# mlelarge/graph_neural_net

Measured on AMD Instinct MI355X. Metric: graph-pairs/sec FGNN fwd+bwd, N=50 regular pairs, higher is better.
Workload: dtype f32

## Files before the change

graph_neural_net_amd/_lib.py:

```python
import ctypes as C
import os

import torch

_HERE = os.path.dirname(os.path.abspath(__file__))
LIB_PATH = os.environ.get('FGNN_LIB') or os.path.join(_HERE, 'libfgnn_hip.so')

FGNN_H = 32
FGNN_TILE = 32
FGNN_MAX_DEPTH = 3
FGNN_RANGE_WG = 256
FGNN_LSAP_MAX_N = 2048
FGNN_MAX_LEVELS = 64
FGNN_QAP_MAX_N = 256
FGNN_QAPW_MAX_N = 256
FGNN_SPECTRAL_MAX_N = 256
FGNN_SPECTRAL_MAX_POWERS = 8
FGNN_PLANTED_MAX_N = 256
FGNN_SCORE_SPLIT = 4

c_float_p = C.c_void_p


class Slab(C.Structure):
    _fields_ = [('ptr', C.c_void_p), ('gstride', C.c_longlong), ('ldp', C.c_longlong), ('C', C.c_int),
                ('nrm', C.c_void_p), ('beta', C.c_void_p)]


class MlpFwdArgs(C.Structure):
    _fields_ = [('G', C.c_int), ('N', C.c_int), ('depth', C.c_int), ('nmlp', C.c_int),
                ('nvalid', C.c_void_p),
                ('a', Slab), ('b', Slab),
                ('W', (C.c_void_p * FGNN_MAX_DEPTH) * 2),
                ('bias', (C.c_void_p * FGNN_MAX_DEPTH) * 2),
                ('z', C.c_void_p * 2),
                ('ldz', C.c_longlong),
                ('part', C.c_void_p * 2),
                ('cnt', C.c_void_p), ('packed', C.c_void_p), ('xbits', C.c_void_p), ('xdeg', C.c_void_p),
                ('ranges', C.c_void_p), ('cu_share', C.c_int)]


class DwJob(C.Structure):
    _fields_ = [('dy', C.c_void_p), ('d_gstride', C.c_longlong), ('d_ld', C.c_longlong), ('relu_mask', C.c_void_p),
                ('x', C.c_void_p), ('x_gstride', C.c_longlong), ('x_ld', C.c_longlong), ('M', C.c_int), ('K', C.c_int)]


class ChainLayer(C.Structure):
    _fields_ = [('W', C.c_void_p), ('w_ostride', C.c_longlong), ('w_kstride', C.c_longlong), ('bias', C.c_void_p),
                ('M', C.c_int), ('K', C.c_int), ('relu', C.c_int), ('mask', C.c_void_p), ('out', C.c_void_p),
                ('o_gstride', C.c_longlong)]


class ChainArgs(C.Structure):
    _fields_ = [('x', C.c_void_p), ('x_gstride', C.c_longlong), ('x_ld', C.c_longlong), ('depth', C.c_int),
                ('layer', ChainLayer * 3), ('o_ld', C.c_longlong), ('nvalid', C.c_void_p), ('G', C.c_int), ('N', C.c_int)]


class Mlp64Args(C.Structure):
    _fields_ = [('x', C.c_void_p), ('x_gstride', C.c_longlong), ('x_ld', C.c_longlong), ('cin', C.c_int),
                ('xb', C.c_void_p), ('xb_gstride', C.c_longlong), ('xb_ld', C.c_longlong), ('cb', C.c_int),
                ('packed', C.c_void_p), ('nvalid', C.c_void_p), ('G', C.c_int), ('N', C.c_int),
                ('out', C.c_void_p), ('o_gstride', C.c_longlong), ('o_ld', C.c_longlong),
                ('dz', C.c_void_p), ('dz_gstride', C.c_longlong), ('dz_ld', C.c_longlong),
                ('dx', C.c_void_p), ('dx_gstride', C.c_longlong), ('dx_ld', C.c_longlong),
                ('dxb', C.c_void_p), ('dxb_gstride', C.c_longlong), ('dxb_ld', C.c_longlong),
                ('accumulate_dx', C.c_int), ('accumulate_dxb', C.c_int),
                ('wpart', C.c_void_p)]


class Mlp64PackJob(C.Structure):
    _fields_ = [('W', C.c_void_p * 3), ('bias', C.c_void_p * 3), ('cin', C.c_int), ('packed', C.c_void_p)]


class MlpBwdArgs(C.Structure):
    _fields_ = [('G', C.c_int), ('N', C.c_int), ('depth', C.c_int),
                ('nvalid', C.c_void_p),
                ('a', Slab), ('b', Slab),
                ('W', C.c_void_p * FGNN_MAX_DEPTH),
                ('bias', C.c_void_p * FGNN_MAX_DEPTH),
                ('dy', C.c_void_p), ('dgstride', C.c_longlong), ('ldd', C.c_longlong),
                ('z', C.c_void_p), ('zgstride', C.c_longlong), ('ldz', C.c_longlong),
                ('coef', C.c_void_p), ('s12', C.c_void_p), ('znrm', C.c_void_p),
                ('dxa', C.c_void_p), ('dxa_gstride', C.c_longlong), ('dxa_ld', C.c_longlong),
                ('dxb', C.c_void_p), ('dxb_gstride', C.c_longlong), ('dxb_ld', C.c_longlong),
                ('accumulate_a', C.c_int), ('accumulate_b', C.c_int),
                ('wpart', C.c_void_p), ('s12part', C.c_void_p), ('packed', C.c_void_p),
                ('s12tiles', C.c_void_p), ('s12_out', C.c_void_p), ('xbits', C.c_void_p), ('xdeg', C.c_void_p),
                ('ranges', C.c_void_p), ('cu_share', C.c_int)]


class Slab16(C.Structure):
    _fields_ = [('ptr', C.c_void_p), ('gstride', C.c_longlong), ('ldp', C.c_longlong), ('C', C.c_int),
                ('nrm', C.c_void_p), ('beta', C.c_void_p)]


class MlpFwd16Args(C.Structure):
    _fields_ = [('G', C.c_int), ('N', C.c_int), ('ldr', C.c_int), ('depth', C.c_int), ('nmlp', C.c_int),
                ('nvalid', C.c_void_p),
                ('a', Slab16), ('b', Slab16),
                ('z', C.c_void_p * 2), ('ldz', C.c_longlong),
                ('part', C.c_void_p * 2), ('cnt', C.c_void_p), ('packed', C.c_void_p), ('ranges', C.c_void_p)]


class MlpBwd16Args(C.Structure):
    _fields_ = [('G', C.c_int), ('N', C.c_int), ('ldr', C.c_int), ('depth', C.c_int),
                ('nvalid', C.c_void_p),
                ('a', Slab16), ('b', Slab16),
                ('dy', C.c_void_p), ('dgstride', C.c_longlong), ('ldd', C.c_longlong),
                ('z', C.c_void_p), ('zgstride', C.c_longlong), ('ldz', C.c_longlong),
                ('coef', C.c_void_p),
                ('dxa', C.c_void_p), ('dxa_gstride', C.c_longlong), ('dxa_ld', C.c_longlong),
                ('dxb', C.c_void_p), ('dxb_gstride', C.c_longlong), ('dxb_ld', C.c_longlong),
                ('accumulate_a', C.c_int), ('accumulate_b', C.c_int),
                ('wpart', C.c_void_p), ('s12part', C.c_void_p), ('packed', C.c_void_p), ('ranges', C.c_void_p)]


class GradJob(C.Structure):
    _fields_ = [('wpart', C.c_void_p), ('count', C.c_int), ('out', C.c_void_p), ('s12', C.c_void_p),
                ('nrm', C.c_void_p), ('dgn_w', C.c_void_p), ('dgn_b', C.c_void_p), ('rows', C.c_int), ('scale', C.c_float), ('scale_dev', C.c_void_p)]


class PackJob(C.Structure):
    _fields_ = [('kind', C.c_int), ('ca', C.c_int), ('cb', C.c_int), ('depth', C.c_int), ('nmlp', C.c_int),
                ('W', (C.c_void_p * FGNN_MAX_DEPTH) * 2), ('bias', (C.c_void_p * FGNN_MAX_DEPTH) * 2),
                ('out', C.c_void_p)]


class PairgenArgs(C.Structure):
    _fields_ = [('seed', C.c_ulonglong), ('first', C.c_longlong), ('B', C.c_int), ('N', C.c_int),
                ('family', C.c_int), ('noise_model', C.c_int), ('edge_density', C.c_double),
                ('thr_edge', C.c_ulonglong), ('thr_noise1', C.c_ulonglong), ('thr_noise2', C.c_ulonglong),
                ('thr_vertex', C.c_ulonglong), ('swaps_per_edge', C.c_int),
                ('bits1', C.c_void_p), ('bits2', C.c_void_p), ('nvalid', C.c_void_p)]


FGNN_GUARD_MAX_PARTS = 64
FGNN_GUARD_SKIP_NONFINITE = 1
FGNN_GUARD_NONFINITE = 1


class GuardRecord(C.Structure):
    _fields_ = [('max_norm', C.c_double), ('norm', C.c_double), ('coef', C.c_double),
                ('flags', C.c_int), ('skipped', C.c_int), ('arrivals', C.c_int), ('mode', C.c_int),
                ('partial', C.c_double * FGNN_GUARD_MAX_PARTS)]


class EvalRecord(C.Structure):
    _fields_ = [('ce_sum', C.c_double), ('nodes', C.c_longlong), ('correct_lsap', C.c_longlong), ('correct_max', C.c_longlong),
                ('pairs', C.c_longlong), ('steps', C.c_longlong)]


MAX_GRAD_JOBS = 16
MAX_PACK_JOBS = 24
_VP, _LL, _I, _F = C.c_void_p, C.c_longlong, C.c_int, C.c_float

_SIGNATURES = {
    'fgnn_last_error': [],
    'fgnn_version': [],
    'fgnn_tiles_per_graph': [_I],
    'fgnn_mlp_bwd_num_workgroups': [],
    'fgnn_pack_floats': [_I, _I, _I, _I, _I],
    'fgnn_pack_operands': [_VP, _I, _VP],
    'fgnn_mlp_fwd': [C.POINTER(MlpFwdArgs), _VP],
    'fgnn_pack_x3_floats': [_I, _I, _I, _I, _I],
    'fgnn_pack_x3_operands': [_VP, _I, _VP],
    'fgnn_mlp_fwd_x3': [C.POINTER(MlpFwdArgs), _VP],
    'fgnn_debug_mlp_fwd_masks': [C.POINTER(MlpFwdArgs), _VP, _VP, _VP],
    'fgnn_debug_mlp_fwd_x3_masks': [C.POINTER(MlpFwdArgs), _VP, _VP, _VP],
    'fgnn_debug_matmul_variant': [_I],
    'fgnn_gn_finalize': [_VP, _VP, _VP, _VP, _I, _I, _I, _F, _VP, _VP],
    'fgnn_gn_finalize2': [_VP, _VP, _VP, _VP, _VP, _VP, _I, _I, _I, _F, _VP, _VP, _VP],
    'fgnn_gn_plane_supported': [_I],
    'fgnn_gn_plane_fwd': [_VP, _LL, _LL, _VP, _VP, _VP, _I, _I, _I, _F, _VP, _LL, _LL, _VP, _VP],
    'fgnn_gn_plane_bwd': [_VP, _LL, _LL, _VP, _LL, _LL, _VP, _VP, _I, _I, _I, _VP, _LL, _LL, _VP, _VP, _VP, _VP],
    'fgnn_gn_stats': [_VP, _LL, _LL, _VP, _VP, _I, _I, _I, _F, _VP, _VP],
    'fgnn_gn_apply': [_VP, _LL, _LL, _VP, _VP, _VP, _I, _I, _I, _VP, _LL, _LL, _VP],
    'fgnn_ragged_tile_ranges': [_VP, _I, _I, _VP, _VP],
    'fgnn_ragged_tile_ranges_order': [_VP, _I, _I, _VP, _VP, _VP],
    'fgnn_ragged_tile_ranges16': [_VP, _I, _I, _I, _VP, _VP],
    'fgnn_conv1x1_dw_multi': [C.POINTER(DwJob), _I, _VP, _I, _I, _VP, _VP],
    'fgnn_conv_chain_supported': [_I, _I, C.POINTER(C.c_int)],
    'fgnn_conv_chain': [C.POINTER(ChainArgs), _VP],
    'fgnn_mlp64_supported': [_I, _I, _I],
    'fgnn_mlp64_num_workgroups': [],
    'fgnn_mlp64_param_count': [_I],
    'fgnn_mlp64_packed_floats': [_I],
    'fgnn_mlp64_pack': [_VP, _VP, _VP, _VP, _VP, _VP, _I, _VP, _VP],
    'fgnn_mlp64_pack_multi': [C.POINTER(Mlp64PackJob), _I, _VP],
    'fgnn_mlp64_fwd': [C.POINTER(Mlp64Args), _VP],
    'fgnn_mlp64_bwd': [C.POINTER(Mlp64Args), _VP],
    'fgnn_conv1x1': [_VP, _LL, _LL, _VP, _VP, _LL, _LL, _VP, _I, _VP, _I, _I, _I, _I, _VP, _LL, _LL, _VP],
    'fgnn_conv1x1_dw_chunks': [_I, _I],
    'fgnn_conv1x1_dw': [_VP, _LL, _LL, _VP, _VP, _LL, _LL, _VP, _I, _I, _I, _I, _VP, _VP],
    'fgnn_chan_matmul_fwd': [C.POINTER(Slab), C.POINTER(Slab), _VP, _I, _I, _VP, _LL, _LL, _VP],
    'fgnn_chan_matmul_fwd_ord': [C.POINTER(Slab), C.POINTER(Slab), _VP, _I, _I, _VP, _LL, _LL, _VP, _I, _VP],
    'fgnn_chan_matmul_fwd_fin_supported': [_I],
    'fgnn_chan_matmul_fwd_fin': [C.POINTER(Slab), C.POINTER(Slab), _VP, _VP, _VP, _VP, _VP, _F, _VP, _I, _I, _VP, _LL, _LL, _VP],
    'fgnn_chan_matmul_fwd_fin_ord': [C.POINTER(Slab), C.POINTER(Slab), _VP, _VP, _VP, _VP, _VP, _F, _VP, _I, _I, _VP, _LL, _LL, _VP, _I, _VP],
    'fgnn_colmax_fwd': [C.POINTER(Slab), _VP, _I, _I, _VP, _VP, _VP],
    'fgnn_colmax_fwd_fin_supported': [_I],
    'fgnn_colmax_fwd_fin': [C.POINTER(Slab), _VP, _VP, _VP, _F, _VP, _I, _I, _VP, _VP, _VP],
    'fgnn_score_ce_fwd': [_VP, _VP, _VP, _I, _I, _I, _VP, _VP, _VP, _VP],
    'fgnn_score_row_blocks': [_I, _I],
    'fgnn_score_ce_fwd_blocks': [_VP, _VP, _VP, _I, _I, _I, _I, _VP, _VP, _VP, _VP],
    'fgnn_score_ce_bwd': [_VP, _VP, _VP, _VP, _VP, _VP, _I, _I, _I, _VP, _VP, _VP],
    'fgnn_score_ce_fwd_blocks_labels': [_VP, _VP, _VP, _VP, _I, _I, _I, _I, _VP, _VP, _VP, _VP],
    'fgnn_score_ce_bwd_labels': [_VP, _VP, _VP, _VP, _VP, _VP, _VP, _I, _I, _I, _VP, _VP, _VP],
    'fgnn_score_ce_bwd_w': [_VP, _VP, _VP, _VP, _VP, _VP, _VP, _VP, _I, _I, _I, _VP, _VP, _VP],
    'fgnn_pair_weights': [_VP, _VP, _I, _VP, _I, _I, _VP, _VP, _VP],
    'fgnn_pair_loss_w': [_VP, _I, _VP, _I, _VP, _VP],
    'fgnn_ce_fwd_labels': [_VP, _VP, _VP, _I, _I, _VP, _VP, _VP],
    'fgnn_ce_bwd_labels': [_VP, _VP, _VP, _VP, _VP, _I, _I, _VP, _VP],
    'fgnn_inv_node_count': [_VP, _I, _VP, _VP],
    'fgnn_score_bwd': [_VP, _VP, _VP, _VP, _I, _I, _I, _VP, _VP, _VP],
    'fgnn_ce_fwd': [_VP, _VP, _I, _I, _VP, _VP, _VP],
    'fgnn_ce_bwd': [_VP, _VP, _VP, _VP, _I, _I, _VP, _VP],
    'fgnn_colmax_bwd': [_VP, _VP, _VP, _I, _I, _I, _VP, _LL, _LL, C.POINTER(Slab), _VP, _VP],
    'fgnn_gn_bwd_stats': [_VP, _LL, _LL, _VP, _LL, _LL, _VP, _VP, _I, _I, _I, _VP, _VP],
    'fgnn_gn_bwd_coef': [_VP, _VP, _VP, _I, _I, _I, _VP, _VP, _VP, _VP],
    'fgnn_gn_bwd_coef_tiles': [_VP, _VP, _VP, _I, _I, _I, _VP, _VP, _VP],
    'fgnn_grad_finalize': [_VP, _I, _I, _I, _I, _VP],
    'fgnn_gn_bwd_apply': [_VP, _LL, _LL, _VP, _LL, _LL, _VP, _VP, _I, _I, _I, _VP, _LL, _LL, _VP],
    'fgnn_mlp_bwd': [C.POINTER(MlpBwdArgs), _VP],
    'fgnn_mlp_bwd_x3': [C.POINTER(MlpBwdArgs), _VP],
    'fgnn_mlp_bwd_pair': [C.POINTER(MlpBwdArgs), C.POINTER(MlpBwdArgs), _VP],
    'fgnn_mlp_bwd_t16': [C.POINTER(MlpBwdArgs), _VP],
    'fgnn_mlp_bwd_t16_supported': [C.POINTER(MlpBwdArgs)],
    'fgnn_mlp_bwd_pair_t16': [C.POINTER(MlpBwdArgs), C.POINTER(MlpBwdArgs), _VP],
    'fgnn_mlp_bwd_pair_x3': [C.POINTER(MlpBwdArgs), C.POINTER(MlpBwdArgs), _VP],
    'fgnn_block1_struct_supported': [_I, _I, _I],
    'fgnn_block1_struct_table_floats': [_I],
    'fgnn_block1_struct_ws_floats': [_I, _I],
    'fgnn_block1_struct_rows': [_I, _I],
    'fgnn_block1_struct_fwd': [_VP, _VP, _I, _I, _VP, _VP, _VP, _VP, _VP, C.c_float, _VP, _VP, _VP, _LL, _LL, _VP, _VP, _VP, _VP, _VP, _VP, _VP],
    'fgnn_block1_struct_bwd': [_VP, _VP, _I, _I, _VP, _VP, _VP, _VP, _VP, _VP, _VP, _VP, _LL, _LL, _VP, _VP, _VP, _VP, _VP, _VP],
    'fgnn_block1_struct_fwd_pack': [_VP, _VP, _I, _I, _VP, _VP, _VP, _VP, _VP, C.c_float, _VP, _VP, _VP, _LL, _LL, _VP, _VP, _VP, _VP, _VP, _VP, _VP, _I, _VP],
    'fgnn_block1_struct_fwd16_pack': [_VP, _VP, _I, _I, _I, _VP, _VP, _VP, _VP, _VP, C.c_float, _VP, _VP, _VP, _LL, _LL, _VP, _VP, _VP, _VP, _VP, _VP, _VP, _I, _VP],
    'fgnn_block1_struct_fwd16': [_VP, _VP, _I, _I, _I, _VP, _VP, _VP, _VP, _VP, C.c_float, _VP, _VP, _VP, _LL, _LL, _VP, _VP, _VP, _VP, _VP, _VP, _VP],
    'fgnn_block1_struct_bwd16': [_VP, _VP, _I, _I, _I, _VP, _VP, _VP, _VP, _VP, _VP, _VP, _VP, _LL, _LL, _VP, _VP, _VP, _VP, _VP, _VP],
    'fgnn_mlp_bwd_coef_tiles_supported': [_I, _I],
    'fgnn_mlp_param_count': [_I, _I],
    'fgnn_reduce_partials': [_VP, _I, _I, _VP, _VP],
    'fgnn_chan_matmul_bwd': [C.POINTER(Slab), C.POINTER(Slab), _VP, _LL, _LL, _VP, _I, _I, _VP, _VP, _LL, _LL, _VP, _VP, _VP],
    'fgnn_chan_matmul_bwd_ord': [C.POINTER(Slab), C.POINTER(Slab), _VP, _LL, _LL, _VP, _I, _I, _VP, _VP, _LL, _LL, _VP, _VP, _VP, _I, _VP],
    'fgnn_sum_scale': [_VP, _I, _I, _F, _VP, _VP],
    'fgnn_adam_step': [_VP, _VP, _VP, _VP, _I, C.c_double, C.c_double, C.c_double, C.c_double, _I, C.c_double, _VP],
    'fgnn_adam_step_dev': [_VP, _VP, _VP, _VP, _I, _VP, _VP, _VP],
    'fgnn_grad_guard': [_VP, _I, _VP, _VP, _VP],
    'fgnn_adam_step_guarded': [_VP, _VP, _VP, _VP, _I, _VP, _VP, _VP, _VP],
    'fgnn_expand_adjacency': [_VP, _VP, _I, _I, _VP, _VP],
    'fgnn_pack_adjacency': [_VP, _VP, _I, _I, _VP, _VP, _VP],
    'fgnn_pack_adjacency_ld': [_VP, _VP, _I, _I, _I, _VP, _VP, _VP],
    'fgnn_pack_adjacency_pair': [_VP, _VP, _VP, _VP, _I, _I, _I, _VP, _VP, _VP, _VP, _VP],
    'fgnn_adjacency_degree': [_VP, _VP, _I, _I, _VP, _VP],
    'fgnn_accuracy_max': [_VP, _VP, _I, _I, _VP, _VP],
    'fgnn_lsap_accuracy': [_VP, _LL, _I, _VP, _I, _I, _VP, _VP, _VP],
    'fgnn_pairgen_supported': [_I, _I, _I],
    'fgnn_pairgen': [C.POINTER(PairgenArgs), _VP],
    'fgnn_pairgen_indexed': [C.POINTER(PairgenArgs), _VP, _VP],
    'fgnn_pairgen_levels': [C.POINTER(PairgenArgs), _VP, _VP, _I, _VP, _VP],
    'fgnn_epoch_index': [C.c_ulonglong, C.c_ulonglong, _LL, _LL, _LL, _VP, _VP],
    'fgnn_qap_objective': [_VP, _VP, _VP, _VP, _I, _I, _VP, _VP, _VP, _VP, _VP],
    'fgnn_qap_improve_cost': [_VP, _VP, _VP, _VP, _I, _I, _VP, _LL, _I, _VP],
    'fgnn_greedy_qap_ws_bytes': [_I, _I],
    'fgnn_greedy_qap': [_VP, _VP, _VP, _VP, _I, _I, _I, _VP, _LL, _VP, _VP, _VP, _VP, _VP],
    'fgnn_greedy_qap_labels': [_VP, _VP, _VP, _VP, _VP, _I, _I, _I, _VP, _LL, _VP, _VP, _VP, _VP, _VP],
    'fgnn_qapw_objective': [_VP, _VP, _LL, _I, _VP, _VP, _I, _I, _VP, _VP, _VP, _VP, _VP, _VP],
    'fgnn_qapw_improve_cost': [_VP, _VP, _LL, _I, _VP, _VP, _I, _I, _VP, _LL, _I, _VP],
    'fgnn_greedy_qapw_ws_bytes': [_I, _I],
    'fgnn_greedy_qapw': [_VP, _VP, _LL, _I, _VP, _VP, _I, _I, _I, _VP, _LL, _VP, _VP, _VP, _VP, _VP],
    'fgnn_greedy_qapw_labels': [_VP, _VP, _LL, _I, _VP, _VP, _VP, _I, _I, _I, _VP, _LL, _VP, _VP, _VP, _VP, _VP],
    'fgnn_planted_perm': [C.c_ulonglong, _LL, _VP, _VP, _I, _I, _VP, _VP],
    'fgnn_relabel_bits': [_VP, _VP, _VP, _I, _I, _VP, _VP],
    'fgnn_relabel_dense': [_VP, _VP, _VP, _I, _I, _I, _I, _VP, _VP],
    'fgnn_count_matches': [_VP, _VP, _VP, _I, _I, _VP, _VP],
    'fgnn_accuracy_max_labels': [_VP, _VP, _VP, _I, _I, _VP, _VP],
    'fgnn_spectral_features': [_VP, _VP, _I, _I, _I, _VP, _I, _VP],
    'fgnn_eval_pairs': [_VP, _VP, _VP, _I, _I, _VP, _LL, _I, _VP, _VP, _VP],
    'fgnn_eval_pairs_labels': [_VP, _VP, _VP, _I, _I, _VP, _LL, _I, _VP, _VP, _VP],
    'fgnn_eval_fold': [_VP, _VP, _VP, _VP, _I, _I, _I, _VP, _VP, _VP, _VP],
    'fgnn_eval_fold_bins': [_VP, _VP, _VP, _VP, _I, _I, _I, _VP, _I, _VP, _VP, _VP, _VP],
    'fgnn_tiles_per_graph16': [_I, _I],
    'fgnn_to_bf16': [_VP, _VP, _I, _I, _I, _I, _VP, _LL, _LL, _VP],
    'fgnn_from_bf16': [_VP, _LL, _LL, _I, _I, _I, _I, _VP, _VP],
    'fgnn_to_bf16_pad': [_VP, _VP, _I, _I, _I, _I, _I, _VP, _LL, _VP],
    'fgnn_pack16_floats': [_I, _I, _I, _I, _I],
    'fgnn_pack16_operands': [_VP, _I, _VP],
    'fgnn_mlp_fwd16': [C.POINTER(MlpFwd16Args), _VP],
    'fgnn_debug_mlp_fwd16_masks': [C.POINTER(MlpFwd16Args), _VP, _VP, _VP],
    'fgnn_gn_finalize_tpg': [_VP, _VP, _VP, _VP, _I, _I, _I, _I, _F, _VP, _VP],
    'fgnn_gn_finalize2_tpg': [_VP, _VP, _VP, _VP, _VP, _VP, _I, _I, _I, _I, _F, _VP, _VP, _VP],
    'fgnn_gn_bwd_coef_tiles_tpg': [_VP, _VP, _VP, _I, _I, _I, _I, _VP, _VP, _VP],
    'fgnn_chan_matmul_fwd16': [C.POINTER(Slab16), C.POINTER(Slab16), _VP, _I, _I, _I, _VP, _LL, _LL, _VP],
    'fgnn_chan_matmul_fwd16_fin': [C.POINTER(Slab16), C.POINTER(Slab16), _VP, _VP, _VP, _VP, _VP, _F, _I, _VP, _I, _I, _I, _VP, _LL,
                                   _LL, _VP],
    'fgnn_chan_matmul_bwd16': [C.POINTER(Slab16), C.POINTER(Slab16), _VP, _LL, _LL, _VP, _I, _I, _I, _VP, _VP, _LL, _LL, _VP, _VP, _VP],
    'fgnn_chan_matmul_bwd16_t': [C.POINTER(Slab16), C.POINTER(Slab16), _VP, _LL, _LL, _VP, _I, _VP, _I, _I, _I, _VP, _VP, _LL, _LL,
                                 _VP, _VP, _VP],
    'fgnn_chan_matmul_bwd16_tc': [C.POINTER(Slab16), C.POINTER(Slab16), _VP, _LL, _LL, _VP, _I, _VP, _I, _I, _I, _VP, _VP, _LL, _LL,
                                  _VP, _VP, _VP, _VP, _VP],
    'fgnn_colmax_bwd16_coef': [_VP, _VP, _VP, _I, _I, _I, _I, _VP, _LL, _LL, C.POINTER(Slab16), _VP, _VP, _VP],
    'fgnn_colmax_fwd16': [C.POINTER(Slab16), _VP, _I, _I, _I, _VP, _VP, _VP],
    'fgnn_colmax_bwd16': [_VP, _VP, _VP, _I, _I, _I, _I, _VP, _LL, _LL, C.POINTER(Slab16), _VP, _VP],
    'fgnn_mlp_bwd16': [C.POINTER(MlpBwd16Args), _VP],
    'fgnn_mlp_bwd16_pair': [C.POINTER(MlpBwd16Args), C.POINTER(MlpBwd16Args), _VP],
}
_RESTYPES = {'fgnn_last_error': C.c_char_p, 'fgnn_block1_struct_ws_floats': C.c_longlong, 'fgnn_greedy_qap_ws_bytes': C.c_longlong,
             'fgnn_greedy_qapw_ws_bytes': C.c_longlong}
EXPORTS = tuple(_SIGNATURES)

_lib = None


def load(allow_missing=False):
    global _lib
    if _lib is not None:
        return _lib
    if not os.path.exists(LIB_PATH):
        raise RuntimeError(
            'graph_neural_net_amd: %s is missing. Build it with '
            '`python -c "import __graft_entry__ as g; g.build()"` or `make -C graph_neural_net_amd/csrc`. '
            'There is no CPU fallback.' % LIB_PATH)
    lib = C.CDLL(LIB_PATH)
    for name, argtypes in _SIGNATURES.items():
        if allow_missing and not hasattr(lib, name):
            continue
        fn = getattr(lib, name)
        fn.argtypes = argtypes
        fn.restype = _RESTYPES.get(name, C.c_int)
    _lib = lib
    return lib


def last_error():
    return load().fgnn_last_error().decode('utf-8', 'replace')


PROFILE = None


def call(name, *args, tag=None):
    if PROFILE is not None:
        e0 = torch.cuda.Event(enable_timing=True)
        e1 = torch.cuda.Event(enable_timing=True)
        e0.record()
        rc = getattr(load(), name)(*args)
        e1.record()
        PROFILE.append((tag or name, e0, e1, name, args))
    else:
        rc = getattr(load(), name)(*args)
    if rc != 0:
        raise RuntimeError('%s failed (rc=%d): %s' % (name, rc, last_error()))


def relaunch(name, args):
    rc = getattr(load(), name)(*args[:-1], stream_ptr())
    if rc != 0:
        raise RuntimeError('%s failed (rc=%d): %s' % (name, rc, last_error()))


def stream_ptr():
    return C.c_void_p(torch.cuda.current_stream().cuda_stream)


def ptr(t):
    if t is None:
        return None
    if not t.is_cuda:
        raise RuntimeError('graph_neural_net_amd: expected a CUDA/HIP tensor, got device %s '
                           '(there is no CPU path)' % (t.device,))
    return C.c_void_p(t.data_ptr())


def make_slab(t, gstride, ldp, channels, nrm=None, beta=None):
    s = Slab()
    s.ptr = t.data_ptr() if t is not None else None
    s.gstride = gstride
    s.ldp = ldp
    s.C = channels
    s.nrm = nrm.data_ptr() if nrm is not None else None
    s.beta = beta.data_ptr() if beta is not None else None
    return s


def make_slab16(t, gstride, ldp, channels, nrm=None, beta=None):
    s = Slab16()
    s.ptr = t.data_ptr() if t is not None else None
    s.gstride = gstride
    s.ldp = ldp
    s.C = channels
    s.nrm = nrm.data_ptr() if nrm is not None else None
    s.beta = beta if isinstance(beta, int) else (beta.data_ptr() if beta is not None else None)
    return s


def tiles_per_graph(n):
    return (n * n + FGNN_TILE - 1) // FGNN_TILE


def mlp_param_count(cin, depth):
    return 32 * cin + 32 + (depth - 1) * (32 * 32 + 32)
```

graph_neural_net_amd/csrc/fgnn_bwd32.h:

```cpp
#pragma once
#include "fgnn_common.h"

namespace {

constexpr int BWD_WG = 256;
constexpr int NW = 8;
constexpr int NP = 4;
static_assert(BWD_WG == FGNN_RANGE_WG, "fgnn_ragged_tile_ranges splits for the backward grid");

DEVI float4 coef_from_sums(const float4 n, const float2 sv, float nv) {
    const float m = nv * nv;
    float4 k;
    k.x = n.x;
    k.y = n.y;
    k.z = m > 0.f ? -n.y * sv.y * n.w / m : 0.f;
    k.w = m > 0.f ? -n.y * sv.x / m : 0.f;
    return k;
}
DEVI float4 coef_record(const fgnn_mlp_bwd_args &A, int g, int ch, int nv) {
    if (A.coef) return reinterpret_cast<const float4 *>(A.coef)[(long long)g * FGNN_H + ch];
    const float4 n = reinterpret_cast<const float4 *>(A.znrm)[(long long)g * FGNN_H + ch];
    const float2 sv = reinterpret_cast<const float2 *>(A.s12)[(long long)g * FGNN_H + ch];
    return coef_from_sums(n, sv, (float)nv);
}
DEVI float4 coef_record(const fgnn_mlp_bwd_args &A, int g, int ch) {
    if (A.coef) return reinterpret_cast<const float4 *>(A.coef)[(long long)g * FGNN_H + ch];
    const float4 n = reinterpret_cast<const float4 *>(A.znrm)[(long long)g * FGNN_H + ch];
    const float2 sv = reinterpret_cast<const float2 *>(A.s12)[(long long)g * FGNN_H + ch];
    return coef_from_sums(n, sv, (float)nvalid_of(A.nvalid, g, A.N));
}


struct PairArgs {
    fgnn_mlp_bwd_args m[2];
};

template <int PCOUNT, int NWV>
DEVI void sum_wave_partials(const float *smem, float *wpart) {
    static_assert(PCOUNT % 4 == 0, "partials are summed four at a time");
    float4 *out = reinterpret_cast<float4 *>(wpart + (long long)blockIdx.x * PCOUNT);
    const float4 *part4 = reinterpret_cast<const float4 *>(smem);
    for (int e = threadIdx.x; e < PCOUNT / 4; e += 64 * NWV) {
        float4 a = part4[e];
#pragma unroll
        for (int w = 1; w < NWV; ++w) {
            const float4 b = part4[w * (PCOUNT / 4) + e];
            a.x += b.x;
            a.y += b.y;
            a.z += b.z;
            a.w += b.w;
        }
        out[e] = a;
    }
}
template <int PCOUNT>
DEVI void sum_pair_partials(const float *smem, const PairArgs &P) {
    static_assert(PCOUNT % 4 == 0, "partials are summed four at a time");
    const float4 *part4 = reinterpret_cast<const float4 *>(smem);
    for (int e = threadIdx.x; e < 2 * (PCOUNT / 4); e += 64 * NW) {
        const int m = e >= PCOUNT / 4 ? 1 : 0, ee = e - m * (PCOUNT / 4);
        float4 a = part4[(4 * m) * (PCOUNT / 4) + ee];
#pragma unroll
        for (int w = 1; w < NP; ++w) {
            const float4 b = part4[(4 * m + w) * (PCOUNT / 4) + ee];
            a.x += b.x;
            a.y += b.y;
            a.z += b.z;
            a.w += b.w;
        }
        reinterpret_cast<float4 *>(P.m[m].wpart + (long long)blockIdx.x * PCOUNT)[ee] = a;
    }
}

inline int check_mlp_bwd_common(const fgnn_mlp_bwd_args *a, const char *fn, int tile_bits) {
    FGNN_CHECK(a->dy && a->z && a->wpart, "%s: missing dy/z/wpart", fn);
    FGNN_CHECK(a->coef || (a->s12 && a->znrm) || (a->s12tiles && a->znrm), "%s: need coef, or s12 + znrm, or s12tiles + znrm", fn);
    const long long lim = 0x7fffffffll / 4, G = a->G;
    FGNN_CHECK(G * a->a.gstride < lim && G * a->b.gstride < lim && G * a->dgstride < lim && G * a->zgstride < lim &&
               G * a->dxa_gstride < lim && G * a->dxb_gstride < lim,
               "%s: a tensor exceeds 2 GiB (32-bit buffer addressing); split the batch", fn);
    FGNN_CHECK(G * fgnn_tiles_per_graph(a->N) < (1ll << tile_bits), "%s: too many tiles", fn);
    FGNN_CHECK(BWD_WG == fgnn_mlp_bwd_num_workgroups(), "%s: workgroup count differs from fgnn_mlp_bwd", fn);
    return 0;
}
inline int check_pair_common(const fgnn_mlp_bwd_args *a1, const fgnn_mlp_bwd_args *a2, const char *fn, int tile_bits, bool dense_only) {
    FGNN_CHECK(a1 && a2, "%s: null args", fn);
    FGNN_CHECK(BWD_WG == fgnn_mlp_bwd_num_workgroups(), "%s: workgroup count differs from fgnn_mlp_bwd", fn);
    FGNN_CHECK(a1->G > 0 && a1->N > 0 && a1->G == a2->G && a1->N == a2->N && a1->depth == a2->depth,
               "%s: the two MLPs must share G, N and depth", fn);
    FGNN_CHECK((!dense_only || a1->a.ptr) && a1->a.ptr == a2->a.ptr && a1->a.C == a2->a.C && a1->a.gstride == a2->a.gstride &&
               a1->a.ldp == a2->a.ldp && a1->a.nrm == a2->a.nrm && a1->a.beta == a2->a.beta &&
               (dense_only || (a1->xbits == a2->xbits && a1->xdeg == a2->xdeg)) && a1->nvalid == a2->nvalid,
               "%s: the two MLPs must read the same input slab", fn);
    FGNN_CHECK(!a1->dxa && !a1->s12part, "%s: the input gradient and its tile sums belong to the SECOND argument block", fn);
    FGNN_CHECK(!a1->s12tiles && !a2->s12tiles, "%s: s12tiles is an mlp3 feature", fn);
    for (const fgnn_mlp_bwd_args *a : {a1, a2}) {
        FGNN_CHECK(a->dy && a->z && a->wpart, "%s: missing dy/z/wpart", fn);
        FGNN_CHECK(a->coef || (a->s12 && a->znrm), "%s: need coef, or s12 + znrm", fn);
        const long long lim = 0x7fffffffll / 4, G = a->G;
        FGNN_CHECK(G * a->a.gstride < lim && G * a->dgstride < lim && G * a->zgstride < lim && G * a->dxa_gstride < lim,
                   "%s: a tensor exceeds 2 GiB (32-bit buffer addressing); split the batch", fn);
    }
    FGNN_CHECK((long long)a1->G * fgnn_tiles_per_graph(a1->N) < (1ll << tile_bits), "%s: too many tiles", fn);
    return 0;
}

}
```

graph_neural_net_amd/csrc/fgnn_bwd_t16.h:

```cpp
#pragma once
#include "fgnn_t16.h"
#include "fgnn_pack.h"
#include "fgnn_bwd32.h"

namespace {

using namespace t16;

template <int CB, int IMAGES, int NSLOTS>
struct BwdT16Layout {
    static constexpr int DEPTH = 3;
    static constexpr PkBwd PK = pk_bwd(32, CB, DEPTH);
    static constexpr int OFF_W1 = PK.off_wh, OFF_WT1 = PK.off_wt, OFF_WT2 = PK.off_wt + 16;
    static constexpr int BIAS_F = PK.bias_f;
    static constexpr int WEIGHT_F = pk_pad_floats(PK.floats);
    static constexpr int NSLOT = NSLOTS;
    static constexpr int CIN = 32 + CB;
    static constexpr int PCOUNT = 32 * CIN + 32 + (DEPTH - 1) * (32 * 32 + 32);
    static constexpr int TILE_OFF = IMAGES * WEIGHT_F;
    static constexpr int TILE_END = TILE_OFF + NW * NSLOT * TILE_F;
    static constexpr int RED_F = NW * PCOUNT;
};


#define FGNN_T16_READ_RECORDS(norm)                                 \
    _Pragma("unroll") for (int s = 0; s < 8; ++s) {                 \
        const float4 k4 = rec[chan_s(s) + chan_q(q)];               \
        kx[s] = k4.x;                                               \
        ky[s] = k4.y;                                               \
        kz[s] = k4.z;                                               \
        kw[s] = k4.w;                                               \
        if (norm) {                                                 \
            const float4 n = rec[32 + chan_s(s) + chan_q(q)];       \
            mean[s] = n.x;                                          \
            av[s] = n.y;                                            \
        }                                                           \
    }

#define FGNN_T16_RECOMPUTE_HIDDEN(acc, h1, h2)                                              \
    _Pragma("unroll") for (int s = 0; s < 8; ++s) h1[s] = relu1(acc[s >> 2][s & 3]);        \
    stage8(S0, lane_base, h1);                                                              \
    load_bias(acc, wl + L::BIAS_F, 1, q);                                                   \
    gemm32<L::OFF_W1>(acc, wl, h1, lane);                                                   \
    _Pragma("unroll") for (int s = 0; s < 8; ++s) h2[s] = relu1(acc[s >> 2][s & 3]);        \
    stage8(S1, lane_base, h2);

#define FGNN_T16_DZ(dpre)                                                                                                   \
    _Pragma("unroll") for (int s = 0; s < 8; ++s) dpre[s] = fmaf(kz[s], zr[s] - kx[s], fmaf(ky[s], dyr[s], kw[s]));         \
    if (!full) {                                                                                                            \
        _Pragma("unroll") for (int s = 0; s < 8; ++s) dpre[s] = valid ? dpre[s] : 0.f;                                      \
    }

#define FGNN_T16_HIDDEN_BWD(OFF_WT, dpre, dW, db, Dt, In, h)                                                \
    {                                                                                                       \
        f32x4 a2[2];                                                                                        \
        a2[0] = a2[1] = zero4();                                                                            \
        gemm32<OFF_WT>(a2, wl, dpre, lane);                                                                 \
        wgrad16(dW, db, Dt, In, lane);                                                                      \
        _Pragma("unroll") for (int s = 0; s < 8; ++s) dpre[s] = h[s] > 0.f ? a2[s >> 2][s & 3] : 0.f;       \
    }

#define FGNN_T16_DB_BUTTERFLY(db0, db1, db2)            \
    _Pragma("unroll") for (int b = 0; b < 2; ++b) {     \
        db0[b] += __shfl_xor(db0[b], 16);               \
        db0[b] += __shfl_xor(db0[b], 32);               \
        db1[b] += __shfl_xor(db1[b], 16);               \
        db1[b] += __shfl_xor(db1[b], 32);               \
        db2[b] += __shfl_xor(db2[b], 16);               \
        db2[b] += __shfl_xor(db2[b], 32);               \
    }

}
```

graph_neural_net_amd/csrc/fgnn_norm.h:

```cpp
#pragma once
#include "fgnn_common.h"

DEVI float4 nrm_record(float mean, float m2, float m, float nv, float w, float eps) {
    const float var = m > 0.f ? m2 / m : 0.f;
    const float ve = var + eps;
    const float q = nv > 0.f ? 1.f / (2.f * sqrtf(nv * ve)) : 0.f;
    float4 o;
    o.x = mean;
    o.y = w * q;
    o.z = q;
    o.w = 1.f / ve;
    return o;
}

struct TilePartials {
    float nb[4], mb[4], qb[4];
};
DEVI TilePartials finalize_load(const float *part, const float *cnt, int g, int c, int C, int tpg, int lane, bool tr = false) {
    TilePartials p;
    const int ts = tr ? 1 : C, cs = tr ? tpg : 1;
#pragma unroll
    for (int k = 0; k < 4; ++k) {
        const int t = lane + WAVE * k;
        const bool ok = t < tpg;
        const int tc = ok ? t : 0;
        const float n = cnt[(long long)g * tpg + tc];
        const float2 pm = reinterpret_cast<const float2 *>(part)[(long long)g * tpg * C + (long long)tc * ts + (long long)c * cs];
        p.nb[k] = ok ? n : 0.f;
        p.mb[k] = pm.x;
        p.qb[k] = ok ? pm.y : 0.f;
    }
    return p;
}
DEVI float4 finalize_reduce(const TilePartials &p, float nv, float w, float eps) {
    float sn = 0.f, sm = 0.f;
#pragma unroll
    for (int k = 0; k < 4; ++k) {
        sn += p.nb[k];
        sm += p.nb[k] * p.mb[k];
    }
    sn = wave_sum(sn);
    sm = wave_sum(sm);
    const float mean = sn > 0.f ? sm / sn : 0.f;
    float m2 = 0.f;
#pragma unroll
    for (int k = 0; k < 4; ++k) {
        const float d = p.mb[k] - mean;
        m2 += p.qb[k] + p.nb[k] * d * d;
    }
    m2 = wave_sum(m2);
    return nrm_record(mean, m2, sn, nv, w, eps);
}

struct NormRec {
    float mean, a, beta;
    bool on;
};
DEVI NormRec norm_of(const fgnn_slab &s, int g, int c) {
    NormRec r;
    r.on = s.nrm != nullptr;
    if (r.on) {
        const float4 n = reinterpret_cast<const float4 *>(s.nrm)[(long long)g * s.C + c];
        r.mean = n.x;
        r.a = n.y;
        r.beta = s.beta ? s.beta[c] : 0.f;
    } else {
        r.mean = 0.f;
        r.a = 1.f;
        r.beta = 0.f;
    }
    return r;
}
DEVI NormRec norm_from(const float4 &n, const fgnn_slab &s, int c) {
    NormRec r;
    r.on = true;
    r.mean = n.x;
    r.a = n.y;
    r.beta = s.beta ? s.beta[c] : 0.f;
    return r;
}

DEVI float4 finalize_wave(const float *part, const float *cnt, int g, int c, int C, int tpg, float nv, float w, float eps,
                          int lane, bool tr = false) {
    return finalize_reduce(finalize_load(part, cnt, g, c, C, tpg, lane, tr), nv, w, eps);
}
DEVI float4 finalize_wave_any(const float *part, const float *cnt, int g, int c, int C, int tpg, float nv, float w, float eps, int lane,
                              bool tr = false) {
    if (tpg <= 4 * WAVE) return finalize_wave(part, cnt, g, c, C, tpg, nv, w, eps, lane, tr);
    constexpr int U = 8;
    float sn = 0.f, sm = 0.f;
    const float *cg = cnt + (long long)g * tpg;
    const int ts = tr ? 1 : C;
    const float2 *pg = reinterpret_cast<const float2 *>(part) + (long long)g * tpg * C + (long long)c * (tr ? tpg : 1);
    for (int t0 = lane; t0 < tpg; t0 += U * WAVE) {
        float n[U], x[U];
#pragma unroll
        for (int k = 0; k < U; ++k) {
            const int t = t0 + k * WAVE, tc = t < tpg ? t : 0;
            n[k] = t < tpg ? cg[tc] : 0.f;
            x[k] = pg[(long long)tc * ts].x;
        }
#pragma unroll
        for (int k = 0; k < U; ++k) {
            sn += n[k];
            sm += n[k] * x[k];
        }
    }
    sn = wave_sum(sn);
    sm = wave_sum(sm);
    const float mean = sn > 0.f ? sm / sn : 0.f;
    float m2 = 0.f;
    for (int t0 = lane; t0 < tpg; t0 += U * WAVE) {
        float n[U];
        float2 pm[U];
#pragma unroll
        for (int k = 0; k < U; ++k) {
            const int t = t0 + k * WAVE, tc = t < tpg ? t : 0;
            n[k] = t < tpg ? cg[tc] : 0.f;
            pm[k] = pg[(long long)tc * ts];
            if (t >= tpg) pm[k].y = 0.f;
        }
#pragma unroll
        for (int k = 0; k < U; ++k) {
            const float d = pm[k].x - mean;
            m2 += pm[k].y + n[k] * d * d;
        }
    }
    m2 = wave_sum(m2);
    return nrm_record(mean, m2, sn, nv, w, eps);
}
```

graph_neural_net_amd/csrc/matmul.hip:

```cpp
#include "fgnn_common.h"
#include "fgnn_norm.h"

namespace {

constexpr int TM = 64;
constexpr int LDS_LD = 65;

DEVI void stage_tile(float *lds, const float *mat, int N, int nv, int row0, int col0, const NormRec &nr, int tid) {
    if (row0 == 0 && col0 == 0 && N <= TM) {
        for (int e = tid; e < TM * TM; e += 256) lds[(e >> 6) * LDS_LD + (e & 63)] = 0.f;
        __syncthreads();
        const int P = N * N;
        for (int e = tid; e < P; e += 256) {
            const int r = e / N, c = e - r * N;
            float v = mat[e];
            const bool ok = r < nv && c < nv;
            v = ok ? (nr.on ? (v - nr.mean) * nr.a + nr.beta : v) : 0.f;
            lds[r * LDS_LD + c] = v;
        }
    } else {
        for (int e = tid; e < TM * TM; e += 256) {
            const int r = e >> 6, c = e & 63;
            const int gr = row0 + r, gc = col0 + c;
            float v = 0.f;
            if (gr < nv && gc < nv) {
                v = mat[(long long)gr * N + gc];
                if (nr.on) v = (v - nr.mean) * nr.a + nr.beta;
            }
            lds[r * LDS_LD + c] = v;
        }
    }
}

DEVI void store_quadrant(float *out, int N, int row0, int col0, const f32x16 &acc, int lane) {
    const int j = lane & 31, h = lane >> 5;
    const int col = col0 + j;
#pragma unroll
    for (int r = 0; r < 16; ++r) {
        const int row = row0 + ch_of(r, h);
        if (row < N && col < N) out[(long long)row * N + col] = acc[r];
    }
}

DEVI void s12_epilogue(float (&red)[4][4], float sa1, float sa2, float sb1, float sb2, float *s12a, float *s12b, int gc, int tid) {
    const int lane = tid & 63, wave = tid >> 6;
    sa1 = wave_sum(sa1);
    sa2 = wave_sum(sa2);
    sb1 = wave_sum(sb1);
    sb2 = wave_sum(sb2);
    if (lane == 0) {
        red[wave][0] = sa1;
        red[wave][1] = sa2;
        red[wave][2] = sb1;
        red[wave][3] = sb2;
    }
    __syncthreads();
    if (tid < 4) {
        const float v = (red[0][tid] + red[1][tid]) + (red[2][tid] + red[3][tid]);
        float *dst = (tid < 2 ? s12a : s12b) + (long long)gc * 2 + (tid & 1);
        *dst = v;
    }
}

__global__ __launch_bounds__(256) void chan_matmul_fwd_kernel(const fgnn_slab ya, const fgnn_slab yb,
                                                              const int *nvalid, int N, float *out,
                                                              long long ogstride, long long ldo) {
    __shared__ float As[TM * LDS_LD];
    __shared__ float Bs[TM * LDS_LD];
    const int C = ya.C;
    const int gc = blockIdx.z;
    const int g = gc / C, c = gc - g * C;
    const int nv = nvalid_of(nvalid, g, N);
    const int row0 = blockIdx.y * TM, col0 = blockIdx.x * TM;
    const int tid = threadIdx.x, lane = tid & 63, wave = tid >> 6;
    const int qi = wave >> 1, qj = wave & 1;
    const int j = lane & 31, h = lane >> 5;
    const float *A = ya.ptr + (long long)g * ya.gstride + (long long)c * ya.ldp;
    const float *B = yb.ptr + (long long)g * yb.gstride + (long long)c * yb.ldp;
    const NormRec na = norm_of(ya, g, c), nb = norm_of(yb, g, c);
    float *O = out + (long long)g * ogstride + (long long)c * ldo;

    f32x16 acc;
#pragma unroll
    for (int r = 0; r < 16; ++r) acc[r] = 0.f;
    const bool live = (row0 + 32 * qi < N) && (col0 + 32 * qj < N);

    for (int k0 = 0; k0 < N; k0 += TM) {
        if (k0) __syncthreads();
        stage_tile(As, A, N, nv, row0, k0, na, tid);
        stage_tile(Bs, B, N, nv, k0, col0, nb, tid);
        __syncthreads();
        if (live) {
            const int kmax = (N - k0 < TM ? N - k0 : TM);
            const float *ap = As + (32 * qi + j) * LDS_LD + h;
            const float *bp = Bs + h * LDS_LD + 32 * qj + j;
            for (int k = 0; k < kmax; k += 2) acc = mfma32(ap[k], bp[k * LDS_LD], acc);
        }
    }
    if (live) store_quadrant(O, N, row0 + 32 * qi, col0 + 32 * qj, acc, lane);
}

__global__ __launch_bounds__(256) void chan_matmul_bwd_kernel(const fgnn_slab ya, const fgnn_slab yb,
                                                              const float *dm, long long dmg, long long ldm,
                                                              const int *nvalid, int N, float *da, float *db,
                                                              long long ogstride, long long ldo, float *s12a,
                                                              float *s12b) {
    __shared__ float Xs[TM * LDS_LD];
    __shared__ float Ds[TM * LDS_LD];
    __shared__ float red[4][4];
    const int C = ya.C;
    const int gc = blockIdx.z;
    const int g = gc / C, c = gc - g * C;
    const int nv = nvalid_of(nvalid, g, N);
    const int row0 = blockIdx.y * TM, col0 = blockIdx.x * TM;
    const int tid = threadIdx.x, lane = tid & 63, wave = tid >> 6;
    const int qi = wave >> 1, qj = wave & 1;
    const int j = lane & 31, h = lane >> 5;
    const float *A = ya.ptr + (long long)g * ya.gstride + (long long)c * ya.ldp;
    const float *B = yb.ptr + (long long)g * yb.gstride + (long long)c * yb.ldp;
    const float *D = dm + (long long)g * dmg + (long long)c * ldm;
    const NormRec na = norm_of(ya, g, c), nb = norm_of(yb, g, c);
    NormRec none;
    none.on = false; none.mean = 0.f; none.a = 1.f; none.beta = 0.f;
    float *OA = da + (long long)g * ogstride + (long long)c * ldo;
    float *OB = db + (long long)g * ogstride + (long long)c * ldo;
    const bool live = (row0 + 32 * qi < N) && (col0 + 32 * qj < N);

    f32x16 acc;
#pragma unroll
    for (int r = 0; r < 16; ++r) acc[r] = 0.f;
    for (int j0 = 0; j0 < N; j0 += TM) {
        if (j0) __syncthreads();
        stage_tile(Ds, D, N, nv, row0, j0, none, tid);
        stage_tile(Xs, B, N, nv, col0, j0, nb, tid);
        __syncthreads();
        if (live) {
            const int kmax = (N - j0 < TM ? N - j0 : TM);
            const float *ap = Ds + (32 * qi + j) * LDS_LD + h;
            const float *bp = Xs + (32 * qj + j) * LDS_LD + h;
            for (int k = 0; k < kmax; k += 2) acc = mfma32(ap[k], bp[k], acc);
        }
    }
    if (live) store_quadrant(OA, N, row0 + 32 * qi, col0 + 32 * qj, acc, lane);
    float sa1 = 0.f, sa2 = 0.f, sb1 = 0.f, sb2 = 0.f;
    if (s12a && live) {
        const int col = col0 + 32 * qj + j;
#pragma unroll
        for (int r = 0; r < 16; ++r) {
            const int row = row0 + 32 * qi + ch_of(r, h);
            if (row < nv && col < nv) {
                sa1 += acc[r];
                sa2 += acc[r] * (A[(long long)row * N + col] - na.mean);
            }
        }
    }

#pragma unroll
    for (int r = 0; r < 16; ++r) acc[r] = 0.f;
    for (int i0 = 0; i0 < N; i0 += TM) {
        __syncthreads();
        stage_tile(Xs, A, N, nv, i0, row0, na, tid);
        stage_tile(Ds, D, N, nv, i0, col0, none, tid);
        __syncthreads();
        if (live) {
            const int kmax = (N - i0 < TM ? N - i0 : TM);
            const float *ap = Xs + h * LDS_LD + 32 * qi + j;
            const float *bp = Ds + h * LDS_LD + 32 * qj + j;
            for (int k = 0; k < kmax; k += 2) acc = mfma32(ap[k * LDS_LD], bp[k * LDS_LD], acc);
        }
    }
    if (live) store_quadrant(OB, N, row0 + 32 * qi, col0 + 32 * qj, acc, lane);
    if (s12a) {
        if (live) {
            const int col = col0 + 32 * qj + j;
#pragma unroll
            for (int r = 0; r < 16; ++r) {
                const int row = row0 + 32 * qi + ch_of(r, h);
                if (row < nv && col < nv) {
                    sb1 += acc[r];
                    sb2 += acc[r] * (B[(long long)row * N + col] - nb.mean);
                }
            }
        }
        s12_epilogue(red, sa1, sa2, sb1, sb2, s12a, s12b, gc, tid);
    }
}

template <bool WANT_U>
DEVI void load_tile_regs(float (&v)[16], float (&u)[16], const float *mat, int N, int nv, const NormRec &nr, int tid) {
#pragma unroll
    for (int k = 0; k < 16; ++k) {
        const int e = tid + 256 * k;
        const int r = e >> 6, c = e & 63;
        const bool ok = r < nv && c < nv;
        const float x = mat[ok ? r * N + c : 0];
        const float d = x - nr.mean;
        v[k] = ok ? (nr.on ? d * nr.a + nr.beta : x) : 0.f;
        if (WANT_U) u[k] = ok ? d : 0.f;
    }
}
DEVI void store_tile_lds(float *lds, const float (&v)[16], int tid) {
#pragma unroll
    for (int k = 0; k < 16; ++k) {
        const int e = tid + 256 * k;
        lds[(e >> 6) * LDS_LD + (e & 63)] = v[k];
    }
}
DEVI void frag_to_lds(float *lds, int row0, int col0, const f32x16 &acc, int lane) {
    const int j = lane & 31, h = lane >> 5;
#pragma unroll
    for (int r = 0; r < 16; ++r) lds[(row0 + ch_of(r, h)) * LDS_LD + col0 + j] = acc[r];
}
template <bool WANT_S>
DEVI void tile_to_global(const View &ov, int mat_off4, const float *lds, int N, const float (&u)[16], float &s1,
                         float &s2, int tid) {
    const int c = tid & 63, r0 = __builtin_amdgcn_readfirstlane(tid >> 6);
    const int voff = c < N ? (r0 * N + c) * 4 : OOB_OFF;
    const float *lp = lds + r0 * LDS_LD + c;
#pragma unroll
    for (int k = 0; k < 16; ++k) {
        const float t = lp[4 * k * LDS_LD];
        buf_store(t, ov, r0 + 4 * k < N ? voff : OOB_OFF, mat_off4 + k * 16 * N);
        if (WANT_S) {
            s1 += t;
            s2 += t * u[k];
        }
    }
}

DEVI void load_tile_raw(float (&x)[16], const View &v, int mat_off4, int N, int nv, int tid) {
    const int c = tid & 63, r0 = __builtin_amdgcn_readfirstlane(tid >> 6);
    const int voff = c < nv ? (r0 * N + c) * 4 : OOB_OFF;
#pragma unroll
    for (int k = 0; k < 16; ++k) {
        const int r = r0 + 4 * k;
        x[k] = buf_load(v, r < nv ? voff : OOB_OFF, mat_off4 + k * 16 * N);
    }
}
template <bool WANT_U>
DEVI void finish_tile(float (&v)[16], float (&u)[16], const float (&x)[16], int nv, const NormRec &nr, int tid) {
#pragma unroll
    for (int k = 0; k < 16; ++k) {
        const int e = tid + 256 * k;
        const int r = e >> 6, c = e & 63;
        const bool ok = r < nv && c < nv;
        const float d = x[k] - nr.mean;
        v[k] = ok ? (nr.on ? d * nr.a + nr.beta : x[k]) : 0.f;
        if (WANT_U) u[k] = ok ? d : 0.f;
    }
}

struct FinArgs {
    const float *part_a, *part_b, *cnt, *gw_a, *gw_b;
    float *nrm_a, *nrm_b;
    float eps;
    int tpg;
};
template <bool FIN>
__global__ __launch_bounds__(256, 4) void chan_matmul_fwd1_kernel(const fgnn_slab ya, const fgnn_slab yb,
                                                               const int *nvalid, int N, int M, float *out,
                                                               long long ogstride, long long ldo, const FinArgs F) {
    __shared__ float As[TM * LDS_LD];
    __shared__ float Bs[TM * LDS_LD];
    __shared__ float4 fin_rec[2];
    const int C = ya.C;
    const int tid = threadIdx.x, lane = tid & 63, wave = tid >> 6;
    const int qi = wave >> 1, qj = wave & 1;
    const int j = lane & 31, h = lane >> 5;
    float xa[16], xb[16], dummy[16];
    const int G = M / C;
    const View vA = make_view(ya.ptr, ya.gstride, ya.ldp, G), vB = make_view(yb.ptr, yb.gstride, yb.ldp, G);
    const View vO = make_view(out, ogstride, ldo, G);
    const int gc = blockIdx.x;
    {
        const int g = gc / C, c = gc - g * C;
        const int nv = nvalid_of(nvalid, g, N);
        TilePartials tp;
        if (FIN && wave < 2) tp = finalize_load(wave ? F.part_b : F.part_a, F.cnt, g, c, C, F.tpg, lane);
        load_tile_raw(xa, vA, g * vA.gs4 + c * vA.ld4, N, nv, tid);
        load_tile_raw(xb, vB, g * vB.gs4 + c * vB.ld4, N, nv, tid);
        NormRec na, nb;
        if (FIN) {
            if (wave < 2) {
                const float4 r = finalize_reduce(tp, (float)nv, (wave ? F.gw_b : F.gw_a) ? (wave ? F.gw_b : F.gw_a)[c] : 1.f, F.eps);
                if (lane == 0) {
                    fin_rec[wave] = r;
                    reinterpret_cast<float4 *>(wave ? F.nrm_b : F.nrm_a)[gc] = r;
                }
            }
            __syncthreads();
            const float4 ra = fin_rec[0], rb = fin_rec[1];
            na = norm_from(ra, ya, c);
            nb = norm_from(rb, yb, c);
        } else {
            na = norm_of(ya, g, c);
            nb = norm_of(yb, g, c);
        }
        const int o_off = g * vO.gs4 + c * vO.ld4;
        {
            float va[16], vb[16];
            finish_tile<false>(va, dummy, xa, nv, na, tid);
            finish_tile<false>(vb, dummy, xb, nv, nb, tid);
            store_tile_lds(As, va, tid);
            store_tile_lds(Bs, vb, tid);
        }
        __syncthreads();
        f32x16 acc;
#pragma unroll
        for (int r = 0; r < 16; ++r) acc[r] = 0.f;
        if (32 * qi < N && 32 * qj < N) {
            const float *ap = As + (32 * qi + j) * LDS_LD + h;
            const float *bp = Bs + h * LDS_LD + 32 * qj + j;
            for (int k = 0; k < N; k += 2) acc = mfma32(ap[k], bp[k * LDS_LD], acc);
        }
        __syncthreads();
        frag_to_lds(As, 32 * qi, 32 * qj, acc, lane);
        __syncthreads();
        float s1 = 0.f, s2 = 0.f;
        tile_to_global<false>(vO, o_off, As, N, dummy, s1, s2, tid);
    }
}

__global__ __launch_bounds__(256, 4) void chan_matmul_bwd1_kernel(const fgnn_slab ya, const fgnn_slab yb,
                                                               const float *dm, long long dmg, long long ldm,
                                                               const int *nvalid, int N, int M, float *da, float *db,
                                                               long long ogstride, long long ldo, float *s12a,
                                                               float *s12b) {
    __shared__ float Bs[TM * LDS_LD];
    __shared__ float Ds[TM * LDS_LD];
    __shared__ float red[4][4];
    const int C = ya.C;
    const int tid = threadIdx.x, lane = tid & 63, wave = tid >> 6;
    const int qi = wave >> 1, qj = wave & 1;
    const int j = lane & 31, h = lane >> 5;
    NormRec none;
    none.on = false; none.mean = 0.f; none.a = 1.f; none.beta = 0.f;
    float xa[16], xb[16], xd[16], dummy[16];
    const int G = M / C;
    const View vA = make_view(ya.ptr, ya.gstride, ya.ldp, G), vB = make_view(yb.ptr, yb.gstride, yb.ldp, G);
    const View vD = make_view(dm, dmg, ldm, G);
    const View vOA = make_view(da, ogstride, ldo, G), vOB = make_view(db, ogstride, ldo, G);
    const int gc = blockIdx.x;
    {
        const int g = gc / C, c = gc - g * C;
        const int nv = nvalid_of(nvalid, g, N);
        load_tile_raw(xa, vA, g * vA.gs4 + c * vA.ld4, N, nv, tid);
        load_tile_raw(xb, vB, g * vB.gs4 + c * vB.ld4, N, nv, tid);
        load_tile_raw(xd, vD, g * vD.gs4 + c * vD.ld4, N, nv, tid);
        const NormRec na = norm_of(ya, g, c), nb = norm_of(yb, g, c);
        const int o_off = g * vOA.gs4 + c * vOA.ld4;
        float ua[16], ub[16], va[16];
        finish_tile<true>(va, ua, xa, nv, na, tid);
        {
            float vb[16], vd[16];
            finish_tile<true>(vb, ub, xb, nv, nb, tid);
            finish_tile<false>(vd, dummy, xd, nv, none, tid);
            store_tile_lds(Bs, vb, tid);
            store_tile_lds(Ds, vd, tid);
        }
        __syncthreads();
        const bool live = 32 * qi < N && 32 * qj < N;
        f32x16 accA, accB;
#pragma unroll
        for (int r = 0; r < 16; ++r) {
            accA[r] = 0.f;
            accB[r] = 0.f;
        }
        if (live) {
            const float *ap = Ds + (32 * qi + j) * LDS_LD + h;
            const float *bp = Bs + (32 * qj + j) * LDS_LD + h;
            for (int k = 0; k < N; k += 2) accA = mfma32(ap[k], bp[k], accA);
        }
        __syncthreads();
        store_tile_lds(Bs, va, tid);
        __syncthreads();
        if (live) {
            const float *ap = Bs + h * LDS_LD + 32 * qi + j;
            const float *bp = Ds + h * LDS_LD + 32 * qj + j;
            for (int k = 0; k < N; k += 2) accB = mfma32(ap[k * LDS_LD], bp[k * LDS_LD], accB);
        }
        __syncthreads();
        frag_to_lds(Ds, 32 * qi, 32 * qj, accA, lane);
        frag_to_lds(Bs, 32 * qi, 32 * qj, accB, lane);
        __syncthreads();
        float sa1 = 0.f, sa2 = 0.f, sb1 = 0.f, sb2 = 0.f;
        if (s12a) {
            tile_to_global<true>(vOA, o_off, Ds, N, ua, sa1, sa2, tid);
            tile_to_global<true>(vOB, o_off, Bs, N, ub, sb1, sb2, tid);
            s12_epilogue(red, sa1, sa2, sb1, sb2, s12a, s12b, gc, tid);
        } else {
            tile_to_global<false>(vOA, o_off, Ds, N, dummy, sa1, sa2, tid);
            tile_to_global<false>(vOB, o_off, Bs, N, dummy, sb1, sb2, tid);
        }
    }
}


int g_mm_wave_variant = 1;
inline bool mm_wave_variant() { return (g_mm_wave_variant & 1) != 0; }
inline bool mm_narrow() { return (g_mm_wave_variant & 8) != 0; }
constexpr int WLD = 68;
constexpr int W_WAVES = 2;

DEVI rsrc_t mat_rsrc(const float *p, int bytes) {
    return __builtin_amdgcn_make_buffer_rsrc(const_cast<float *>(p), 0, bytes, 0x00020000);
}
DEVI float rsrc_load(rsrc_t r, int voff, int soff) {
    return __builtin_bit_cast(float, __builtin_amdgcn_raw_buffer_load_b32(r, voff, soff, 0));
}
DEVI void rsrc_store(float x, rsrc_t r, int voff, int soff) {
    __builtin_amdgcn_raw_buffer_store_b32(__builtin_bit_cast(unsigned, x), r, voff, soff, 0);
}
DEVI float2 rsrc_load2(rsrc_t r, int voff, int soff) {
    typedef unsigned u2 __attribute__((ext_vector_type(2)));
    const u2 v = __builtin_amdgcn_raw_buffer_load_b64(r, voff, soff, 0);
    const unsigned a = v.x, b = v.y;
    return make_float2(__builtin_bit_cast(float, a), __builtin_bit_cast(float, b));
}
DEVI void rsrc_store2(float x, float y, rsrc_t r, int voff, int soff) {
    typedef unsigned u2 __attribute__((ext_vector_type(2)));
    u2 v;
    v.x = __builtin_bit_cast(unsigned, x);
    v.y = __builtin_bit_cast(unsigned, y);
    __builtin_amdgcn_raw_buffer_store_b64(v, r, voff, soff, 0);
}

#define FGNN_W_CONTEXT(LDS_FLOATS)                                                                                       \
    __shared__ __attribute__((aligned(16))) float lds[W_WAVES * (LDS_FLOATS)];                                           \
    const int lane = threadIdx.x & 63, wv = __builtin_amdgcn_readfirstlane(threadIdx.x >> 6);                            \
    const int gc = xcd_swizzle(blockIdx.x, gridDim.x) * W_WAVES + wv;                                                    \
    if (gc >= M) return;                                                                                                 \
    const int C = ya.C;                                                                                                  \
    const int g = gc / C, c = gc - g * C;                                                                                \
    const int nv = __builtin_amdgcn_readfirstlane(nvalid_of(nvalid, g, N));                                              \
    const int j = lane & 31, h = lane >> 5;                                                                              \
    float *As = lds + wv * (LDS_FLOATS);                                                                                 \
    const rsrc_t rA = mat_rsrc(ya.ptr + (long long)g * ya.gstride + (long long)c * ya.ldp, nv * N * 4);                  \
    const rsrc_t rB = mat_rsrc(yb.ptr + (long long)g * yb.gstride + (long long)c * yb.ldp, nv * N * 4);                  \
    const rsrc_t rO = mat_rsrc(out + (long long)g * ogstride + (long long)c * ldo, N * N * 4);
#define FGNN_W_PRODUCTS(NB_, BVAL)                                                                                       \
    f32x16 acc[NB_][NB_];                                                                                                \
    _Pragma("unroll") for (int rb = 0; rb < NB_; ++rb)                                                                   \
        _Pragma("unroll") for (int cb = 0; cb < NB_; ++cb)                                                               \
            _Pragma("unroll") for (int r = 0; r < 16; ++r) acc[rb][cb][r] = 0.f;                                         \
    _Pragma("unroll") for (int q = 0; q < KQ; ++q) {                                                                     \
        float4 af[NB_];                                                                                                  \
        _Pragma("unroll") for (int rb = 0; rb < NB_; ++rb)                                                               \
            af[rb] = *reinterpret_cast<const float4 *>(As + (32 * rb + j) * WLD + h * 32 + 4 * q);                       \
        _Pragma("unroll") for (int t = 0; t < 4; ++t) {                                                                  \
            const int s = 4 * q + t;                                                                                     \
            if (q == KQ - 1 && 2 * s >= N) break;                                                                        \
            float bv[NB_];                                                                                               \
            BVAL                                                                                                         \
            _Pragma("unroll") for (int rb = 0; rb < NB_; ++rb) {                                                         \
                const float a = t == 0 ? af[rb].x : (t == 1 ? af[rb].y : (t == 2 ? af[rb].z : af[rb].w));               \
                _Pragma("unroll") for (int cb = 0; cb < NB_; ++cb) acc[rb][cb] = mfma32(a, bv[cb], acc[rb][cb]);         \
            }                                                                                                            \
        }                                                                                                                \
    }
#define FGNN_W_RECORDS                                                                                                   \
    float meanA, aA, meanB, aB;                                                                                          \
    if (FIN) {                                                                                                           \
        const float4 ra = finalize_reduce(ta, (float)nv, F.gw_a ? F.gw_a[c] : 1.f, F.eps);                               \
        const float4 rb = finalize_reduce(tb, (float)nv, F.gw_b ? F.gw_b[c] : 1.f, F.eps);                               \
        if (lane == 0) {                                                                                                 \
            reinterpret_cast<float4 *>(F.nrm_a)[gc] = ra;                                                                \
            reinterpret_cast<float4 *>(F.nrm_b)[gc] = rb;                                                                \
        }                                                                                                                \
        meanA = ra.x; aA = ra.y; meanB = rb.x; aB = rb.y;                                                                \
    } else {                                                                                                             \
        const NormRec na = norm_of(ya, g, c), nb = norm_of(yb, g, c);                                                    \
        meanA = na.mean; aA = na.a; meanB = nb.mean; aB = nb.a;                                                          \
    }                                                                                                                    \
    const bool onA = FIN || ya.nrm != nullptr, onB = FIN || yb.nrm != nullptr;                                           \
    const float betaA = (onA && ya.beta) ? ya.beta[c] : 0.f, betaB = (onB && yb.beta) ? yb.beta[c] : 0.f;
DEVI constexpr int wave_row_off(int rb, int r, int N) { return (32 * rb + (r & 3) + 8 * (r >> 2)) * N * 4; }

template <int KQ>
DEVI void wave_rows_load(float (&x)[8 * KQ], rsrc_t r, int N, int voff) {
#pragma unroll
    for (int i = 0; i < 8 * KQ; ++i) x[i] = rsrc_load(r, voff, i < N ? i * N * 4 : 0);
}
template <int KQ>
DEVI void wave_rows_stage(float *T, const float (&x)[8 * KQ], float mean, float a_eff, float b_eff, int nv, int N, int lane) {
    if (nv < N) {
#pragma unroll
        for (int i = 0; i < 8 * KQ; ++i) {
            const float v = (x[i] - mean) * a_eff + b_eff;
            T[i * WLD + lane] = i < nv ? v : 0.f;
        }
    } else {
#pragma unroll
        for (int i = 0; i < 8 * KQ; ++i) T[i * WLD + lane] = (x[i] - mean) * a_eff + b_eff;
    }
}

template <int KQ, bool FIN>
__global__ __launch_bounds__(64 * W_WAVES, 2) void chan_matmul_fwd_w_kernel(const fgnn_slab ya, const fgnn_slab yb,
                                                                           const int *nvalid, int N, int M, float *out,
                                                                           long long ogstride, long long ldo,
                                                                           const FinArgs F) {
    constexpr int KH = 4 * KQ;
    constexpr bool TWO = KQ > 4;
    constexpr int NB = TWO ? 2 : 1;
    FGNN_W_CONTEXT(32 * NB * WLD)

    TilePartials ta, tb;
    if (FIN) {
        ta = finalize_load(F.part_a, F.cnt, g, c, C, F.tpg, lane);
        tb = finalize_load(F.part_b, F.cnt, g, c, C, F.tpg, lane);
    }
    float xa[8 * KQ], xb[NB][KH];
    wave_rows_load<KQ>(xa, rA, N, lane < nv ? lane * 4 : OOB_OFF);
    int voffB[NB];
#pragma unroll
    for (int cb = 0; cb < NB; ++cb) {
        const int col = 32 * cb + j;
        voffB[cb] = col < nv ? (h * N + col) * 4 : OOB_OFF;
    }
#pragma unroll
    for (int s = 0; s < KH; ++s)
#pragma unroll
        for (int cb = 0; cb < NB; ++cb) xb[cb][s] = rsrc_load(rB, voffB[cb] + s * 2 * N * 4, 0);
    FGNN_W_RECORDS
    {
        const bool okc = lane < nv;
        wave_rows_stage<KQ>(As, xa, meanA, okc ? aA : 0.f, okc ? betaA : 0.f, nv, N, (lane & 1) * 32 + (lane >> 1));
    }
    float aeB[NB], beB[NB];
#pragma unroll
    for (int cb = 0; cb < NB; ++cb) {
        const bool okc = 32 * cb + j < nv;
        aeB[cb] = okc ? aB : 0.f;
        beB[cb] = okc ? betaB : 0.f;
    }
    FGNN_W_PRODUCTS(NB, _Pragma("unroll") for (int cb = 0; cb < NB; ++cb) bv[cb] = (xb[cb][s] - meanB) * aeB[cb] + beB[cb];)
#pragma unroll
    for (int cb = 0; cb < NB; ++cb) {
        const int col = 32 * cb + j;
        const int voffO = col < N ? (4 * h * N + col) * 4 : OOB_OFF;
#pragma unroll
        for (int rb = 0; rb < NB; ++rb)
#pragma unroll
            for (int r = 0; r < 16; ++r) rsrc_store(acc[rb][cb][r], rO, voffO + wave_row_off(rb, r, N), 0);
    }
}

template <int KQ, bool FIN>
__global__ __launch_bounds__(64 * W_WAVES, 2) void chan_matmul_fwd_w2_kernel(const fgnn_slab ya, const fgnn_slab yb,
                                                                            const int *nvalid, int N, int M, float *out,
                                                                            long long ogstride, long long ldo,
                                                                            const FinArgs F) {
    static_assert(KQ > 4, "two column blocks: 32 < N <= 64");
    constexpr int KH = 4 * KQ;
    FGNN_W_CONTEXT(64 * WLD)

    TilePartials ta, tb;
    if (FIN) {
        ta = finalize_load(F.part_a, F.cnt, g, c, C, F.tpg, lane);
        tb = finalize_load(F.part_b, F.cnt, g, c, C, F.tpg, lane);
    }
    const bool ok0 = 2 * j < nv, ok1 = 2 * j + 1 < nv;
    float2 xa[KH], xb[KH];
    {
        const int voffA = ok0 ? (h * N + 2 * j) * 4 : OOB_OFF;
#pragma unroll
        for (int p = 0; p < KH; ++p) xa[p] = rsrc_load2(rA, voffA, 2 * p < N ? 2 * p * N * 4 : 0);
        const int voffB = ok0 ? (h * N + 2 * j) * 4 : OOB_OFF;
#pragma unroll
        for (int s = 0; s < KH; ++s) xb[s] = rsrc_load2(rB, voffB, 2 * s < N ? 2 * s * N * 4 : 0);
    }
    FGNN_W_RECORDS
    {
        const float a0 = ok0 ? aA : 0.f, b0 = ok0 ? betaA : 0.f, a1 = ok1 ? aA : 0.f, b1 = ok1 ? betaA : 0.f;
#pragma unroll
        for (int p = 0; p < KH; ++p) {
            const int row = 2 * p + h;
            const bool rok = row < nv;
            const float v0 = (xa[p].x - meanA) * a0 + b0;
            const float v1 = ((ok1 ? xa[p].y : 0.f) - meanA) * a1 + b1;
            As[row * WLD + j] = rok ? v0 : 0.f;
            As[row * WLD + 32 + j] = rok ? v1 : 0.f;
        }
    }
    const float aeB[2] = {ok0 ? aB : 0.f, ok1 ? aB : 0.f}, beB[2] = {ok0 ? betaB : 0.f, ok1 ? betaB : 0.f};
    FGNN_W_PRODUCTS(2, bv[0] = (xb[s].x - meanB) * aeB[0] + beB[0];
                       bv[1] = ((ok1 ? xb[s].y : 0.f) - meanB) * aeB[1] + beB[1];)
    {
        const bool two = 2 * j + 1 < N;
        const int voffO = 2 * j < N ? (4 * h * N + 2 * j) * 4 : OOB_OFF;
#pragma unroll
        for (int rb = 0; rb < 2; ++rb)
#pragma unroll
            for (int r = 0; r < 16; ++r) {
                if (two) rsrc_store2(acc[rb][0][r], acc[rb][1][r], rO, voffO, wave_row_off(rb, r, N));
                else rsrc_store(acc[rb][0][r], rO, voffO, wave_row_off(rb, r, N));
            }
    }
}

template <bool FIN>
int launch_fwd_w(const fgnn_slab *ya, const fgnn_slab *yb, const int *nvalid, int N, int M, float *out, long long ogstride,
                 long long ldo, const FinArgs &F, hipStream_t st) {
    const int KQ = (N + 7) / 8, grid = (M + W_WAVES - 1) / W_WAVES;
    if (KQ == 8 && !mm_narrow() && (N & 1) == 0) {
        hipLaunchKernelGGL((chan_matmul_fwd_w2_kernel<8, FIN>), dim3(grid), dim3(64 * W_WAVES), 0, st, *ya, *yb, nvalid, N, M, out,
                           ogstride, ldo, F);
        return 0;
    }
#define FGNN_W(K_)                                                                                                       \
    case K_:                                                                                                             \
        hipLaunchKernelGGL((chan_matmul_fwd_w_kernel<K_, FIN>), dim3(grid), dim3(64 * W_WAVES), 0, st, *ya, *yb, nvalid, N, \
                           M, out, ogstride, ldo, F);                                                                    \
        break;
    switch (KQ) {
        FGNN_W(1) FGNN_W(2) FGNN_W(3) FGNN_W(4) FGNN_W(5) FGNN_W(6) FGNN_W(7) FGNN_W(8)
    }
#undef FGNN_W
    return 0;
}

constexpr int BIG_NW = 8, BIG_THREADS = 64 * BIG_NW, BIG_KC = 32, BIG_LDK = 36;
constexpr int BIG_SPLIT_MAX_MATRICES = 8 * 256;

struct BigSrc {
    View v;
    int off4;
    NormRec nr;
};

template <int NT>
struct BigCfg {
    static constexpr int XM = 32 * NT;
    static constexpr int MAXT = NT * NT / BIG_NW;
    static constexpr int SWEEPS = XM * BIG_KC / BIG_THREADS;
    static constexpr int KC_F = XM * BIG_LDK, KR_F = BIG_KC * XM;
    static constexpr int BUF_F = 2 * KC_F;
    static constexpr int LDS_BYTES = 2 * BUF_F * 4;
};

template <int NT, bool KC>
DEVI void big_load(float (&x)[BigCfg<NT>::SWEEPS], const BigSrc &s, int N, int nv, int k0, int tid) {
    using Cf = BigCfg<NT>;
    if (KC) {
        const int kk = tid & 31, xr = tid >> 5;
        const int base = (k0 + kk) < nv ? (xr * N + k0 + kk) * 4 : OOB_OFF;
#pragma unroll
        for (int i = 0; i < Cf::SWEEPS; ++i)
            x[i] = buf_load(s.v, (xr + 16 * i) < nv ? base : OOB_OFF, s.off4 + 16 * i * N * 4);
    } else {
        constexpr int RPS = BIG_THREADS / Cf::XM;
        const int kk = tid / Cf::XM, c = tid % Cf::XM;
        const int base = c < nv ? ((k0 + kk) * N + c) * 4 : OOB_OFF;
#pragma unroll
        for (int i = 0; i < Cf::SWEEPS; ++i)
            x[i] = buf_load(s.v, (k0 + kk + RPS * i) < nv ? base : OOB_OFF, s.off4 + RPS * i * N * 4);
    }
}

template <int NT, bool KC>
DEVI void big_stage(float *P, const float (&x)[BigCfg<NT>::SWEEPS], const BigSrc &s, int nv, int k0, int tid) {
    using Cf = BigCfg<NT>;
    if (KC) {
        const int kk = tid & 31, xr = tid >> 5;
        const bool kok = (k0 + kk) < nv;
        float *dst = P + xr * BIG_LDK + kk;
#pragma unroll
        for (int i = 0; i < Cf::SWEEPS; ++i) {
            const float m = (kok && (xr + 16 * i) < nv) ? 1.f : 0.f;
            dst[16 * i * BIG_LDK] = s.nr.on ? ((x[i] - s.nr.mean) * s.nr.a + s.nr.beta) * m : x[i];
        }
    } else {
        constexpr int RPS = BIG_THREADS / Cf::XM;
        const int kk = tid / Cf::XM, c = tid % Cf::XM;
        const bool cok = c < nv;
        float *dst = P + kk * Cf::XM + c;
#pragma unroll
        for (int i = 0; i < Cf::SWEEPS; ++i) {
            const float m = (cok && (k0 + kk + RPS * i) < nv) ? 1.f : 0.f;
            dst[RPS * i * Cf::XM] = s.nr.on ? ((x[i] - s.nr.mean) * s.nr.a + s.nr.beta) * m : x[i];
        }
    }
}

template <int NT, bool KC>
DEVI void big_operand(float (&o)[16], const float *P, int t, int j, int h) {
    if (KC) {
        const float4 *p = reinterpret_cast<const float4 *>(P + (32 * t + j) * BIG_LDK + 16 * h);
#pragma unroll
        for (int q = 0; q < 4; ++q) {
            const float4 v = p[q];
            o[4 * q + 0] = v.x;
            o[4 * q + 1] = v.y;
            o[4 * q + 2] = v.z;
            o[4 * q + 3] = v.w;
        }
    } else {
        const float *p = P + (16 * h) * BigCfg<NT>::XM + 32 * t + j;
#pragma unroll
        for (int s = 0; s < 16; ++s) o[s] = p[s * BigCfg<NT>::XM];
    }
}

template <int NT, bool KC>
DEVI void big_operand4(float (&o)[4], const float *P, int t, int j, int h, int q) {
    if (KC) {
        const float4 v = reinterpret_cast<const float4 *>(P + (32 * t + j) * BIG_LDK + 16 * h)[q];
        o[0] = v.x;
        o[1] = v.y;
        o[2] = v.z;
        o[3] = v.w;
    } else {
        const float *p = P + (16 * h + 4 * q) * BigCfg<NT>::XM + 32 * t + j;
#pragma unroll
        for (int s = 0; s < 4; ++s) o[s] = p[s * BigCfg<NT>::XM];
    }
}

template <int NT, bool A_KC, bool B_KC>
DEVI void big_gemm(f32x16 (&acc)[BigCfg<NT>::MAXT], const BigSrc &A, const BigSrc &B, float *lds, int N, int nv,
                   int ntv, int tid) {
    using Cf = BigCfg<NT>;
    const int lane = tid & 63, wv = __builtin_amdgcn_readfirstlane(tid >> 6);
    const int j = lane & 31, h = lane >> 5;
    const int T = ntv * ntv;
    constexpr int FA = A_KC ? Cf::KC_F : Cf::KR_F;
#pragma unroll
    for (int ti = 0; ti < Cf::MAXT; ++ti)
#pragma unroll
        for (int r = 0; r < 16; ++r) acc[ti][r] = 0.f;
    const int nkc = (nv + BIG_KC - 1) / BIG_KC;
    int tms[Cf::MAXT], tns[Cf::MAXT];
    if constexpr (NT != 8) {
#pragma unroll
        for (int ti = 0; ti < Cf::MAXT; ++ti) {
            const int t = wv + BIG_NW * ti;
            tms[ti] = t / ntv;
            tns[ti] = t - tms[ti] * ntv;
        }
    }
    float xa[Cf::SWEEPS], xb[Cf::SWEEPS];
    big_load<NT, A_KC>(xa, A, N, nv, 0, tid);
    big_load<NT, B_KC>(xb, B, N, nv, 0, tid);
    big_stage<NT, A_KC>(lds, xa, A, nv, 0, tid);
    big_stage<NT, B_KC>(lds + FA, xb, B, nv, 0, tid);
    __syncthreads();
    for (int c = 0; c < nkc; ++c) {
        const int cur = c & 1;
        const bool more = c + 1 < nkc;
        if (more) {
            big_load<NT, A_KC>(xa, A, N, nv, (c + 1) * BIG_KC, tid);
            big_load<NT, B_KC>(xb, B, N, nv, (c + 1) * BIG_KC, tid);
        }
        const float *pa = lds + cur * Cf::BUF_F, *pb = pa + FA;
        const int kv = nv - c * BIG_KC;
        const int nq = kv >= 13 ? 4 : (kv + 3) >> 2;
        if constexpr (NT == 8) {
#pragma unroll
            for (int ti = 0; ti < Cf::MAXT; ++ti) {
                const int t = wv + BIG_NW * ti;
                if (t < T) {
                    const int tm = t / ntv, tn = t - tm * ntv;
                    float a[16], b[16];
                    big_operand<NT, A_KC>(a, pa, tm, j, h);
                    big_operand<NT, B_KC>(b, pb, tn, j, h);
#pragma unroll
                    for (int s = 0; s < 16; ++s) acc[ti] = mfma32(a[s], b[s], acc[ti]);
                }
            }
        } else {
        for (int q = 0; q < nq; ++q) {
#pragma unroll
            for (int ti = 0; ti < Cf::MAXT; ++ti) {
                if (wv + BIG_NW * ti < T) {
                    float a[4], b[4];
                    big_operand4<NT, A_KC>(a, pa, tms[ti], j, h, q);
                    big_operand4<NT, B_KC>(b, pb, tns[ti], j, h, q);
#pragma unroll
                    for (int s = 0; s < 4; ++s) acc[ti] = mfma32(a[s], b[s], acc[ti]);
                }
            }
        }
        }
        if (more) {
            float *nx = lds + (cur ^ 1) * Cf::BUF_F;
            big_stage<NT, A_KC>(nx, xa, A, nv, (c + 1) * BIG_KC, tid);
            big_stage<NT, B_KC>(nx + FA, xb, B, nv, (c + 1) * BIG_KC, tid);
        }
        __syncthreads();
    }
}

template <int NT, bool WANT_S>
DEVI void big_store(const f32x16 (&acc)[BigCfg<NT>::MAXT], const View &ov, int o_off4, const BigSrc &raw, int N,
                    int nv, int ntv, float &s1, float &s2, int tid) {
    const int lane = tid & 63, wv = __builtin_amdgcn_readfirstlane(tid >> 6);
    const int j = lane & 31, h = lane >> 5;
    const int T = ntv * ntv;
#pragma unroll
    for (int ti = 0; ti < BigCfg<NT>::MAXT; ++ti) {
        const int t = wv + BIG_NW * ti;
        if (t < T) {
            const int tm = t / ntv, tn = t - tm * ntv;
            const int col = 32 * tn + j;
            const int rowb = 32 * tm + 4 * h;
            const int base = col < N ? (rowb * N + col) * 4 : OOB_OFF;
            const int vbase = col < nv ? (rowb * N + col) * 4 : OOB_OFF;
            float u[16];
            if (WANT_S) {
#pragma unroll
                for (int r = 0; r < 16; ++r) {
                    const int dr = (r & 3) + 8 * (r >> 2);
                    u[r] = buf_load(raw.v, (rowb + dr) < nv ? vbase : OOB_OFF, raw.off4 + dr * N * 4);
                }
            }
#pragma unroll
            for (int r = 0; r < 16; ++r) {
                const int dr = (r & 3) + 8 * (r >> 2);
                buf_store(acc[ti][r], ov, (rowb + dr) < N ? base : OOB_OFF, o_off4 + dr * N * 4);
                if (WANT_S) {
                    const float m = ((rowb + dr) < nv && col < nv) ? 1.f : 0.f;
                    s1 += acc[ti][r] * m;
                    s2 += acc[ti][r] * ((u[r] - raw.nr.mean) * m);
                }
            }
        }
    }
}

DEVI void big_zero_fill(const View &ov, int o_off4, int N, int nv, int X, int tid, bool tiles_only) {
    if (X >= N) return;
    if (!tiles_only) {
        for (int e = tid; e < N * N; e += BIG_THREADS) {
            const int r = e / N, c = e - r * N;
            if (r >= X || c >= X) buf_store(0.f, ov, e * 4, o_off4);
        }
        return;
    }
    const int w = N - X;
    for (int e = tid; e < nv * w; e += BIG_THREADS) {
        const int r = e / w, c = X + (e - r * w);
        buf_store(0.f, ov, (r * N + c) * 4, o_off4);
    }
    if (nv == X && tid < 32 && tid < N) buf_store(0.f, ov, (nv * N + tid) * 4, o_off4);
}

DEVI BigSrc big_src(const fgnn_slab &s, int G, int g, int c) {
    BigSrc b;
    b.v = make_view(s.ptr, s.gstride, s.ldp, G);
    b.off4 = g * b.v.gs4 + c * b.v.ld4;
    b.nr = norm_of(s, g, c);
    return b;
}
DEVI BigSrc big_src_plain(const float *p, long long gs, long long ld, int G, int g, int c) {
    BigSrc b;
    b.v = make_view(p, gs, ld, G);
    b.off4 = g * b.v.gs4 + c * b.v.ld4;
    b.nr.on = false;
    b.nr.mean = 0.f;
    b.nr.a = 1.f;
    b.nr.beta = 0.f;
    return b;
}

template <int NT, bool FIN>
__global__ __launch_bounds__(BIG_THREADS) void chan_matmul_fwd_big_kernel(const fgnn_slab ya, const fgnn_slab yb,
                                                                           const int *nvalid, int N, int G, float *out,
                                                                           long long ogstride, long long ldo,
                                                                           const int *order, const FinArgs F, const int fill) {
    extern __shared__ __attribute__((aligned(16))) float big_lds[];
    __shared__ float4 fin_rec[2];
    const int C = ya.C, gi = blockIdx.x / C, c = blockIdx.x - gi * C, tid = threadIdx.x;
    const int g = order ? order[gi] : gi;
    const int nv = nvalid_of(nvalid, g, N), ntv = (nv + 31) / 32;
    BigSrc A = FIN ? big_src_plain(ya.ptr, ya.gstride, ya.ldp, G, g, c) : big_src(ya, G, g, c);
    BigSrc B = FIN ? big_src_plain(yb.ptr, yb.gstride, yb.ldp, G, g, c) : big_src(yb, G, g, c);
    if (FIN) {
        const int wv = tid >> 6, lane = tid & 63;
        if (wv < 2) {
            const float *gw = wv ? F.gw_b : F.gw_a;
            const float4 r = finalize_wave_any(wv ? F.part_b : F.part_a, F.cnt, g, c, C, F.tpg, (float)nv, gw ? gw[c] : 1.f, F.eps, lane);
            if (lane == 0) {
                fin_rec[wv] = r;
                reinterpret_cast<float4 *>(wv ? F.nrm_b : F.nrm_a)[g * C + c] = r;
            }
        }
        __syncthreads();
        const float4 ra = fin_rec[0], rb = fin_rec[1];
        A.nr = norm_from(ra, ya, c);
        B.nr = norm_from(rb, yb, c);
    }
    const View vO = make_view(out, ogstride, ldo, G);
    const int o_off = g * vO.gs4 + c * vO.ld4;
    big_zero_fill(vO, o_off, N, nv, 32 * ntv, tid, fill != 0);
    if (ntv == 0) return;
    f32x16 acc[BigCfg<NT>::MAXT];
    big_gemm<NT, true, false>(acc, A, B, big_lds, N, nv, ntv, tid);
    float s1 = 0.f, s2 = 0.f;
    big_store<NT, false>(acc, vO, o_off, A, N, nv, ntv, s1, s2, tid);
}

template <int NT>
__global__ __launch_bounds__(BIG_THREADS) void chan_matmul_bwd_big_kernel(const fgnn_slab ya, const fgnn_slab yb,
                                                                           const float *dm, long long dmg, long long ldm,
                                                                           const int *nvalid, int N, int G, float *da,
                                                                           float *db, long long ogstride, long long ldo,
                                                                           float *s12a, float *s12b, const int *order,
                                                                           int split, const int fill) {
    extern __shared__ __attribute__((aligned(16))) float big_lds[];
    __shared__ float red[BIG_NW][4];
    const int item = split ? blockIdx.x >> 1 : blockIdx.x;
    const bool do_a = !split || (blockIdx.x & 1) == 0, do_b = !split || (blockIdx.x & 1) == 1;
    const int C = ya.C, gi = item / C, c = item - gi * C, tid = threadIdx.x;
    const int g = order ? order[gi] : gi, gc = g * C + c;
    const int lane = tid & 63, wv = tid >> 6;
    const int nv = nvalid_of(nvalid, g, N), ntv = (nv + 31) / 32;
    const BigSrc A = big_src(ya, G, g, c), B = big_src(yb, G, g, c);
    const BigSrc D = big_src_plain(dm, dmg, ldm, G, g, c);
    const View vOA = make_view(da, ogstride, ldo, G), vOB = make_view(db, ogstride, ldo, G);
    const int o_off = g * vOA.gs4 + c * vOA.ld4;
    if (do_a) big_zero_fill(vOA, o_off, N, nv, 32 * ntv, tid, fill != 0);
    if (do_b) big_zero_fill(vOB, o_off, N, nv, 32 * ntv, tid, fill != 0);
    float sa1 = 0.f, sa2 = 0.f, sb1 = 0.f, sb2 = 0.f;
    if (ntv > 0) {
        f32x16 acc[BigCfg<NT>::MAXT];
        if (do_a) {
            big_gemm<NT, true, true>(acc, D, B, big_lds, N, nv, ntv, tid);
            if (s12a) big_store<NT, true>(acc, vOA, o_off, A, N, nv, ntv, sa1, sa2, tid);
            else big_store<NT, false>(acc, vOA, o_off, A, N, nv, ntv, sa1, sa2, tid);
        }
        if (do_b) {
            big_gemm<NT, false, false>(acc, A, D, big_lds, N, nv, ntv, tid);
            if (s12a) big_store<NT, true>(acc, vOB, o_off, B, N, nv, ntv, sb1, sb2, tid);
            else big_store<NT, false>(acc, vOB, o_off, B, N, nv, ntv, sb1, sb2, tid);
        }
    }
    if (s12a) {
        sa1 = wave_sum(sa1);
        sa2 = wave_sum(sa2);
        sb1 = wave_sum(sb1);
        sb2 = wave_sum(sb2);
        if (lane == 0) {
            red[wv][0] = sa1;
            red[wv][1] = sa2;
            red[wv][2] = sb1;
            red[wv][3] = sb2;
        }
        __syncthreads();
        if (tid < 4 && (tid < 2 ? do_a : do_b)) {
            float v = 0.f;
#pragma unroll
            for (int w = 0; w < BIG_NW; ++w) v += red[w][tid];
            float *dst = (tid < 2 ? s12a : s12b) + (long long)gc * 2 + (tid & 1);
            *dst = v;
        }
    }
}

inline bool big_path(int N) { return N > TM && N <= 256; }

}

template <int MT, bool FIN>
static void launch_fwd_big(const fgnn_slab *ya, const fgnn_slab *yb, const int *nvalid, int N, int G, float *out, long long ogstride,
                           long long ldo, const int *order, const FinArgs &F, int fill, hipStream_t st) {
    static LdsAttrCache attr_cache;
    (void)fgnn_raise_lds(attr_cache, (const void *)chan_matmul_fwd_big_kernel<MT, FIN>, BigCfg<MT>::LDS_BYTES);
    hipLaunchKernelGGL((chan_matmul_fwd_big_kernel<MT, FIN>), dim3(G * ya->C), dim3(BIG_THREADS), BigCfg<MT>::LDS_BYTES, st, *ya, *yb, nvalid, N, G, out,
                       ogstride, ldo, order, F, fill);
}

static int check_2gib(const char *name, int G, long long s0, long long s1, long long s2 = 0, long long s3 = 0) {
    FGNN_CHECK((long long)G * s0 < 0x7fffffffll / 4 && (long long)G * s1 < 0x7fffffffll / 4 && (long long)G * s2 < 0x7fffffffll / 4 &&
               (long long)G * s3 < 0x7fffffffll / 4,
               "%s: a tensor exceeds 2 GiB (32-bit buffer addressing); split the batch", name);
    return 0;
}

template <bool FIN>
static int chan_matmul_fwd_dispatch(const char *name, const fgnn_slab *ya, const fgnn_slab *yb, const int *nvalid, int G, int N,
                                    float *out, long long ogstride, long long ldo, const int *order, int fill, const FinArgs &F,
                                    hipStream_t st) {
    const int M = G * ya->C;
    if (FIN || big_path(N)) {
        if (check_2gib(name, G, ya->gstride, yb->gstride, ogstride)) return 1;
    } else if (N <= TM) {
        if (check_2gib(name, G, ya->gstride, yb->gstride)) return 1;
        FGNN_CHECK((long long)G * ogstride < 0x7fffffffll / 4, "%s: output exceeds 2 GiB", name);
    }
    if (N <= TM) {
        if (mm_wave_variant()) launch_fwd_w<FIN>(ya, yb, nvalid, N, M, out, ogstride, ldo, F, st);
        else hipLaunchKernelGGL(chan_matmul_fwd1_kernel<FIN>, dim3(M), dim3(256), 0, st, *ya, *yb, nvalid, N, M, out, ogstride, ldo, F);
    } else if (big_path(N)) {
        if (N <= 128) launch_fwd_big<4, FIN>(ya, yb, nvalid, N, G, out, ogstride, ldo, order, F, fill, st);
        else launch_fwd_big<8, FIN>(ya, yb, nvalid, N, G, out, ogstride, ldo, order, F, fill, st);
    } else if constexpr (!FIN) {
        const int t = (N + TM - 1) / TM;
        hipLaunchKernelGGL(chan_matmul_fwd_kernel, dim3(t, t, M), dim3(256), 0, st, *ya, *yb, nvalid, N, out, ogstride, ldo);
    }
    FGNN_LAUNCH_CHECK();
    return 0;
}

extern "C" int fgnn_chan_matmul_fwd(const fgnn_slab *ya, const fgnn_slab *yb, const int *nvalid, int G, int N,
                                    float *out, long long ogstride, long long ldo, void *stream) {
    return fgnn_chan_matmul_fwd_ord(ya, yb, nvalid, G, N, out, ogstride, ldo, nullptr, 0, stream);
}

extern "C" int fgnn_chan_matmul_fwd_ord(const fgnn_slab *ya, const fgnn_slab *yb, const int *nvalid, int G, int N,
                                        float *out, long long ogstride, long long ldo, const int *order, int fill, void *stream) {
    FGNN_CHECK(!order || nvalid, "fgnn_chan_matmul_fwd_ord: an order needs the nvalid it was derived from");
    FGNN_CHECK(ya && yb && out && ya->ptr && yb->ptr, "fgnn_chan_matmul_fwd: null argument");
    FGNN_CHECK(ya->C == yb->C && ya->C > 0 && G > 0 && N > 0, "fgnn_chan_matmul_fwd: bad shapes");
    FGNN_CHECK((long long)G * ya->C <= 65535 * 1024ll, "fgnn_chan_matmul_fwd: G*C too large");
    return chan_matmul_fwd_dispatch<false>("fgnn_chan_matmul_fwd", ya, yb, nvalid, G, N, out, ogstride, ldo, order, fill, FinArgs{},
                                           (hipStream_t)stream);
}

extern "C" int fgnn_chan_matmul_fwd_fin_supported(int N) { return (N <= TM || big_path(N)) ? 1 : 0; }

extern "C" int fgnn_debug_matmul_variant(int wave_per_matrix) {
    FGNN_CHECK((wave_per_matrix & ~9) == 0, "fgnn_debug_matmul_variant: bits 0 and 3 only (got %d)", wave_per_matrix);
    g_mm_wave_variant = wave_per_matrix;
    return 0;
}

extern "C" int fgnn_chan_matmul_fwd_fin(const fgnn_slab *ya, const fgnn_slab *yb, const float *part_a, const float *part_b,
                                        const float *cnt, const float *gn_weight_a, const float *gn_weight_b, float eps,
                                        const int *nvalid, int G, int N, float *out, long long ogstride, long long ldo,
                                        void *stream) {
    return fgnn_chan_matmul_fwd_fin_ord(ya, yb, part_a, part_b, cnt, gn_weight_a, gn_weight_b, eps, nvalid, G, N, out, ogstride, ldo, nullptr, 0, stream);
}

extern "C" int fgnn_chan_matmul_fwd_fin_ord(const fgnn_slab *ya, const fgnn_slab *yb, const float *part_a, const float *part_b,
                                            const float *cnt, const float *gn_weight_a, const float *gn_weight_b, float eps,
                                            const int *nvalid, int G, int N, float *out, long long ogstride, long long ldo,
                                            const int *order, int fill, void *stream) {
    FGNN_CHECK(!order || nvalid, "fgnn_chan_matmul_fwd_fin_ord: an order needs the nvalid it was derived from");
    FGNN_CHECK(ya && yb && out && ya->ptr && yb->ptr && part_a && part_b && cnt, "fgnn_chan_matmul_fwd_fin: null argument");
    FGNN_CHECK(ya->nrm && yb->nrm, "fgnn_chan_matmul_fwd_fin: the slabs must carry the record buffers to fill");
    FGNN_CHECK(ya->C == yb->C && ya->C > 0 && G > 0 && N > 0, "fgnn_chan_matmul_fwd_fin: bad shapes");
    FGNN_CHECK(N <= TM || big_path(N), "fgnn_chan_matmul_fwd_fin: N=%d > 256 (use fgnn_gn_finalize2 + fgnn_chan_matmul_fwd)", N);
    const FinArgs F = {part_a, part_b, cnt, gn_weight_a, gn_weight_b, const_cast<float *>(ya->nrm), const_cast<float *>(yb->nrm), eps,
                       fgnn_tiles_per_graph(N)};
    return chan_matmul_fwd_dispatch<true>("fgnn_chan_matmul_fwd_fin", ya, yb, nvalid, G, N, out, ogstride, ldo, order, fill, F,
                                          (hipStream_t)stream);
}

extern "C" int fgnn_chan_matmul_bwd(const fgnn_slab *ya, const fgnn_slab *yb, const float *dm, long long dmgstride,
                                    long long ldm, const int *nvalid, int G, int N, float *da, float *db,
                                    long long ogstride, long long ldo, float *s12a, float *s12b, void *stream) {
    return fgnn_chan_matmul_bwd_ord(ya, yb, dm, dmgstride, ldm, nvalid, G, N, da, db, ogstride, ldo, s12a, s12b, nullptr,
                                    0, stream);
}

extern "C" int fgnn_chan_matmul_bwd_ord(const fgnn_slab *ya, const fgnn_slab *yb, const float *dm, long long dmgstride,
                                        long long ldm, const int *nvalid, int G, int N, float *da, float *db,
                                        long long ogstride, long long ldo, float *s12a, float *s12b, const int *order,
                                        int fill, void *stream) {
    FGNN_CHECK(!order || nvalid, "fgnn_chan_matmul_bwd_ord: an order needs the nvalid it was derived from");
    FGNN_CHECK(ya && yb && dm && da && db && ya->ptr && yb->ptr, "fgnn_chan_matmul_bwd: null argument");
    FGNN_CHECK(ya->C == yb->C && ya->C > 0 && G > 0 && N > 0, "fgnn_chan_matmul_bwd: bad shapes");
    FGNN_CHECK((s12a == nullptr) == (s12b == nullptr), "fgnn_chan_matmul_bwd: s12a and s12b come together");
    FGNN_CHECK(!s12a || (ya->nrm && yb->nrm), "fgnn_chan_matmul_bwd: s12 outputs need normalised slabs");
    const int t = (N + TM - 1) / TM;
    const bool fused = s12a && t == 1;
    if (t == 1) {
        if (check_2gib("fgnn_chan_matmul_bwd", G, ya->gstride, yb->gstride, dmgstride)) return 1;
        FGNN_CHECK((long long)G * ogstride < 0x7fffffffll / 4, "fgnn_chan_matmul_bwd: output exceeds 2 GiB");
        const int M = G * ya->C;
        hipLaunchKernelGGL(chan_matmul_bwd1_kernel, dim3(M), dim3(256), 0, (hipStream_t)stream, *ya, *yb, dm,
                           dmgstride, ldm, nvalid, N, M, da, db, ogstride, ldo, s12a, s12b);
        FGNN_LAUNCH_CHECK();
        return 0;
    }
    if (big_path(N)) {
        if (check_2gib("fgnn_chan_matmul_bwd", G, ya->gstride, yb->gstride, dmgstride, ogstride)) return 1;
#define FGNN_BIG_BWD(MT)                                                                                              \
    {                                                                                                                 \
        static LdsAttrCache attr_cache;                                                                           \
        (void)fgnn_raise_lds(attr_cache, (const void *)chan_matmul_bwd_big_kernel<MT>, BigCfg<MT>::LDS_BYTES);                   \
        hipLaunchKernelGGL(chan_matmul_bwd_big_kernel<MT>, dim3(G * ya->C * (split ? 2 : 1)), dim3(BIG_THREADS),      \
                           BigCfg<MT>::LDS_BYTES, (hipStream_t)stream, *ya, *yb, dm, dmgstride, ldm, nvalid, N, G, da, \
                           db, ogstride, ldo, s12a, s12b, order, split, fill);                                            \
    }
        const int split = (order && (long long)G * ya->C <= BIG_SPLIT_MAX_MATRICES) ? 1 : 0;
        if (N <= 128) FGNN_BIG_BWD(4)
        else FGNN_BIG_BWD(8)
#undef FGNN_BIG_BWD
        FGNN_LAUNCH_CHECK();
        return 0;
    }
    hipLaunchKernelGGL(chan_matmul_bwd_kernel, dim3(t, t, G * ya->C), dim3(256), 0, (hipStream_t)stream, *ya, *yb, dm,
                       dmgstride, ldm, nvalid, N, da, db, ogstride, ldo, fused ? s12a : nullptr, fused ? s12b : nullptr);
    FGNN_LAUNCH_CHECK();
    if (s12a && !fused) {
        int rc = fgnn_gn_bwd_stats(da, ogstride, ldo, ya->ptr, ya->gstride, ya->ldp, ya->nrm, nvalid, G, ya->C, N, s12a, stream);
        if (rc) return rc;
        rc = fgnn_gn_bwd_stats(db, ogstride, ldo, yb->ptr, yb->gstride, yb->ldp, yb->nrm, nvalid, G, yb->C, N, s12b, stream);
        if (rc) return rc;
    }
    return 0;
}
```

graph_neural_net_amd/csrc/mlp_bwd_pair_t16.hip:

```cpp
#include "fgnn_bwd_t16.h"

#ifdef FGNN_PHASES
__device__ unsigned long long *g_phase16_buf = nullptr;
#define PH_DECL unsigned long long ph_[16] = {0, 0, 0, 0, 0, 0, 0, 0, 0, 0, 0, 0, 0, 0, 0, 0}; unsigned long long ph_last_ = __builtin_amdgcn_s_memtime();
#define PH(k) { const unsigned long long t_ = __builtin_amdgcn_s_memtime(); ph_[k] += t_ - ph_last_; ph_last_ = t_; }
#define PH_FLUSH if (g_phase16_buf && (threadIdx.x & 63) == 0) { for (int k_ = 0; k_ < 16; ++k_) g_phase16_buf[((long long)blockIdx.x * NW + wv) * 16 + k_] = ph_[k_]; }
#else
#define PH_DECL
#define PH(k)
#define PH_FLUSH
#endif

namespace {

struct PairLayout16 : BwdT16Layout<0, 2, 4> {
    static constexpr int OFF_W0 = PK.off_w1a, OFF_WT0 = PK.off_wt0a;
    static constexpr int XCH_OFF = TILE_END;
    static constexpr int FLAG_OFF = XCH_OFF + NP * 1024;
    static constexpr int REC_OFF = FLAG_OFF + 4 * NP;
    static constexpr int LIVE_OFF = REC_OFF + NW * 256;
    static constexpr int MAIN_F = LIVE_OFF + LIVE_LIST_CAP + NW;
    static constexpr int LDS_F = MAIN_F > RED_F ? MAIN_F : RED_F;
};

template <bool SKIP, bool HAS_DX>
__global__ __launch_bounds__(64 * NW, 2) void mlp_bwd_pair_t16_kernel(const PairArgs P, const int tpg, const int total_tiles) {
    extern __shared__ __attribute__((aligned(16))) float smem[];
    using L = PairLayout16;
    const int lane = threadIdx.x & 63, wv = __builtin_amdgcn_readfirstlane(threadIdx.x >> 6);
    const int role = wv >> 2, pair = wv & 3;
    const int px = lane & 15, q = lane >> 4;
    const fgnn_mlp_bwd_args &A = P.m[role];
    const int P2 = A.N * A.N;
    const View va = make_view(A.a.ptr, A.a.gstride, A.a.ldp, A.G);
    const View vdy = make_view(A.dy, A.dgstride, A.ldd, A.G);
    const View vz = make_view(A.z, A.zgstride, A.ldz, A.G);
    const View vdx = make_view(P.m[1].dxa, P.m[1].dxa_gstride, P.m[1].dxa_ld, P.m[1].G);

    PH_DECL
    if (role == 1) __builtin_amdgcn_s_setprio(1);
    float *wl = smem + role * L::WEIGHT_F;
    float *my = smem + L::TILE_OFF + wv * (L::NSLOT * TILE_F);
    float *XA = my, *S0 = my + TILE_F, *S1 = my + 2 * TILE_F, *S2 = my + 3 * TILE_F;
    float *XCH = smem + L::XCH_OFF + pair * 1024;
    int *flags = reinterpret_cast<int *>(smem + L::FLAG_OFF) + 4 * pair;
    const int lane_base = tile_lane_base(px, q);

    f32x4 dW0[4], dW1[4], dW2[4];
    float db0[2] = {0.f, 0.f}, db1[2] = {0.f, 0.f}, db2[2] = {0.f, 0.f};
#pragma unroll
    for (int k = 0; k < 4; ++k) dW0[k] = dW1[k] = dW2[k] = zero4();

    int T0, T1;
    wg_tile_range<SKIP>(A.ranges, total_tiles, T0, T1);
    const bool normA = A.a.nrm != nullptr;
    constexpr bool has_dx = HAS_DX;
    const bool emit = role == 1 && normA && has_dx && P.m[1].s12part != nullptr;
    const bool rmw = has_dx && P.m[1].accumulate_a;
    const bool ragged = A.nvalid != nullptr;
    const rsrc_t rnv = __builtin_amdgcn_make_buffer_rsrc(const_cast<int *>(A.nvalid), 0, ragged ? A.G * 4 : 0, 0x00020000);
    const float rcpN = 1.f / (float)A.N;

    PH(14)
    pk_glds<NW>(smem, P.m[0].packed, L::WEIGHT_F, wv, lane);
    pk_glds<NW>(smem + L::WEIGHT_F, P.m[1].packed, L::WEIGHT_F, wv, lane);
    PH(15)

    float mean[8], av[8], beta[8], kx[8], ky[8], kz[8], kw[8];
#pragma unroll
    for (int s = 0; s < 8; ++s) {
        mean[s] = 0.f;
        av[s] = 1.f;
        beta[s] = normA && A.a.beta ? A.a.beta[chan(s, 0) + chan_q(q)] : 0.f;
        kx[s] = ky[s] = kz[s] = kw[s] = 0.f;
    }
    float4 *rec = reinterpret_cast<float4 *>(smem + L::REC_OFF) + wv * 64;
    auto fetch_records = [&](int g, int nv) {
        if (lane < 32) {
            rec[lane] = coef_record(A, g, lane, nv);
            if (normA) rec[32 + lane] = reinterpret_cast<const float4 *>(A.a.nrm)[(long long)g * A.a.C + lane];
        }
    };
    auto read_records = [&]() { FGNN_T16_READ_RECORDS(normA) };

    float xa[8], dyr[8], zr[8], oldr[8];
#pragma unroll
    for (int s = 0; s < 8; ++s) oldr[s] = 0.f;
    int cached_g = -1, cur_nv = A.N;
    int tile = T0 + pair;
    int live_cnt = 0;
    if constexpr (SKIP) tile = __builtin_amdgcn_readfirstlane(next_owned_live_tile_p(T0, T1, live_cnt, pair, NP, tpg, FGNN_TILE, A.N, A.nvalid));
    int hf = 0;
    {
        const bool act = tile < T1;
        const int g = __builtin_amdgcn_readfirstlane(act ? tile / tpg : 0);
        const int p = (act ? tile - g * tpg : 0) * 32 + px;
        const bool inb0 = act && p < P2;
        load8(xa, va, lane_voff(va, q, p, inb0), g * va.gs4);
        if (act) {
            cur_nv = graph_nv(rnv, ragged, g, A.N);
            fetch_records(g, cur_nv);
            cached_g = g;
        }
    }
    PH(12)
    if (threadIdx.x < 4 * NP) reinterpret_cast<int *>(smem + L::FLAG_OFF)[threadIdx.x] = 0;
    PH(13)
    int *live_list = reinterpret_cast<int *>(smem + L::LIVE_OFF);
    int nlive = 0, li = pair;
    if constexpr (SKIP) nlive = build_live_list(live_list, live_list + LIVE_LIST_CAP, T0, T1, tpg, FGNN_TILE, A.N, A.nvalid, threadIdx.x, 64 * NW);
    const bool use_list = SKIP && nlive <= LIVE_LIST_CAP;
    __syncthreads();
    {
        const bool act = tile < T1;
        const int g = __builtin_amdgcn_readfirstlane(act ? tile / tpg : 0);
        const int p = (act ? tile - g * tpg : 0) * 32 + px;
        const bool inb0 = act && p < P2;
        load8(dyr, vdy, lane_voff(vdy, q, p, inb0), g * vdy.gs4);
        load8(zr, vz, lane_voff(vz, q, p, inb0), g * vz.gs4);
        if (has_dx) load8(oldr, vdx, lane_voff(vdx, q, p, inb0 && rmw && role == 0), g * vdx.gs4);
    }
    if (cached_g >= 0) read_records();
    PH(9)

    int hk = 0;
    float es1[8], es2[8];
#pragma unroll
    for (int s = 0; s < 8; ++s) es1[s] = es2[s] = 0.f;
    while (tile < T1) {
        int tnext = tile + NP;
        if constexpr (SKIP) {
            if (hf == 1) {
                if (use_list) {
                    li += NP;
                    tnext = __builtin_amdgcn_readfirstlane(li < nlive ? live_list[li] : T1);
                } else {
                    tnext = __builtin_amdgcn_readfirstlane(next_owned_live_tile_p(tile + 1, T1, live_cnt, pair, NP, tpg, FGNN_TILE, A.N, A.nvalid));
                }
            }
        }
        const int g = __builtin_amdgcn_readfirstlane(tile / tpg), tt = tile - g * tpg;
        const int p = tt * 32 + 16 * hf + px;
        const bool inb = p < P2;
        if (g != cached_g) {
            cur_nv = graph_nv(rnv, ragged, g, A.N);
            fetch_records(g, cur_nv);
            read_records();
            cached_g = g;
        }
        bool valid = inb;
        if (ragged) {
            int i, jj;
            row_col(p, A.N, rcpN, i, jj);
            valid = inb && i < cur_nv && jj < cur_nv;
        }
        const unsigned long long vmask = __ballot(valid);
        const bool full = vmask == ~0ull;

        const int ntile = hf == 0 ? tile : tnext, nhf = hf ^ 1;
        int np, ng;
        bool ninb;
        {
            const bool act = ntile < T1;
            ng = __builtin_amdgcn_readfirstlane(act ? ntile / tpg : 0);
            np = (act ? ntile - ng * tpg : 0) * 32 + 16 * nhf + px;
            ninb = act && np < P2;
        }

        {
            f32x4 dx[2];
            const int dvoff = lane_voff(vdx, q, p, inb), ds0 = g * vdx.gs4;

            float h1[8], h2[8], u[8];
            {
                float ya[8];
#pragma unroll
                for (int s = 0; s < 8; ++s) {
                    u[s] = xa[s] - mean[s];
                    ya[s] = u[s] * av[s] + beta[s];
                }
                stage8(XA, lane_base, ya);
                f32x4 acc[2];
                load_bias(acc, wl + L::BIAS_F, 0, q);
                gemm32<L::OFF_W0>(acc, wl, ya, lane);
                FGNN_T16_RECOMPUTE_HIDDEN(acc, h1, h2)
            }
            PH(1)
            float dpre[8];
            FGNN_T16_DZ(dpre)
            stage8(S2, lane_base, dpre);
            load8(dyr, vdy, lane_voff(vdy, q, np, ninb), ng * vdy.gs4);
            load8(zr, vz, lane_voff(vz, q, np, ninb), ng * vz.gs4);
            PH(2)
            __builtin_amdgcn_sched_barrier(0);
            FGNN_T16_HIDDEN_BWD(L::OFF_WT2, dpre, dW2, db2, S2, S1, h2)
            PH(3)
            __builtin_amdgcn_sched_barrier(0);
            stage8(S1, lane_base, dpre);
            FGNN_T16_HIDDEN_BWD(L::OFF_WT1, dpre, dW1, db1, S1, S0, h1)
            PH(4)
            __builtin_amdgcn_sched_barrier(0);
            stage8(S2, lane_base, dpre);
            __builtin_amdgcn_sched_barrier(0);
#pragma unroll
            for (int s = 0; s < 8; ++s) dx[s >> 2][s & 3] = oldr[s];
            load8(xa, va, lane_voff(va, q, np, ninb), ng * va.gs4);
            if (has_dx) load8(oldr, vdx, lane_voff(vdx, q, np, ninb && rmw && role == 0), ng * vdx.gs4);
            if (role == 0 && has_dx) gemm32<L::OFF_WT0>(dx, wl, dpre, lane);
            wgrad16(dW0, db0, S2, XA, lane);
            PH(5)
            if (role == 0) {
                if (has_dx) {
                    if (hk >= 2)
                        while (__hip_atomic_load(&flags[1], __ATOMIC_ACQUIRE, __HIP_MEMORY_SCOPE_WORKGROUP) < hk - 1) __builtin_amdgcn_s_sleep(1);
                    PH(6)
                    float *slot = XCH + (hk & 1) * 512;
#pragma unroll
                    for (int s = 0; s < 8; ++s) slot[s * 64 + lane] = dx[s >> 2][s & 3];
                    __hip_atomic_store(&flags[0], hk + 1, __ATOMIC_RELEASE, __HIP_MEMORY_SCOPE_WORKGROUP);
                }
            } else {
                if (has_dx) {
                    while (__hip_atomic_load(&flags[0], __ATOMIC_ACQUIRE, __HIP_MEMORY_SCOPE_WORKGROUP) < hk + 1) __builtin_amdgcn_s_sleep(1);
                    PH(6)
                    const float *slot = XCH + (hk & 1) * 512;
#pragma unroll
                    for (int s = 0; s < 8; ++s) dx[s >> 2][s & 3] = slot[s * 64 + lane];
                    __hip_atomic_store(&flags[1], hk + 1, __ATOMIC_RELEASE, __HIP_MEMORY_SCOPE_WORKGROUP);
                    gemm32<L::OFF_WT0>(dx, wl, dpre, lane);
                    float v[8];
#pragma unroll
                    for (int s = 0; s < 8; ++s) v[s] = dx[s >> 2][s & 3];
                    store8(v, vdx, dvoff, ds0);
                    if (emit) {
                        if (!full) {
#pragma unroll
                            for (int s = 0; s < 8; ++s) v[s] = valid ? v[s] : 0.f;
                        }
#pragma unroll
                        for (int s = 0; s < 8; ++s) {
                            es1[s] += v[s];
                            es2[s] = fmaf(v[s], u[s], es2[s]);
                        }
                    }
                }
            }
            ++hk;
        }
        PH(7)
        if (emit && hf == 1) {
            float t1 = 0.f, t2 = 0.f;
            if (ntile >= T1 || ng != g) {
                stage8(S0, lane_base, es1);
                stage8(S1, lane_base, es2);
                const int ch = lane & 31, hh = lane >> 5;
                const float4 *vp = reinterpret_cast<const float4 *>(S0 + ch * TLD + 8 * hh);
                const float4 *up = reinterpret_cast<const float4 *>(S1 + ch * TLD + 8 * hh);
#pragma unroll
                for (int k = 0; k < 2; ++k) {
                    const float4 a = vp[k], b = up[k];
                    t1 += (a.x + a.y) + (a.z + a.w);
                    t2 += (b.x + b.y) + (b.z + b.w);
                }
                t1 += __shfl_xor(t1, 32);
                t2 += __shfl_xor(t2, 32);
#pragma unroll
                for (int s = 0; s < 8; ++s) es1[s] = es2[s] = 0.f;
            }
            if (lane < 32) reinterpret_cast<float2 *>(P.m[1].s12part)[((long long)g * tpg + tt) * FGNN_H + row_chan(lane)] = make_float2(t1, t2);
        }
        tile = ntile;
        hf = nhf;
        PH(8)
    }

    if constexpr (SKIP) {
        if (emit) {
            for (int t = T0 + pair; t < T1; t += NP) {
                const int g = t / tpg, tt = t - g * tpg;
                if (tile_live(tt, A.N, A.nvalid[g])) continue;
                if (lane < 32) reinterpret_cast<float2 *>(P.m[1].s12part)[((long long)g * tpg + tt) * FGNN_H + lane] = make_float2(0.f, 0.f);
            }
        }
    }

    constexpr int PCOUNT = L::PCOUNT;
    static_assert(PCOUNT == 3 * 1056, "put() below: three layers of 32 x 32 + 32");
    FGNN_T16_DB_BUTTERFLY(db0, db1, db2)
    __syncthreads();
    PH(10)
    {
        float *red = smem + wv * PCOUNT;
        auto put = [&](int off, const f32x4 (&dW)[4], const float (&db)[2]) {
#pragma unroll
            for (int mb = 0; mb < 2; ++mb)
#pragma unroll
                for (int nb = 0; nb < 2; ++nb)
#pragma unroll
                    for (int r = 0; r < 4; ++r) red[off + row_chan(16 * mb + 4 * q + r) * 32 + row_chan(16 * nb + px)] = dW[2 * mb + nb][r];
            if (q == 0) {
                red[off + 1024 + row_chan(px)] = db[0];
                red[off + 1024 + row_chan(16 + px)] = db[1];
            }
        };
        put(0, dW0, db0);
        put(1056, dW1, db1);
        put(2112, dW2, db2);
    }
    __syncthreads();
    sum_pair_partials<PCOUNT>(smem, P);
    PH(11)
    PH_FLUSH
}

template <bool SKIP, bool HAS_DX>
int launch_pair16(const fgnn_mlp_bwd_args *a1, const fgnn_mlp_bwd_args *a2, int tpg, int total, hipStream_t st) {
    constexpr int LDS = PairLayout16::LDS_F * 4;
    static_assert(LDS <= 160 * 1024, "LDS budget");
    static LdsAttrCache attr_cache;
    (void)fgnn_raise_lds(attr_cache, (const void *)mlp_bwd_pair_t16_kernel<SKIP, HAS_DX>, LDS);
    PairArgs P;
    P.m[0] = *a1;
    P.m[1] = *a2;
    hipLaunchKernelGGL((mlp_bwd_pair_t16_kernel<SKIP, HAS_DX>), dim3(a1->cu_share == 2 && !SKIP ? BWD_WG / 2 : BWD_WG), dim3(64 * NW), LDS, st, P, tpg,
                       total);
    FGNN_LAUNCH_CHECK();
    return 0;
}

}

#ifdef FGNN_PHASES
extern "C" int fgnn_debug_phase_buffer_t16(void *p) { return hipMemcpyToSymbol(HIP_SYMBOL(g_phase16_buf), &p, sizeof(p)) == hipSuccess ? 0 : 1; }
#endif

extern "C" int fgnn_mlp_bwd_pair_t16(const fgnn_mlp_bwd_args *a1, const fgnn_mlp_bwd_args *a2, void *stream) {
    if (check_pair_common(a1, a2, "fgnn_mlp_bwd_pair_t16", 29, true)) return 1;
    FGNN_CHECK(a1->depth == 3 && a1->a.C == 32 && a1->b.C == 0 && a2->b.C == 0 && !a1->xbits && !a2->xbits,
               "fgnn_mlp_bwd_pair_t16: built for depth 3 and ONE dense input slab of 32 channels (got depth %d, %d + %d); use fgnn_mlp_bwd_pair",
               a1->depth, a1->a.C, a1->b.C);
    FGNN_CHECK(a1->ranges == a2->ranges && (!a1->ranges || a1->nvalid), "fgnn_mlp_bwd_pair_t16: both MLPs take the same ranges (with nvalid)");
    FGNN_CHECK(a1->packed && a2->packed, "fgnn_mlp_bwd_pair_t16: needs both operand images (fgnn_pack_operands, kind 5)");
    FGNN_CHECK(a1->N <= 256, "fgnn_mlp_bwd_pair_t16: N <= 256 (division-free pixel decode)");
    const int tpg = fgnn_tiles_per_graph(a1->N);
    const long long total = (long long)a1->G * tpg;
    hipStream_t st = (hipStream_t)stream;
    if (a2->dxa) return a1->ranges ? launch_pair16<true, true>(a1, a2, tpg, (int)total, st) : launch_pair16<false, true>(a1, a2, tpg, (int)total, st);
    return a1->ranges ? launch_pair16<true, false>(a1, a2, tpg, (int)total, st) : launch_pair16<false, false>(a1, a2, tpg, (int)total, st);
}
```

graph_neural_net_amd/engine.py:

```python
import ctypes as C
import os

import torch

from . import _lib
from .engine_base import EngineBase

EPS = 1e-05


class ParamLayout:

    def __init__(self, original_features_num=2, num_blocks=4, in_features=32, out_features=32, depth_of_mlp=3):
        if in_features != _lib.FGNN_H or out_features != _lib.FGNN_H:
            raise RuntimeError('the fused engine is built for in_features = out_features = 32 (got %d, %d); other widths '
                               'run through the per-layer modules (layers.MlpBlock_Real)' % (in_features, out_features))
        if not 1 <= depth_of_mlp <= _lib.FGNN_MAX_DEPTH:
            raise RuntimeError('depth_of_mlp must be in 1..%d' % _lib.FGNN_MAX_DEPTH)
        if original_features_num not in (2, 32):
            raise RuntimeError('the fused engine is built for original_features_num = 2 or 32 (got %d); other widths run '
                               'through the per-layer modules (layers.MlpBlock_Real)' % original_features_num)
        self.c0 = original_features_num
        self.num_blocks = num_blocks
        self.depth = depth_of_mlp
        self.entries = []
        self.mlp = {}
        off = 0
        last = original_features_num
        for blk in range(1, num_blocks + 1):
            for j, cin in ((1, last), (2, last), (3, last + 32)):
                pfx = 'ne_bm_block%d_mlp%d.' % (blk, j)
                rec = {'off': off, 'cin': cin, 'w': [], 'b': []}
                c = cin
                for i in range(depth_of_mlp):
                    self.entries.append((pfx + 'convs.%d.weight' % i, off, (32, c, 1, 1)))
                    rec['w'].append(off)
                    off += 32 * c
                    self.entries.append((pfx + 'convs.%d.bias' % i, off, (32,)))
                    rec['b'].append(off)
                    off += 32
                    c = 32
                self.entries.append((pfx + 'gn.weight', off, (1, 32, 1, 1)))
                rec['gn_w'] = off
                off += 32
                self.entries.append((pfx + 'gn.bias', off, (1, 32, 1, 1)))
                rec['gn_b'] = off
                off += 32
                rec['count'] = _lib.mlp_param_count(cin, depth_of_mlp)
                self.mlp[(blk, j)] = rec
            last = 32
        self.total = off

    def flatten(self, state_dict, device):
        flat = torch.empty(self.total, dtype=torch.float32, device=device)
        for name, off, shape in self.entries:
            key = name if name in state_dict else 'node_embedder.' + name
            t = state_dict[key]
            n = t.numel()
            flat[off:off + n].copy_(t.reshape(-1).to(torch.float32))
        return flat

    def init_flat(self, seed, device):
        gen = torch.Generator().manual_seed(seed)
        flat = torch.zeros(self.total, dtype=torch.float32)
        for name, off, shape in self.entries:
            n = _numel(shape)
            if name.endswith('.weight') and '.convs.' in name:
                fan_out, fan_in = shape[0], shape[1]
                bound = (6.0 / (fan_in + fan_out)) ** 0.5
                flat[off:off + n] = (torch.rand(n, generator=gen) * 2 - 1) * bound
            elif name.endswith('gn.weight'):
                flat[off:off + n] = 1.0
        return flat.to(device)

    def unflatten(self, flat):
        return {name: flat[off:off + _numel(shape)].view(shape) for name, off, shape in self.entries}


def _numel(shape):
    n = 1
    for s in shape:
        n *= s
    return n


def _round_up(x, m):
    return (x + m - 1) // m * m


class EngineCache:

    def __init__(self, budget):
        import collections
        self.budget = budget
        self._items = collections.OrderedDict()

    @staticmethod
    def engine_bytes(G, N, num_blocks, elt=4):
        ldp = -(-N * N // 32) * 32
        return (4 * num_blocks + 5) * G * 32 * ldp * elt

    def get(self, key, factory, nbytes):
        hit = self._items.get(key)
        if hit is not None:
            self._items.move_to_end(key)
            return hit[0], []
        eng = factory()
        self._items[key] = (eng, nbytes)
        evicted = []
        while self.used() > self.budget and len(self._items) > 1:
            k, _ = self._items.popitem(last=False)
            evicted.append(k)
        return eng, evicted

    def used(self):
        return sum(b for _, b in self._items.values())

    def keys(self):
        return list(self._items)

    def clear(self):
        self._items.clear()

    def __len__(self):
        return len(self._items)

    def __iter__(self):
        return iter(list(self._items))

    def values(self):
        return [e for e, _ in self._items.values()]


class FgnnEngine(EngineBase):
    SKIP_PADDING_TILES = True
    MM_ORDER = True
    PAIR_BWD = os.environ.get('FGNN_PAIR_BWD', '1') != '0'
    PACK_IN_STRUCT = os.environ.get('FGNN_PACK_IN_STRUCT', '1') != '0'
    T16 = os.environ.get('FGNN_T16', 'pair,bwd')

    MFMA = os.environ.get('FGNN_MFMA', 'f32')

    BLOCK1 = os.environ.get('FGNN_BLOCK1', 'generic')
    GN_FINALIZE = ('fgnn_gn_finalize', 'fgnn_gn_finalize2')

    def __init__(self, layout, G, N, device, ragged=False, cu_share=0, mfma=None, block1=None):
        _lib.load()
        self.T16 = type(self).T16
        self.cu_share = int(cu_share)
        mfma = self.MFMA if mfma is None else mfma
        if mfma not in ('f32', 'x3'):
            raise ValueError("mfma must be 'f32' or 'x3' (got %r)" % (mfma,))
        self.x3 = (mfma == 'x3' and not ragged and layout.depth == 3 and layout.c0 in (2, 32))
        block1 = self.BLOCK1 if block1 is None else block1
        if block1 not in ('generic', 'structured'):
            raise ValueError("block1 must be 'generic' or 'structured' (got %r)" % (block1,))
        self.struct1 = (block1 == 'structured' and cu_share == 0
                        and bool(_lib.load().fgnn_block1_struct_supported(N, layout.depth, layout.c0)))
        super().__init__(layout, G, N, device, ragged)
        self.P = N * N
        self.ldp = _round_up(self.P, 32)
        self.tpg = _lib.tiles_per_graph(N)
        self._gn_args = (EPS,)
        K = layout.num_blocks
        f32 = dict(dtype=torch.float32, device=device)
        self._act = act = lambda: torch.empty(G * 32 * self.ldp, **f32)
        self.z = {(k, j): act() for k in range(1, K + 1) for j in (1, 2, 3)}
        self.mult = {k: act() for k in range(1, K + 1)}
        self.part = [torch.empty(G * self.tpg * 32 * 2, **f32) for _ in range(2)]
        self.cnt = torch.empty(G * 2 * self.tpg, **f32)
        self.mm_order = (torch.empty(G, dtype=torch.int32, device=device)
                         if self.ranges is not None and self.MM_ORDER and 64 < N <= 256 else None)
        self.x = None
        self.xdeg = None
        self._packs = {}
        self._pack_entry = 'fgnn_pack_x3_operands' if self.x3 else 'fgnn_pack_operands'
        for k in range(1, K + 1):
            cin = layout.c0 if k == 1 else 32
            fl = _lib.load().fgnn_pack_x3_floats if self.x3 else _lib.load().fgnn_pack_floats
            f12, b12 = 0, (5 if self._t16_pair(cin) else 1)
            f3 = 2 if self.x3 else 0
            b3 = 5 if self._t16_bwd3(cin) else (3 if self.x3 else 1)
            self._packs[('f', k, 12)] = (f12, cin, 0, 2, torch.empty(fl(f12, cin, 0, layout.depth, 2), **f32))
            self._packs[('f', k, 3)] = (f3, 32, cin, 1, torch.empty(fl(f3, 32, cin, layout.depth, 1), **f32))
            for j in (1, 2):
                self._packs[('b', k, j)] = (b12, cin, 0, 1, torch.empty(fl(b12, cin, 0, layout.depth, 1), **f32))
            self._packs[('b', k, 3)] = (b3, 32, cin, 1, torch.empty(fl(b3, 32, cin, layout.depth, 1), **f32))

    def _t16(self, what):
        return self.T16 not in ('0', '') and what in self.T16.split(',')

    def _t16_pair(self, cin):
        return (self._t16('pair') and self.PAIR_BWD and not self.x3 and self.layout.depth == 3 and cin == 32 and self.N <= 256)

    def _t16_bwd3(self, cin):
        return self._t16('bwd') and not self.x3 and self.layout.depth == 3 and cin in (2, 32) and self.N <= 256

    def _slab_in(self, k, params):
        if k == 1:
            if self.xbits is not None:
                s = _lib.Slab()
                s.gstride, s.ldp, s.C = self.layout.c0 * self.P, self.P, self.layout.c0
                return s
            return _lib.make_slab(self.x, self.layout.c0 * self.P, self.P, self.layout.c0)
        rec = self.layout.mlp[(k - 1, 3)]
        s = _lib.make_slab(self.z[(k - 1, 3)], 32 * self.ldp, self.ldp, 32, nrm=self.nrm[(k - 1, 3)])
        s.beta = self._w(params, rec['gn_b'])
        return s

    def _slab_z(self, k, j, params):
        rec = self.layout.mlp[(k, j)]
        s = _lib.make_slab(self.z[(k, j)], 32 * self.ldp, self.ldp, 32, nrm=self.nrm[(k, j)])
        s.beta = self._w(params, rec['gn_b'])
        return s

    def _slab_raw(self, t):
        return _lib.make_slab(t, 32 * self.ldp, self.ldp, 32)

    def _mlp_fwd(self, params, k, js, a, b, finalize=True):
        L = self.layout
        args = _lib.MlpFwdArgs()
        args.G, args.N, args.depth, args.nmlp = self.G, self.N, L.depth, len(js)
        args.nvalid = self.nvalid.data_ptr() if self.nvalid is not None else None
        args.a = a
        if b is not None:
            args.b = b
        for m, j in enumerate(js):
            rec = L.mlp[(k, j)]
            for l in range(L.depth):
                args.W[m][l] = self._w(params, rec['w'][l])
                args.bias[m][l] = self._w(params, rec['b'][l])
            args.z[m] = self.z[(k, j)].data_ptr()
            args.part[m] = self.part[m].data_ptr()
        args.ldz = self.ldp
        args.cnt = self.cnt.data_ptr()
        args.packed = self._packs[('f', k, 12 if len(js) == 2 else 3)][4].data_ptr()
        self._packed_input(args, k)
        if self.ranges is not None:
            args.ranges = self.ranges.data_ptr()
        args.cu_share = self.cu_share
        st = _lib.stream_ptr()
        entry = 'fgnn_mlp_fwd_x3' if (self.x3 and len(js) == 2) else 'fgnn_mlp_fwd'
        _lib.call(entry, C.byref(args), st, tag='mlp_fwd[cin=%d,nmlp=%d]' % (a.C + (b.C if b is not None else 0), len(js)))
        if self.decisions is not None:
            bufs = [torch.zeros(self.G * (L.depth - 1) * 32 * self.tpg, dtype=torch.int32, device=self.device) for _ in js]
            _lib.call('fgnn_debug_mlp_fwd_x3_masks' if (self.x3 and len(js) == 2) else 'fgnn_debug_mlp_fwd_masks', C.byref(args),
                      _lib.ptr(bufs[0]), _lib.ptr(bufs[1]) if len(js) == 2 else None, st)
            for j, buf in zip(js, bufs):
                self.decisions[(k, j)] = buf
        if finalize:
            self._gn_finalize(params, k, js)

    def _packed_input(self, args, k):
        if k == 1 and self.xbits is not None:
            args.xbits = self.xbits.data_ptr()
            args.xdeg = self.xdeg.data_ptr()

    def embed(self, params, x, nvalid=None, bits=None, pack=True):
        L = self.layout
        self._adopt_nvalid(nvalid)
        st = _lib.stream_ptr()
        if self.ranges is not None:
            _lib.call('fgnn_ragged_tile_ranges_order', _lib.ptr(self.nvalid), self.G, self.N, _lib.ptr(self.ranges),
                      _lib.ptr(self.mm_order) if self.mm_order is not None else None, st, tag='fgnn_ragged_tile_ranges')
        if bits is not None:
            if x is not None or L.c0 != 2 or L.depth != 3:
                raise RuntimeError('FgnnEngine.embed: bits= replaces x and needs original_features_num = 2, depth_of_mlp = 3')
            self._check_bits(bits)
            if self.xdeg is None:
                self.xdeg = torch.empty(self.G * self.N, dtype=torch.float32, device=self.device)
            self.x, self.xbits = None, bits
            if not self.struct1:
                _lib.call('fgnn_adjacency_degree', _lib.ptr(bits), self._nv(), self.G, self.N, _lib.ptr(self.xdeg), st)
        else:
            if x.shape != (self.G, L.c0, self.N, self.N) or not x.is_contiguous() or x.dtype != torch.float32:
                raise RuntimeError('FgnnEngine.embed: expected contiguous fp32 %s, got %s %s'
                                   % ((self.G, L.c0, self.N, self.N), tuple(x.shape), x.dtype))
            self.x, self.xbits = x, None
        struct_now = self.struct1 and self.xbits is not None
        pack_in_struct = pack and struct_now and self.PACK_IN_STRUCT and not self.x3 and len(self._packs) <= _lib.MAX_PACK_JOBS
        if pack and not pack_in_struct:
            self.pack_operands(params)
        for k in range(1, L.num_blocks + 1):
            sin = self._slab_in(k, params)
            if k == 1 and struct_now:
                self._struct_fwd(params, with_pack=pack_in_struct)
                pool_fin = L.num_blocks == 1 and bool(_lib.load().fgnn_colmax_fwd_fin_supported(self.N))
                self._mlp_fwd(params, 1, (3,), self._slab_raw(self.mult[1]), sin, finalize=not pool_fin)
                continue
            fin = bool(_lib.load().fgnn_chan_matmul_fwd_fin_supported(self.N)) and self.G * 32 <= 4096
            self._mlp_fwd(params, k, (1, 2), sin, None, finalize=not fin)
            ya, yb = self._slab_z(k, 1, params), self._slab_z(k, 2, params)
            if fin:
                r1, r2 = L.mlp[(k, 1)], L.mlp[(k, 2)]
                _lib.call('fgnn_chan_matmul_fwd_fin_ord', C.byref(ya), C.byref(yb), _lib.ptr(self.part[0]), _lib.ptr(self.part[1]),
                          _lib.ptr(self.cnt), C.c_void_p(self._w(params, r1['gn_w'])), C.c_void_p(self._w(params, r2['gn_w'])),
                          EPS, self._nv(), self.G, self.N, _lib.ptr(self.mult[k]), 32 * self.ldp, self.ldp,
                          _lib.ptr(self.mm_order) if self.mm_order is not None else None, self._fill(), st, tag='fgnn_chan_matmul_fwd')
            else:
                _lib.call('fgnn_chan_matmul_fwd_ord', C.byref(ya), C.byref(yb), self._nv(), self.G, self.N,
                          _lib.ptr(self.mult[k]), 32 * self.ldp, self.ldp,
                          _lib.ptr(self.mm_order) if self.mm_order is not None else None, self._fill(), st, tag='fgnn_chan_matmul_fwd')
            pool_fin = k == L.num_blocks and bool(_lib.load().fgnn_colmax_fwd_fin_supported(self.N))
            self._mlp_fwd(params, k, (3,), self._slab_raw(self.mult[k]), sin, finalize=not pool_fin)
        out = self._slab_z(L.num_blocks, 3, params)
        if pool_fin:
            rec = L.mlp[(L.num_blocks, 3)]
            _lib.call('fgnn_colmax_fwd_fin', C.byref(out), _lib.ptr(self.part[0]), _lib.ptr(self.cnt),
                      C.c_void_p(self._w(params, rec['gn_w'])), EPS, self._nv(), self.G, self.N, _lib.ptr(self.E),
                      _lib.ptr(self.idx), st, tag='fgnn_colmax_fwd')
        else:
            _lib.call('fgnn_colmax_fwd', C.byref(out), self._nv(), self.G, self.N, _lib.ptr(self.E), _lib.ptr(self.idx), st)
        return self.E

    def _fill(self):
        return 1 if self.ranges is not None else 0

    def _struct_fwd(self, params, with_pack=False):
        S = self._struct_ws()
        st = _lib.stream_ptr()
        (w1, b1), (w2, b2) = self._w3(params, 1), self._w3(params, 2)
        r1, r2 = self.layout.mlp[(1, 1)], self.layout.mlp[(1, 2)]
        args = [_lib.ptr(self.xbits), self._nv(), self.G, self.N, _lib.ptr(S['tab']),
                C.c_void_p(self._w(params, r1['gn_w'])), C.c_void_p(self._w(params, r1['gn_b'])),
                C.c_void_p(self._w(params, r2['gn_w'])), C.c_void_p(self._w(params, r2['gn_b'])), EPS,
                _lib.ptr(self.nrm[(1, 1)]), _lib.ptr(self.nrm[(1, 2)]), _lib.ptr(self.mult[1]), 32 * self.ldp, self.ldp,
                _lib.ptr(self.xdeg), _lib.ptr(S['ws']), w1, b1, w2, b2]
        if with_pack:
            items = list(self._packs.items())
            _lib.call('fgnn_block1_struct_fwd_pack', *args, self._pack_jobs(params, items), len(items), st)
        else:
            _lib.call('fgnn_block1_struct_fwd', *args, st)

    def _struct_bwd(self, params):
        S, W = self._struct_ws(), self._bwd
        W['struct_rows'] = int(_lib.load().fgnn_block1_struct_rows(self.G, self.N))
        (w1, _), (w2, _) = self._w3(params, 1), self._w3(params, 2)
        r1, r2 = self.layout.mlp[(1, 1)], self.layout.mlp[(1, 2)]
        _lib.call('fgnn_block1_struct_bwd', _lib.ptr(self.xbits), self._nv(), self.G, self.N, _lib.ptr(S['tab']), w1, w2,
                  _lib.ptr(self.nrm[(1, 1)]), _lib.ptr(self.nrm[(1, 2)]),
                  C.c_void_p(self._w(params, r1['gn_b'])), C.c_void_p(self._w(params, r2['gn_b'])),
                  _lib.ptr(W['dmult']), 32 * self.ldp, self.ldp, _lib.ptr(S['ws']),
                  _lib.ptr(W['wpart'][(1, 1)]), _lib.ptr(W['wpart'][(1, 2)]), _lib.ptr(W['s12'][(1, 1)]), _lib.ptr(W['s12'][(1, 2)]),
                  _lib.stream_ptr())

    def _partial_rows(self):
        nwg = super()._partial_rows()
        if self.cu_share == 2 and self.ranges is None:
            nwg //= 2
        return nwg

    def _coef(self, kj, slot):
        W = self._bwd
        _lib.call('fgnn_gn_bwd_coef', _lib.ptr(W['s12'][kj]), _lib.ptr(self.nrm[kj]), self._nv(), self.G, 32, self.N,
                  _lib.ptr(W['coef'][slot]), None, None, _lib.stream_ptr())

    def _mlp_bwd(self, params, k, j, a, b, dy, coef, dxa, dxb, acc_a, acc_b, emit=False, dx_strides=None):
        args = self._mlp_bwd_args(params, k, j, a, b, dy, coef, dxa, dxb, acc_a, acc_b, emit, dx_strides)
        entry = 'fgnn_mlp_bwd_x3' if (self.x3 and j != 3) else 'fgnn_mlp_bwd'
        if j == 3 and b is not None and self._t16_bwd3(b.C) and _lib.load().fgnn_mlp_bwd_t16_supported(C.byref(args)):
            entry = 'fgnn_mlp_bwd_t16'
        elif self._packs[('b', k, j)][0] == 5:
            args.packed = None
        _lib.call(entry, C.byref(args), _lib.stream_ptr(),
                  tag='mlp_bwd[cin=%d,dx=%d]' % (a.C + (b.C if b is not None else 0),
                                                (a.C if dxa is not None else 0) + (b.C if (b is not None and dxb is not None) else 0)))

    def _mlp_bwd_pair(self, params, k, sin, din, emit):
        W = self._bwd
        a1 = self._mlp_bwd_args(params, k, 1, sin, None, W['dy1'], None, None, None, False, False, False, None)
        a2 = self._mlp_bwd_args(params, k, 2, sin, None, W['dy2'], None, din, None, True, False, emit, None)
        entry = 'fgnn_mlp_bwd_pair_x3' if self.x3 else ('fgnn_mlp_bwd_pair_t16' if self._t16_pair(sin.C) else 'fgnn_mlp_bwd_pair')
        _lib.call(entry, C.byref(a1), C.byref(a2), _lib.stream_ptr(),
                  tag='mlp_bwd_pair[cin=%d,dx=%d]' % (sin.C, sin.C if din is not None else 0))

    def _mlp_bwd_args(self, params, k, j, a, b, dy, coef, dxa, dxb, acc_a, acc_b, emit, dx_strides):
        L = self.layout
        W = self._bwd
        rec = L.mlp[(k, j)]
        gs = 32 * self.ldp
        args = _lib.MlpBwdArgs()
        args.G, args.N, args.depth = self.G, self.N, L.depth
        args.nvalid = self.nvalid.data_ptr() if self.nvalid is not None else None
        args.a = a
        if b is not None:
            args.b = b
        for l in range(L.depth):
            args.W[l] = self._w(params, rec['w'][l])
            args.bias[l] = self._w(params, rec['b'][l])
        args.dy, args.dgstride, args.ldd = dy.data_ptr(), gs, self.ldp
        args.z, args.zgstride, args.ldz = self.z[(k, j)].data_ptr(), gs, self.ldp
        if isinstance(coef, str):
            args.s12tiles = W['s12part'].data_ptr()
            args.s12_out = W['s12'][(k, j)].data_ptr()
            args.znrm = self.nrm[(k, j)].data_ptr()
        elif coef is not None:
            args.coef = coef.data_ptr()
        else:
            args.s12 = W['s12'][(k, j)].data_ptr()
            args.znrm = self.nrm[(k, j)].data_ptr()
        dgs, dld = (gs, self.ldp) if dx_strides is None else dx_strides
        if dxa is not None:
            args.dxa, args.dxa_gstride, args.dxa_ld = dxa.data_ptr(), (gs if (b is not None and dx_strides is not None) else dgs), \
                (self.ldp if (b is not None and dx_strides is not None) else dld)
        if dxb is not None:
            args.dxb, args.dxb_gstride, args.dxb_ld = dxb.data_ptr(), dgs, dld
        args.accumulate_a, args.accumulate_b = int(acc_a), int(acc_b)
        args.wpart = W['wpart'][(k, j)].data_ptr()
        args.packed = self._packs[('b', k, j)][4].data_ptr()
        self._packed_input(args, k)
        if self.ranges is not None:
            args.ranges = self.ranges.data_ptr()
        args.cu_share = self.cu_share
        if emit:
            args.s12part = W['s12part'].data_ptr()
        return args

    def backward_from_dE(self, params, grads, dE, finalize=True, dx=None):
        L = self.layout
        W = self._alloc_bwd()
        st = _lib.stream_ptr()
        gs = 32 * self.ldp
        K = L.num_blocks
        in_prologue = bool(_lib.load().fgnn_mlp_bwd_coef_tiles_supported(self.G, self.N)) and self.ranges is None
        dy = W['dy'][0]
        out = self._slab_z(K, 3, params)
        _lib.call('fgnn_colmax_bwd', _lib.ptr(dE), _lib.ptr(self.idx), self._nv(), self.G, 32, self.N,
                  _lib.ptr(dy), gs, self.ldp, C.byref(out), _lib.ptr(W['s12'][(K, 3)]), st)
        for k in range(K, 0, -1):
            sin = self._slab_in(k, params)
            first = (k == 1)
            din = None if first else W['dy'][(K - k + 1) % 2]
            dxs = None
            if first and dx is not None:
                if self.xbits is not None or self.x3 or tuple(dx.shape) != (self.G, L.c0, self.N, self.N) or dx.dtype != torch.float32 \
                        or not dx.is_contiguous():
                    raise RuntimeError('FgnnEngine: the input gradient needs a dense fp32 input, the fp32-MFMA kernels (mfma="f32") '
                                       'and a contiguous (G, c0, N, N) fp32 dx')
                din, dxs = dx, (L.c0 * self.P, self.P)
            self._mlp_bwd(params, k, 3, self._slab_raw(self.mult[k]), sin, dy,
                          None if k == K else ('tiles' if in_prologue else W['coef'][2]), W['dmult'], din, False, False, dx_strides=dxs)
            if first and self.struct1 and self.xbits is not None and dxs is None:
                self._struct_bwd(params)
                dy = din
                continue
            ya, yb = self._slab_z(k, 1, params), self._slab_z(k, 2, params)
            _lib.call('fgnn_chan_matmul_bwd_ord', C.byref(ya), C.byref(yb), _lib.ptr(W['dmult']), gs, self.ldp,
                      self._nv(), self.G, self.N, _lib.ptr(W['dy1']), _lib.ptr(W['dy2']), gs, self.ldp,
                      _lib.ptr(W['s12'][(k, 1)]), _lib.ptr(W['s12'][(k, 2)]),
                      _lib.ptr(self.mm_order) if self.mm_order is not None else None, self._fill(), st, tag='fgnn_chan_matmul_bwd')
            if first:
                W['struct_rows'] = 0
            if self.PAIR_BWD and dxs is None and L.depth == 3 and sin.C in (2, 32):
                self._mlp_bwd_pair(params, k, sin, din, emit=not first)
            else:
                self._mlp_bwd(params, k, 1, sin, None, W['dy1'], None, din, None, True, False, dx_strides=dxs)
                self._mlp_bwd(params, k, 2, sin, None, W['dy2'], None, din, None, True, False, emit=not first, dx_strides=dxs)
            if not first and not in_prologue:
                _lib.call('fgnn_gn_bwd_coef_tiles', _lib.ptr(W['s12part']), _lib.ptr(self.nrm[(k - 1, 3)]), self._nv(),
                          self.G, 32, self.N, _lib.ptr(W['s12'][(k - 1, 3)]), _lib.ptr(W['coef'][2]), st)
            dy = din
        if finalize:
            self.grad_finalize(grads)
        return grads

    def relu_decisions(self, params=None):
        L, G, N, P = self.layout, self.G, self.N, self.P
        out = {}
        bit = torch.arange(32, device=self.device, dtype=torch.int32)
        for (k, j), buf in self.decisions.items():
            w = buf.view(G, L.depth - 1, 32, self.tpg)
            m = ((w.unsqueeze(-1) >> bit) & 1).reshape(G, L.depth - 1, 32, self.tpg * 32)[..., :P].reshape(G, L.depth - 1, 32, N, N)
            for l in range(L.depth - 1):
                out[(k, j, l)] = m[:, l].bool()
        if self.struct1 and self.xbits is not None and (1, 1) not in self.decisions:
            nc = 2 + 2 * (N + 1)
            tab = self._struct['tab'].view(2, nc, 4, 32)
            words = (N + 31) // 32
            b = self.xbits.view(G, N, words).to(torch.int64) & 0xffffffff
            col = torch.arange(N, device=self.device)
            wmat = ((b[:, :, col // 32] >> (col % 32)) & 1)
            if self.nvalid is not None:
                nv = self.nvalid.to(torch.int64)
                inside = (col[None, :] < nv[:, None])
                wmat = wmat * (inside[:, :, None] & inside[:, None, :])
            deg = wmat.sum(-1)
            eye = torch.eye(N, device=self.device, dtype=torch.bool)
            diag_cls = 2 + 2 * deg + torch.diagonal(wmat, dim1=1, dim2=2)
            cls = torch.where(eye[None], diag_cls[:, :, None].expand(G, N, N), wmat)
            for j in (1, 2):
                for l in range(2):
                    hv = tab[j - 1, :, l, :] > 0
                    out[(1, j, l)] = hv[cls].permute(0, 3, 1, 2).contiguous()
        return out


    def normalized(self, k, j, params):
        rec = self.layout.mlp[(k, j)]
        y = torch.empty(self.G, 32, self.N, self.N, dtype=torch.float32, device=self.device)
        _lib.call('fgnn_gn_apply', _lib.ptr(self.z[(k, j)]), 32 * self.ldp, self.ldp, _lib.ptr(self.nrm[(k, j)]),
                  C.c_void_p(self._w(params, rec['gn_b'])), self._nv(), self.G, 32, self.N,
                  _lib.ptr(y), 32 * self.P, self.P, _lib.stream_ptr())
        return y

    def unpadded(self, buf):
        return buf.view(self.G, 32, self.ldp)[:, :, :self.P].reshape(self.G, 32, self.N, self.N).clone()
```

include/fgnn_hip.h:

```cpp
#ifndef FGNN_HIP_H
#define FGNN_HIP_H

#ifdef __cplusplus
extern "C" {
#endif

#define FGNN_H 32
#define FGNN_TILE 32
#define FGNN_MAX_DEPTH 3

typedef struct {
    const float *ptr;
    long long gstride;
    long long ldp;
    int C;
    const float *nrm;
    const float *beta;
} fgnn_slab;

const char *fgnn_last_error(void);
int fgnn_version(void);
int fgnn_tiles_per_graph(int N);
int fgnn_mlp_bwd_num_workgroups(void);

#define FGNN_MAX_PACK_JOBS 24
typedef struct {
    int kind, ca, cb, depth, nmlp;
    const float *W[2][FGNN_MAX_DEPTH];
    const float *bias[2][FGNN_MAX_DEPTH];
    float *out;
} fgnn_pack_job;
int fgnn_pack_floats(int kind, int ca, int cb, int depth, int nmlp);
int fgnn_pack_operands(const fgnn_pack_job *jobs, int njobs, void *stream);

typedef struct {
    int G, N, depth, nmlp;
    const int *nvalid;
    fgnn_slab a, b;
    const float *W[2][FGNN_MAX_DEPTH];
    const float *bias[2][FGNN_MAX_DEPTH];
    float *z[2];
    long long ldz;
    float *part[2];
    float *cnt;
    const float *packed;
    const unsigned *xbits;
    const float *xdeg;
    const int *ranges;
    int cu_share;
} fgnn_mlp_fwd_args;
int fgnn_mlp_fwd(const fgnn_mlp_fwd_args *args, void *stream);

int fgnn_pack_x3_floats(int kind, int ca, int cb, int depth, int nmlp);
int fgnn_pack_x3_operands(const fgnn_pack_job *jobs, int njobs, void *stream);
int fgnn_mlp_fwd_x3(const fgnn_mlp_fwd_args *args, void *stream);

int fgnn_gn_finalize(const float *part, const float *cnt, const float *gn_weight ,
                     const int *nvalid, int G, int C, int N, float eps, float *nrm, void *stream);
int fgnn_gn_finalize2(const float *part0, const float *part1, const float *cnt, const float *gn_weight0,
                      const float *gn_weight1, const int *nvalid, int G, int C, int N, float eps,
                      float *nrm0, float *nrm1, void *stream);
int fgnn_gn_stats(const float *x, long long gstride, long long ldp, const float *gn_weight,
                  const int *nvalid, int G, int C, int N, float eps, float *nrm, void *stream);
int fgnn_gn_apply(const float *z, long long zgstride, long long ldz, const float *nrm, const float *beta ,
                  const int *nvalid, int G, int C, int N, float *y, long long ygstride, long long ldy, void *stream);

int fgnn_gn_plane_supported(int N);
int fgnn_gn_plane_fwd(const float *x, long long gstride, long long ldp, const float *gn_weight, const float *beta ,
                      const int *nvalid, int G, int C, int N, float eps, float *y, long long ygstride, long long ldy,
                      float *nrm , void *stream);
int fgnn_gn_plane_bwd(const float *dy, long long dgstride, long long ldd, const float *z, long long zgstride, long long ldz,
                      const float *nrm, const int *nvalid, int G, int C, int N, float *dz, long long ogstride, long long ldo,
                      float *s12 , float *dgn_w , float *dgn_b , void *stream);

#define FGNN_CONV_MAX_CH 256
int fgnn_conv1x1(const float *x, long long x_gstride, long long x_ld, const float *relu_mask, const float *W,
                 long long w_ostride, long long w_kstride, const float *bias, int relu, const int *nvalid, int G, int N,
                 int M, int K, float *y, long long y_gstride, long long y_ld, void *stream);
int fgnn_conv1x1_dw_chunks(int G, int N);
int fgnn_conv1x1_dw(const float *dy, long long d_gstride, long long d_ld, const float *relu_mask, const float *x,
                    long long x_gstride, long long x_ld, const int *nvalid, int G, int N, int M, int K, float *wpart,
                    void *stream);

#define FGNN_DW_MAX_JOBS 4
typedef struct {
    const float *dy; long long d_gstride, d_ld;
    const float *relu_mask;
    const float *x; long long x_gstride, x_ld;
    int M, K;
} fgnn_dw_job;
int fgnn_conv1x1_dw_multi(const fgnn_dw_job *jobs, int njobs, const int *nvalid, int G, int N, float *wpart, void *stream);

typedef struct {
    const float *W;
    long long w_ostride, w_kstride;
    const float *bias;
    int M, K;
    int relu;
    const float *mask;
    float *out;
    long long o_gstride;
} fgnn_chain_layer;
typedef struct {
    const float *x;
    long long x_gstride, x_ld;
    int depth;
    fgnn_chain_layer layer[3];
    long long o_ld;
    const int *nvalid;
    int G, N;
} fgnn_chain_args;
int fgnn_conv_chain_supported(int depth, int K0, const int *M );
int fgnn_conv_chain(const fgnn_chain_args *args, void *stream);

typedef struct {
    const float *x;
    long long x_gstride, x_ld;
    int cin;
    const float *xb;
    long long xb_gstride, xb_ld;
    int cb;
    const float *packed;
    const int *nvalid;
    int G, N;
    float *out;
    long long o_gstride, o_ld;
    const float *dz;
    long long dz_gstride, dz_ld;
    float *dx;
    long long dx_gstride, dx_ld;
    float *dxb;
    long long dxb_gstride, dxb_ld;
    int accumulate_dx, accumulate_dxb;
    float *wpart;
} fgnn_mlp64_args;
int fgnn_mlp64_supported(int cin, int depth, int width);
int fgnn_mlp64_num_workgroups(void);
int fgnn_mlp64_param_count(int cin);
int fgnn_mlp64_packed_floats(int cin);
int fgnn_mlp64_pack(const float *W0, const float *W1, const float *W2, const float *b0, const float *b1, const float *b2, int cin,
                    float *packed, void *stream);
typedef struct {
    const float *W[3];
    const float *bias[3];
    int cin;
    float *packed;
} fgnn_mlp64_pack_job;
int fgnn_mlp64_pack_multi(const fgnn_mlp64_pack_job *jobs, int njobs, void *stream);
int fgnn_mlp64_fwd(const fgnn_mlp64_args *args, void *stream);
int fgnn_mlp64_bwd(const fgnn_mlp64_args *args, void *stream);

int fgnn_chan_matmul_fwd(const fgnn_slab *ya, const fgnn_slab *yb, const int *nvalid, int G, int N,
                         float *out, long long ogstride, long long ldo, void *stream);
int fgnn_chan_matmul_fwd_ord(const fgnn_slab *ya, const fgnn_slab *yb, const int *nvalid, int G, int N,
                             float *out, long long ogstride, long long ldo, const int *order, int fill, void *stream);
int fgnn_chan_matmul_fwd_fin_supported(int N);
int fgnn_chan_matmul_fwd_fin(const fgnn_slab *ya, const fgnn_slab *yb, const float *part_a, const float *part_b,
                             const float *cnt, const float *gn_weight_a, const float *gn_weight_b, float eps,
                             const int *nvalid, int G, int N, float *out, long long ogstride, long long ldo, void *stream);
int fgnn_chan_matmul_fwd_fin_ord(const fgnn_slab *ya, const fgnn_slab *yb, const float *part_a, const float *part_b,
                                 const float *cnt, const float *gn_weight_a, const float *gn_weight_b, float eps,
                                 const int *nvalid, int G, int N, float *out, long long ogstride, long long ldo,
                                 const int *order , int fill, void *stream);

int fgnn_colmax_fwd(const fgnn_slab *y, const int *nvalid, int G, int N, float *e ,
                    int *idx , void *stream);
int fgnn_colmax_fwd_fin_supported(int N);
int fgnn_colmax_fwd_fin(const fgnn_slab *y, const float *part, const float *cnt, const float *gn_weight, float eps,
                        const int *nvalid, int G, int N, float *e, int *idx, void *stream);

#define FGNN_SCORE_SPLIT 4
int fgnn_score_ce_fwd(const float *e1, const float *e2, const int *nvalid, int B, int C, int N,
                      float *scores, float *lse, float *pair_loss, void *stream);
int fgnn_score_row_blocks(int B, int N);
int fgnn_score_ce_fwd_blocks(const float *e1, const float *e2, const int *nvalid, int B, int C, int N, int row_blocks,
                             float *scores, float *lse, float *pair_loss, void *stream);
int fgnn_score_ce_bwd(const float *e1, const float *e2, const float *scores, const float *lse,
                      const int *nvalid, const float *gscale, int B, int C, int N,
                      float *de1, float *de2, void *stream);

int fgnn_score_ce_fwd_blocks_labels(const float *e1, const float *e2, const int *nvalid, const int *labels, int B, int C, int N,
                                    int row_blocks, float *scores, float *lse, float *pair_loss, void *stream);
int fgnn_score_ce_bwd_labels(const float *e1, const float *e2, const float *scores, const float *lse, const int *nvalid,
                             const int *labels, const float *gscale, int B, int C, int N, float *de1, float *de2, void *stream);
int fgnn_ce_fwd_labels(const float *scores, const int *nvalid, const int *labels, int B, int N, float *lse, float *pair_loss,
                       void *stream);
int fgnn_ce_bwd_labels(const float *scores, const float *lse, const int *nvalid, const int *labels, const float *gscale, int B, int N,
                       float *dscores, void *stream);

int fgnn_score_ce_bwd_w(const float *e1, const float *e2, const float *scores, const float *lse, const int *nvalid,
                        const int *labels , const float *pair_weight, const float *gscale, int B, int C, int N,
                        float *de1, float *de2, void *stream);
int fgnn_pair_weights(const int *nvalid, const int *live_dev, int mode, const float *user, int B, int N, float *w_out,
                      float *denom_out, void *stream);
int fgnn_pair_loss_w(const float *pair_loss, int row_blocks, const float *pair_weight, int B, float *out, void *stream);

int fgnn_ce_fwd(const float *scores, const int *nvalid, int B, int N, float *lse, float *pair_loss, void *stream);
int fgnn_ce_bwd(const float *scores, const float *lse, const int *nvalid, const float *gscale, int B, int N,
                float *dscores, void *stream);
int fgnn_score_bwd(const float *e1, const float *e2, const float *dscores, const int *nvalid,
                   int B, int C, int N, float *de1, float *de2, void *stream);

int fgnn_colmax_bwd(const float *de, const int *idx, const int *nvalid, int G, int C, int N,
                    float *dy, long long gstride, long long ldp, const fgnn_slab *y, float *s12, void *stream);

int fgnn_gn_bwd_stats(const float *dy, long long dgstride, long long ldd,
                      const float *z, long long zgstride, long long ldz, const float *nrm,
                      const int *nvalid, int G, int C, int N, float *s12 , void *stream);
int fgnn_gn_bwd_coef(const float *s12, const float *nrm, const int *nvalid, int G, int C, int N,
                     float *coef , float *dgn_w , float *dgn_b ,
                     void *stream);
int fgnn_gn_bwd_coef_tiles(const float *s12part, const float *nrm, const int *nvalid, int G, int C, int N,
                           float *s12, float *coef, void *stream);
int fgnn_gn_bwd_apply(const float *dy, long long dgstride, long long ldd,
                      const float *z, long long zgstride, long long ldz, const float *coef,
                      const int *nvalid, int G, int C, int N, float *dz, long long ogstride, long long ldo, void *stream);

typedef struct {
    int G, N, depth;
    const int *nvalid;
    fgnn_slab a, b;
    const float *W[FGNN_MAX_DEPTH];
    const float *bias[FGNN_MAX_DEPTH];
    const float *dy;  long long dgstride, ldd;
    const float *z;   long long zgstride, ldz;
    const float *coef;
    const float *s12;
    const float *znrm;
    float *dxa; long long dxa_gstride, dxa_ld;
    float *dxb; long long dxb_gstride, dxb_ld;
    int accumulate_a, accumulate_b;
    float *wpart;
    float *s12part;
    const float *packed;
    const float *s12tiles;
    float *s12_out;
    const unsigned *xbits;
    const float *xdeg;
    const int *ranges;
    int cu_share;
} fgnn_mlp_bwd_args;
int fgnn_mlp_bwd(const fgnn_mlp_bwd_args *args, void *stream);
int fgnn_mlp_bwd_x3(const fgnn_mlp_bwd_args *args, void *stream);
int fgnn_mlp_bwd_pair(const fgnn_mlp_bwd_args *m1, const fgnn_mlp_bwd_args *m2, void *stream);
int fgnn_mlp_bwd_pair_x3(const fgnn_mlp_bwd_args *m1, const fgnn_mlp_bwd_args *m2, void *stream);
int fgnn_mlp_bwd_t16_supported(const fgnn_mlp_bwd_args *args);
int fgnn_mlp_bwd_t16(const fgnn_mlp_bwd_args *args, void *stream);
int fgnn_mlp_bwd_pair_t16(const fgnn_mlp_bwd_args *m1, const fgnn_mlp_bwd_args *m2, void *stream);
#define FGNN_BWD_COEF_GRAPHS 4
int fgnn_mlp_bwd_coef_tiles_supported(int G, int N);
int fgnn_mlp_param_count(int Cin, int depth);
int fgnn_reduce_partials(const float *wpart, int num_wg, int count, float *out, void *stream);

#define FGNN_MAX_GRAD_JOBS 16
typedef struct {
    const float *wpart; int count; float *out;
    const float *s12; const float *nrm; float *dgn_w; float *dgn_b;
    int rows;
    float scale;
    const float *scale_dev;
} fgnn_grad_job;
int fgnn_grad_finalize(const fgnn_grad_job *jobs, int njobs, int num_wg, int G, int C, void *stream);
int fgnn_inv_node_count(const int *nvalid, int B, float *out, void *stream);

int fgnn_chan_matmul_bwd(const fgnn_slab *ya, const fgnn_slab *yb, const float *dm, long long dmgstride, long long ldm,
                         const int *nvalid, int G, int N,
                         float *da, float *db, long long ogstride, long long ldo,
                         float *s12a ,
                         float *s12b , void *stream);
int fgnn_chan_matmul_bwd_ord(const fgnn_slab *ya, const fgnn_slab *yb, const float *dm, long long dmgstride, long long ldm,
                             const int *nvalid, int G, int N, float *da, float *db, long long ogstride, long long ldo,
                             float *s12a, float *s12b, const int *order, int fill , void *stream);

int fgnn_adam_step(float *params, const float *grads, float *exp_avg, float *exp_avg_sq, int n, double lr,
                   double beta1, double beta2, double eps, int step, double grad_scale, void *stream);
int fgnn_adam_step_dev(float *params, const float *grads, float *exp_avg, float *exp_avg_sq, int n,
                       const double *hp, int *state, void *stream);
#define FGNN_GUARD_MAX_PARTS 64
#define FGNN_GUARD_SKIP_NONFINITE 1
#define FGNN_GUARD_NONFINITE 1
typedef struct {
    double max_norm;
    double norm;
    double coef;
    int flags;
    int skipped;
    int arrivals;
    int mode;
    double partial[FGNN_GUARD_MAX_PARTS];
} fgnn_guard_record;
int fgnn_grad_guard(const float *grads, int n, const double *hp, fgnn_guard_record *guard, void *stream);
int fgnn_adam_step_guarded(float *params, const float *grads, float *exp_avg, float *exp_avg_sq, int n, const double *hp,
                           int *state, const fgnn_guard_record *guard, void *stream);
int fgnn_accuracy_max(const float *scores, const int *nvalid, int B, int N, int *correct, void *stream);
#define FGNN_LSAP_MAX_N 2048
int fgnn_lsap_accuracy(const float *cost, long long bstride, int ld, const int *nvalid, int B, int N, int *correct,
                       int *assign , void *stream);

int fgnn_block1_struct_supported(int N, int depth, int original_features_num);
int fgnn_block1_struct_table_floats(int N);
long long fgnn_block1_struct_ws_floats(int G, int N);
int fgnn_block1_struct_rows(int G, int N);
int fgnn_block1_struct_fwd(const unsigned *bits, const int *nvalid, int G, int N, const float *tables, const float *gnw1, const float *gnb1,
                           const float *gnw2, const float *gnb2, float eps, float *nrm1, float *nrm2, float *mult, long long gstride,
                           long long ldp, float *xdeg , float *ws,
                           const float *const *tW1, const float *const *tb1, const float *const *tW2, const float *const *tb2
                           ,
                           void *stream);
int fgnn_block1_struct_bwd(const unsigned *bits, const int *nvalid, int G, int N, const float *tables, const float *const *W1,
                           const float *const *W2, const float *nrm1, const float *nrm2, const float *gnb1, const float *gnb2,
                           const float *dmult, long long gstride, long long ldp, float *ws, float *wpart1, float *wpart2, float *s12_1,
                           float *s12_2, void *stream);
int fgnn_block1_struct_fwd_pack(const unsigned *bits, const int *nvalid, int G, int N, const float *tables, const float *gnw1, const float *gnb1,
                                const float *gnw2, const float *gnb2, float eps, float *nrm1, float *nrm2, float *mult, long long gstride,
                                long long ldp, float *xdeg, float *ws, const float *const *tW1, const float *const *tb1,
                                const float *const *tW2, const float *const *tb2, const fgnn_pack_job *jobs, int njobs, void *stream);
int fgnn_block1_struct_fwd16(const unsigned *bits, const int *nvalid, int G, int N, int ldr, const float *tables, const float *gnw1,
                             const float *gnb1, const float *gnw2, const float *gnb2, float eps, float *nrm1, float *nrm2,
                             void *mult , long long gstride, long long ldp, void *x16 , float *ws,
                             const float *const *tW1, const float *const *tb1, const float *const *tW2, const float *const *tb2, void *stream);
int fgnn_block1_struct_fwd16_pack(const unsigned *bits, const int *nvalid, int G, int N, int ldr, const float *tables, const float *gnw1,
                                  const float *gnb1, const float *gnw2, const float *gnb2, float eps, float *nrm1, float *nrm2, void *mult,
                                  long long gstride, long long ldp, void *x16, float *ws, const float *const *tW1, const float *const *tb1,
                                  const float *const *tW2, const float *const *tb2, const fgnn_pack_job *jobs, int njobs, void *stream);
int fgnn_block1_struct_bwd16(const unsigned *bits, const int *nvalid, int G, int N, int ldr, const float *tables, const float *const *W1,
                             const float *const *W2, const float *nrm1, const float *nrm2, const float *gnb1, const float *gnb2,
                             const void *dmult , long long gstride, long long ldp, float *ws, float *wpart1, float *wpart2,
                             float *s12_1, float *s12_2, void *stream);

int fgnn_expand_adjacency(const unsigned *bits, const int *nvalid, int G, int N, float *x, void *stream);
int fgnn_pack_adjacency(const float *x, const int *nvalid, int G, int N, unsigned *bits, int *bad, void *stream);
int fgnn_pack_adjacency_ld(const float *x, const int *nvalid, int G, int Nin, int N, unsigned *bits, int *bad, void *stream);
int fgnn_pack_adjacency_pair(const float *x1, const float *x2, const int *nvalid1, const int *nvalid2, int B, int Nin, int N, unsigned *bits,
                             int *nv_out, float *inv_out, int *bad, void *stream);
int fgnn_adjacency_degree(const unsigned *bits, const int *nvalid, int G, int N, float *deg, void *stream);

#define FGNN_RANGE_WG 256
int fgnn_ragged_tile_ranges(const int *nvalid, int G, int N, int *ranges , void *stream);
int fgnn_ragged_tile_ranges_order(const int *nvalid, int G, int N, int *ranges , int *order ,
                                  void *stream);
int fgnn_ragged_tile_ranges16(const int *nvalid, int G, int N, int ldr, int *ranges , void *stream);

int fgnn_sum_scale(const float *in, int rows, int cols, float scale, float *out, void *stream);

typedef struct {
    const void *ptr;
    long long gstride;
    long long ldp;
    int C;
    const float *nrm;
    const float *beta;
} fgnn_slab16;
int fgnn_tiles_per_graph16(int N, int ldr);

int fgnn_to_bf16(const float *x, const int *nvalid, int G, int C, int N, int ldr, void *y, long long gstride, long long ldp,
                 void *stream);
int fgnn_from_bf16(const void *y, long long gstride, long long ldp, int G, int C, int N, int ldr, float *x, void *stream);
int fgnn_to_bf16_pad(const float *x, const int *nvalid, int G, int c, int CP, int N, int ldr, void *y, long long ldp, void *stream);

int fgnn_pack16_floats(int kind, int ca, int cb, int depth, int nmlp);
int fgnn_pack16_operands(const fgnn_pack_job *jobs, int njobs, void *stream);

typedef struct {
    int G, N, ldr, depth, nmlp;
    const int *nvalid;
    fgnn_slab16 a, b;
    void *z[2];
    long long ldz;
    float *part[2];
    float *cnt;
    const void *packed;
    const int *ranges;
} fgnn_mlp_fwd16_args;
int fgnn_mlp_fwd16(const fgnn_mlp_fwd16_args *args, void *stream);
int fgnn_debug_mlp_fwd16_masks(const fgnn_mlp_fwd16_args *args, unsigned *masks0, unsigned *masks1, void *stream);

int fgnn_gn_finalize_tpg(const float *part, const float *cnt, const float *gn_weight, const int *nvalid, int G, int C, int N,
                         int tpg, float eps, float *nrm, void *stream);
int fgnn_gn_finalize2_tpg(const float *part0, const float *part1, const float *cnt, const float *gn_weight0,
                          const float *gn_weight1, const int *nvalid, int G, int C, int N, int tpg, float eps, float *nrm0,
                          float *nrm1, void *stream);
int fgnn_gn_bwd_coef_tiles_tpg(const float *s12part, const float *nrm, const int *nvalid, int G, int C, int N, int tpg,
                               float *s12, float *coef, void *stream);

int fgnn_chan_matmul_fwd16(const fgnn_slab16 *ya, const fgnn_slab16 *yb, const int *nvalid, int G, int N, int ldr,
                           void *out, long long ogstride, long long ldo, void *stream);
int fgnn_chan_matmul_fwd16_fin(const fgnn_slab16 *ya, const fgnn_slab16 *yb, const float *part_a, const float *part_b,
                               const float *cnt, const float *gn_weight_a, const float *gn_weight_b, float eps, int tpg,
                               const int *nvalid, int G, int N, int ldr, void *out, long long ogstride, long long ldo,
                               void *stream);
int fgnn_chan_matmul_bwd16(const fgnn_slab16 *ya, const fgnn_slab16 *yb, const void *dm, long long dmgstride, long long ldm,
                           const int *nvalid, int G, int N, int ldr, void *da, void *db, long long ogstride, long long ldo,
                           float *s12a, float *s12b, void *stream);

int fgnn_chan_matmul_bwd16_t(const fgnn_slab16 *ya, const fgnn_slab16 *yb, const void *dm, long long dmgstride, long long ldm,
                             const float *tpart, int tpg, const int *nvalid, int G, int N, int ldr, void *da, void *db,
                             long long ogstride, long long ldo, float *s12a, float *s12b, void *stream);

int fgnn_chan_matmul_bwd16_tc(const fgnn_slab16 *ya, const fgnn_slab16 *yb, const void *dm, long long dmgstride, long long ldm,
                              const float *tpart, int tpg, const int *nvalid, int G, int N, int ldr, void *da, void *db,
                              long long ogstride, long long ldo, float *s12a, float *s12b, float *coefa, float *coefb,
                              void *stream);
int fgnn_colmax_fwd16(const fgnn_slab16 *y, const int *nvalid, int G, int N, int ldr, float *e, int *idx, void *stream);
int fgnn_colmax_bwd16(const float *de, const int *idx, const int *nvalid, int G, int C, int N, int ldr, void *dy,
                      long long gstride, long long ldp, const fgnn_slab16 *y, float *s12, void *stream);
int fgnn_colmax_bwd16_coef(const float *de, const int *idx, const int *nvalid, int G, int C, int N, int ldr, void *dy,
                           long long gstride, long long ldp, const fgnn_slab16 *y, float *s12, float *coef, void *stream);

typedef struct {
    int G, N, ldr, depth;
    const int *nvalid;
    fgnn_slab16 a, b;
    const void *dy;  long long dgstride, ldd;
    const void *z;   long long zgstride, ldz;
    const float *coef;
    void *dxa; long long dxa_gstride, dxa_ld;
    void *dxb; long long dxb_gstride, dxb_ld;
    int accumulate_a, accumulate_b;
    float *wpart;
    float *s12part;
    const void *packed;
    const int *ranges;
} fgnn_mlp_bwd16_args;
int fgnn_mlp_bwd16(const fgnn_mlp_bwd16_args *args, void *stream);
int fgnn_mlp_bwd16_pair(const fgnn_mlp_bwd16_args *m1, const fgnn_mlp_bwd16_args *m2, void *stream);

#define FGNN_PAIRGEN_ERDOS_RENYI 0
#define FGNN_PAIRGEN_REGULAR 1
#define FGNN_PAIRGEN_BARABASI_ALBERT 2
#define FGNN_PAIRGEN_EDGE_SWAP 1
#define FGNN_PAIRGEN_MAX_N 256
typedef struct {
    unsigned long long seed;
    long long first;
    int B, N;
    int family, noise_model;
    double edge_density;
    unsigned long long thr_edge;
    unsigned long long thr_noise1;
    unsigned long long thr_noise2;
    unsigned long long thr_vertex;
    int swaps_per_edge;
    unsigned *bits1, *bits2;
    int *nvalid;
} fgnn_pairgen_args;
int fgnn_pairgen_supported(int N, int family, int noise_model);
int fgnn_pairgen(const fgnn_pairgen_args *args, void *stream);
int fgnn_pairgen_indexed(const fgnn_pairgen_args *args, const long long *index, void *stream);
#define FGNN_MAX_LEVELS 64
int fgnn_pairgen_levels(const fgnn_pairgen_args *args, const long long *index ,
                        const unsigned long long *level_thr , int K, const int *level , void *stream);

#define FGNN_EPOCH_ROUNDS 8
#define FGNN_EPOCH_STREAM 6
#define FGNN_EPOCH_MAX_LOG2_M 40
int fgnn_epoch_index(unsigned long long seed, unsigned long long epoch, long long M, long long first_pos, long long count,
                     long long *out, void *stream);

#define FGNN_PLANTED_STREAM 7
#define FGNN_PLANTED_MAX_N 256
int fgnn_planted_perm(unsigned long long seed, long long first, const long long *index , const int *nvalid ,
                      int B, int N, int *labels, void *stream);
int fgnn_relabel_bits(const unsigned *in, const int *labels, const int *nvalid, int B, int N, unsigned *out, void *stream);
int fgnn_relabel_dense(const float *in, const int *labels, const int *nvalid, int B, int C, int ld, int NL, float *out, void *stream);
int fgnn_count_matches(const int *assign, const int *labels, const int *nvalid, int B, int N, int *correct, void *stream);
int fgnn_accuracy_max_labels(const float *scores, const int *labels, const int *nvalid, int B, int N, int *correct, void *stream);

#define FGNN_QAP_MAX_N 256
int fgnn_qap_objective(const unsigned *bits1, const unsigned *bits2, const int *assign, const int *nvalid, int B, int N, int *qap,
                       int *planted, int *na, int *nb, void *stream);
int fgnn_qap_improve_cost(const unsigned *bits1, const unsigned *bits2, const int *assign, const int *nvalid, int B, int N, float *cost,
                          long long bstride, int ld, void *stream);
long long fgnn_greedy_qap_ws_bytes(int B, int N);
int fgnn_greedy_qap(const unsigned *bits1, const unsigned *bits2, const int *assign0, const int *nvalid, int B, int N, int T, void *ws,
                    long long ws_bytes, int *s_best2, int *acc_best, int *t_best, int *perm_best , void *stream);
int fgnn_greedy_qap_labels(const unsigned *bits1, const unsigned *bits2, const int *assign0, const int *labels, const int *nvalid, int B,
                           int N, int T, void *ws, long long ws_bytes, int *s_best2, int *acc_best, int *t_best,
                           int *perm_best , void *stream);

#define FGNN_QAPW_MAX_N 256
int fgnn_qapw_objective(const float *a1, const float *a2, long long gstride, int ld, const int *assign, const int *nvalid, int B, int N,
                        float *qap, float *trace, float *planted, float *na, float *nb, void *stream);
int fgnn_qapw_improve_cost(const float *a1, const float *a2, long long gstride, int ld, const int *assign, const int *nvalid, int B, int N,
                           float *cost, long long bstride, int cost_ld, void *stream);
long long fgnn_greedy_qapw_ws_bytes(int B, int N);
int fgnn_greedy_qapw(const float *a1, const float *a2, long long gstride, int ld, const int *assign0, const int *nvalid, int B, int N, int T,
                     void *ws, long long ws_bytes, float *s_best, int *acc_best, int *t_best, int *perm_best ,
                     void *stream);
int fgnn_greedy_qapw_labels(const float *a1, const float *a2, long long gstride, int ld, const int *assign0, const int *labels,
                            const int *nvalid, int B, int N, int T, void *ws, long long ws_bytes, float *s_best, int *acc_best,
                            int *t_best, int *perm_best , void *stream);

#define FGNN_SPECTRAL_MAX_N 256
#define FGNN_SPECTRAL_MAX_POWERS 8
int fgnn_spectral_features(const unsigned *bits, const int *nvalid, int G, int N, int n_powers, float *out, int Nout, void *stream);

typedef struct {
    double ce_sum;
    long long nodes;
    long long correct_lsap;
    long long correct_max;
    long long pairs;
    long long steps;
} fgnn_eval_record;
int fgnn_eval_pairs(const float *scores, const int *nvalid , const int *labels , int B, int N, float *cost,
                    long long cost_bstride, int cost_ld, float *row_ce, int *row_hit, void *stream);
int fgnn_eval_pairs_labels(const float *scores, const int *nvalid , const int *labels, int B, int N, float *cost,
                           long long cost_bstride, int cost_ld, float *row_ce, int *row_hit, void *stream);
int fgnn_eval_fold(const float *row_ce, const int *row_hit, const int *correct_lsap , const int *nvalid ,
                   int B, int N, int live, double *pair_ce , int *pair_max , fgnn_eval_record *meter,
                   void *stream);
int fgnn_eval_fold_bins(const float *row_ce, const int *row_hit, const int *correct_lsap , const int *nvalid ,
                        int B, int N, int live, const int *bin , int K, double *pair_ce ,
                        int *pair_max , fgnn_eval_record *records , void *stream);

int fgnn_debug_mlp_fwd_masks(const fgnn_mlp_fwd_args *args, unsigned *masks0, unsigned *masks1 , void *stream);
int fgnn_debug_mlp_fwd_x3_masks(const fgnn_mlp_fwd_args *args, unsigned *masks0, unsigned *masks1, void *stream);
int fgnn_debug_matmul_variant(int wave_per_matrix);

#ifdef __cplusplus
}
#endif
#endif
```

Measured before the change: 42590.

## Fold GraphNorm dz into channel matmul backward and skip z reads in pair MLP bwd

The channel-matmul backward kernel gains a DZ variant. After computing the S1/S2 tile sums, it reduces them in-block, builds the GraphNorm backward coefficients and writes dz directly instead of dy. The pair MLP backward then takes dz as input, skipping the z loads and coefficient records. This removes a full read of z per element from the MLP backward. In exchange the matmul epilogue does more work and depends on the whole graph fitting in one tile (N <= TM). It is on by default through FGNN_DZ_HANDOFF.

```diff
diff --git a/graph_neural_net_amd/_lib.py b/graph_neural_net_amd/_lib.py
--- a/graph_neural_net_amd/_lib.py
+++ b/graph_neural_net_amd/_lib.py
@@ -243,6 +243,8 @@
     'fgnn_reduce_partials': [_VP, _I, _I, _VP, _VP],
     'fgnn_chan_matmul_bwd': [C.POINTER(Slab), C.POINTER(Slab), _VP, _LL, _LL, _VP, _I, _I, _VP, _VP, _LL, _LL, _VP, _VP, _VP],
     'fgnn_chan_matmul_bwd_ord': [C.POINTER(Slab), C.POINTER(Slab), _VP, _LL, _LL, _VP, _I, _I, _VP, _VP, _LL, _LL, _VP, _VP, _VP, _I, _VP],
+    'fgnn_chan_matmul_bwd_dz_supported': [_I],
+    'fgnn_chan_matmul_bwd_dz': [C.POINTER(Slab), C.POINTER(Slab), _VP, _LL, _LL, _VP, _I, _I, _VP, _VP, _LL, _LL, _VP, _VP, _VP],
     'fgnn_sum_scale': [_VP, _I, _I, _F, _VP, _VP],
     'fgnn_adam_step': [_VP, _VP, _VP, _VP, _I, C.c_double, C.c_double, C.c_double, C.c_double, _I, C.c_double, _VP],
     'fgnn_adam_step_dev': [_VP, _VP, _VP, _VP, _I, _VP, _VP, _VP],
diff --git a/graph_neural_net_amd/csrc/fgnn_bwd32.h b/graph_neural_net_amd/csrc/fgnn_bwd32.h
--- a/graph_neural_net_amd/csrc/fgnn_bwd32.h
+++ b/graph_neural_net_amd/csrc/fgnn_bwd32.h
@@ -1,5 +1,6 @@
 #pragma once
 #include "fgnn_common.h"
+#include "fgnn_norm.h"
 
 namespace {
 
@@ -8,15 +9,6 @@
 constexpr int NP = 4;
 static_assert(BWD_WG == FGNN_RANGE_WG, "fgnn_ragged_tile_ranges splits for the backward grid");
 
-DEVI float4 coef_from_sums(const float4 n, const float2 sv, float nv) {
-    const float m = nv * nv;
-    float4 k;
-    k.x = n.x;
-    k.y = n.y;
-    k.z = m > 0.f ? -n.y * sv.y * n.w / m : 0.f;
-    k.w = m > 0.f ? -n.y * sv.x / m : 0.f;
-    return k;
-}
 DEVI float4 coef_record(const fgnn_mlp_bwd_args &A, int g, int ch, int nv) {
     if (A.coef) return reinterpret_cast<const float4 *>(A.coef)[(long long)g * FGNN_H + ch];
     const float4 n = reinterpret_cast<const float4 *>(A.znrm)[(long long)g * FGNN_H + ch];
@@ -83,7 +75,8 @@
     FGNN_CHECK(BWD_WG == fgnn_mlp_bwd_num_workgroups(), "%s: workgroup count differs from fgnn_mlp_bwd", fn);
     return 0;
 }
-inline int check_pair_common(const fgnn_mlp_bwd_args *a1, const fgnn_mlp_bwd_args *a2, const char *fn, int tile_bits, bool dense_only) {
+inline int check_pair_common(const fgnn_mlp_bwd_args *a1, const fgnn_mlp_bwd_args *a2, const char *fn, int tile_bits, bool dense_only,
+                             bool dz_in_ok = false) {
     FGNN_CHECK(a1 && a2, "%s: null args", fn);
     FGNN_CHECK(BWD_WG == fgnn_mlp_bwd_num_workgroups(), "%s: workgroup count differs from fgnn_mlp_bwd", fn);
     FGNN_CHECK(a1->G > 0 && a1->N > 0 && a1->G == a2->G && a1->N == a2->N && a1->depth == a2->depth,
@@ -94,9 +87,16 @@
                "%s: the two MLPs must read the same input slab", fn);
     FGNN_CHECK(!a1->dxa && !a1->s12part, "%s: the input gradient and its tile sums belong to the SECOND argument block", fn);
     FGNN_CHECK(!a1->s12tiles && !a2->s12tiles, "%s: s12tiles is an mlp3 feature", fn);
+    const bool dz_in = dz_in_ok && !a1->z && !a2->z;
+    FGNN_CHECK(!dz_in_ok || (a1->z == nullptr) == (a2->z == nullptr), "%s: both MLPs take dz (no z), or neither does", fn);
     for (const fgnn_mlp_bwd_args *a : {a1, a2}) {
-        FGNN_CHECK(a->dy && a->z && a->wpart, "%s: missing dy/z/wpart", fn);
-        FGNN_CHECK(a->coef || (a->s12 && a->znrm), "%s: need coef, or s12 + znrm", fn);
+        if (dz_in) {
+            FGNN_CHECK(a->dy && a->wpart, "%s: missing dy/wpart", fn);
+            FGNN_CHECK(!a->coef && !a->s12 && !a->znrm, "%s: without z, dy holds dz: no coef, s12 or znrm", fn);
+        } else {
+            FGNN_CHECK(a->dy && a->z && a->wpart, "%s: missing dy/z/wpart", fn);
+            FGNN_CHECK(a->coef || (a->s12 && a->znrm), "%s: need coef, or s12 + znrm", fn);
+        }
         const long long lim = 0x7fffffffll / 4, G = a->G;
         FGNN_CHECK(G * a->a.gstride < lim && G * a->dgstride < lim && G * a->zgstride < lim && G * a->dxa_gstride < lim,
                    "%s: a tensor exceeds 2 GiB (32-bit buffer addressing); split the batch", fn);
diff --git a/graph_neural_net_amd/csrc/fgnn_bwd_t16.h b/graph_neural_net_amd/csrc/fgnn_bwd_t16.h
--- a/graph_neural_net_amd/csrc/fgnn_bwd_t16.h
+++ b/graph_neural_net_amd/csrc/fgnn_bwd_t16.h
@@ -46,9 +46,24 @@
     stage8(S1, lane_base, h2);
 
 #define FGNN_T16_DZ(dpre)                                                                                                   \
-    _Pragma("unroll") for (int s = 0; s < 8; ++s) dpre[s] = fmaf(kz[s], zr[s] - kx[s], fmaf(ky[s], dyr[s], kw[s]));         \
+    _Pragma("unroll") for (int s = 0; s < 8; ++s) dpre[s] = dz_from_coef(ky[s], kz[s], kw[s], zr[s] - kx[s], dyr[s]);       \
     if (!full) {                                                                                                            \
         _Pragma("unroll") for (int s = 0; s < 8; ++s) dpre[s] = valid ? dpre[s] : 0.f;                                      \
+    }
+
+#define FGNN_T16_DZ_IN(dpre)                                                                                                \
+    _Pragma("unroll") for (int s = 0; s < 8; ++s) dpre[s] = dyr[s];                                                         \
+    if (!full) {                                                                                                            \
+        _Pragma("unroll") for (int s = 0; s < 8; ++s) dpre[s] = valid ? dpre[s] : 0.f;                                      \
+    }
+
+#define FGNN_T16_READ_IN_RECORDS(norm)                              \
+    if (norm) {                                                     \
+        _Pragma("unroll") for (int s = 0; s < 8; ++s) {             \
+            const float4 n = rec[32 + chan_s(s) + chan_q(q)];       \
+            mean[s] = n.x;                                          \
+            av[s] = n.y;                                            \
+        }                                                           \
     }
 
 #define FGNN_T16_HIDDEN_BWD(OFF_WT, dpre, dW, db, Dt, In, h)                                                \
diff --git a/graph_neural_net_amd/csrc/fgnn_norm.h b/graph_neural_net_amd/csrc/fgnn_norm.h
--- a/graph_neural_net_amd/csrc/fgnn_norm.h
+++ b/graph_neural_net_amd/csrc/fgnn_norm.h
@@ -80,6 +80,17 @@
     return r;
 }
 
+DEVI float4 coef_from_sums(const float4 n, const float2 sv, float nv) {
+    const float m = nv * nv;
+    float4 k;
+    k.x = n.x;
+    k.y = n.y;
+    k.z = m > 0.f ? -n.y * sv.y * n.w / m : 0.f;
+    k.w = m > 0.f ? -n.y * sv.x / m : 0.f;
+    return k;
+}
+DEVI float dz_from_coef(float ca, float cb, float cc, float u, float dy) { return fmaf(cb, u, fmaf(ca, dy, cc)); }
+
 DEVI float4 finalize_wave(const float *part, const float *cnt, int g, int c, int C, int tpg, float nv, float w, float eps,
                           int lane, bool tr = false) {
     return finalize_reduce(finalize_load(part, cnt, g, c, C, tpg, lane, tr), nv, w, eps);
diff --git a/graph_neural_net_amd/csrc/matmul.hip b/graph_neural_net_amd/csrc/matmul.hip
--- a/graph_neural_net_amd/csrc/matmul.hip
+++ b/graph_neural_net_amd/csrc/matmul.hip
@@ -225,6 +225,29 @@
             s1 += t;
             s2 += t * u[k];
         }
+    }
+}
+
+DEVI void tile_sums(float (&t)[16], const float *lds, const float (&u)[16], float &s1, float &s2, int tid) {
+    const int c = tid & 63, r0 = __builtin_amdgcn_readfirstlane(tid >> 6);
+    const float *lp = lds + r0 * LDS_LD + c;
+#pragma unroll
+    for (int k = 0; k < 16; ++k) {
+        t[k] = lp[4 * k * LDS_LD];
+        s1 += t[k];
+        s2 += t[k] * u[k];
+    }
+}
+DEVI void tile_dz_to_global(const View &ov, int mat_off4, const float (&t)[16], const float (&u)[16], const float4 &kc, int N, int nv,
+                            int tid) {
+    const int c = tid & 63, r0 = __builtin_amdgcn_readfirstlane(tid >> 6);
+    const int voff = c < N ? (r0 * N + c) * 4 : OOB_OFF;
+    const bool cok = c < nv;
+#pragma unroll
+    for (int k = 0; k < 16; ++k) {
+        const int r = r0 + 4 * k;
+        const float dz = (cok && r < nv) ? dz_from_coef(kc.y, kc.z, kc.w, u[k], t[k]) : 0.f;
+        buf_store(dz, ov, r < N ? voff : OOB_OFF, mat_off4 + k * 16 * N);
     }
 }
 
@@ -321,6 +344,7 @@
     }
 }
 
+template <bool DZ>
 __global__ __launch_bounds__(256, 4) void chan_matmul_bwd1_kernel(const fgnn_slab ya, const fgnn_slab yb,
                                                                const float *dm, long long dmg, long long ldm,
                                                                const int *nvalid, int N, int M, float *da, float *db,
@@ -384,7 +408,20 @@
         frag_to_lds(Bs, 32 * qi, 32 * qj, accB, lane);
         __syncthreads();
         float sa1 = 0.f, sa2 = 0.f, sb1 = 0.f, sb2 = 0.f;
-        if (s12a) {
+        if constexpr (DZ) {
+            const float4 ra = reinterpret_cast<const float4 *>(ya.nrm)[gc], rb = reinterpret_cast<const float4 *>(yb.nrm)[gc];
+            float ta[16], tb[16];
+            tile_sums(ta, Ds, ua, sa1, sa2, tid);
+            tile_sums(tb, Bs, ub, sb1, sb2, tid);
+            s12_epilogue(red, sa1, sa2, sb1, sb2, s12a, s12b, gc, tid);
+            float tot[4];
+#pragma unroll
+            for (int i = 0; i < 4; ++i) tot[i] = (red[0][i] + red[1][i]) + (red[2][i] + red[3][i]);
+            const float4 ka = coef_from_sums(ra, make_float2(tot[0], tot[1]), (float)nv);
+            const float4 kb = coef_from_sums(rb, make_float2(tot[2], tot[3]), (float)nv);
+            tile_dz_to_global(vOA, o_off, ta, ua, ka, N, nv, tid);
+            tile_dz_to_global(vOB, o_off, tb, ub, kb, N, nv, tid);
+        } else if (s12a) {
             tile_to_global<true>(vOA, o_off, Ds, N, ua, sa1, sa2, tid);
             tile_to_global<true>(vOB, o_off, Bs, N, ub, sb1, sb2, tid);
             s12_epilogue(red, sa1, sa2, sb1, sb2, s12a, s12b, gc, tid);
@@ -1069,7 +1106,7 @@
         if (check_2gib("fgnn_chan_matmul_bwd", G, ya->gstride, yb->gstride, dmgstride)) return 1;
         FGNN_CHECK((long long)G * ogstride < 0x7fffffffll / 4, "fgnn_chan_matmul_bwd: output exceeds 2 GiB");
         const int M = G * ya->C;
-        hipLaunchKernelGGL(chan_matmul_bwd1_kernel, dim3(M), dim3(256), 0, (hipStream_t)stream, *ya, *yb, dm,
+        hipLaunchKernelGGL(chan_matmul_bwd1_kernel<false>, dim3(M), dim3(256), 0, (hipStream_t)stream, *ya, *yb, dm,
                            dmgstride, ldm, nvalid, N, M, da, db, ogstride, ldo, s12a, s12b);
         FGNN_LAUNCH_CHECK();
         return 0;
@@ -1102,3 +1139,22 @@
     }
     return 0;
 }
+
+extern "C" int fgnn_chan_matmul_bwd_dz_supported(int N) { return (N > 0 && N <= TM) ? 1 : 0; }
+
+extern "C" int fgnn_chan_matmul_bwd_dz(const fgnn_slab *ya, const fgnn_slab *yb, const float *dm, long long dmgstride,
+                                       long long ldm, const int *nvalid, int G, int N, float *dza, float *dzb,
+                                       long long ogstride, long long ldo, float *s12a, float *s12b, void *stream) {
+    FGNN_CHECK(ya && yb && dm && dza && dzb && ya->ptr && yb->ptr, "fgnn_chan_matmul_bwd_dz: null argument");
+    FGNN_CHECK(ya->C == yb->C && ya->C > 0 && G > 0 && N > 0, "fgnn_chan_matmul_bwd_dz: bad shapes");
+    FGNN_CHECK(fgnn_chan_matmul_bwd_dz_supported(N), "fgnn_chan_matmul_bwd_dz: N=%d > %d (use fgnn_chan_matmul_bwd: the MLP backward forms dz)", N, TM);
+    FGNN_CHECK(s12a && s12b, "fgnn_chan_matmul_bwd_dz: dz needs the S1 / S2 sums: s12a and s12b are outputs, not optional");
+    FGNN_CHECK(ya->nrm && yb->nrm, "fgnn_chan_matmul_bwd_dz: dz needs normalised slabs (GraphNorm records)");
+    if (check_2gib("fgnn_chan_matmul_bwd_dz", G, ya->gstride, yb->gstride, dmgstride)) return 1;
+    FGNN_CHECK((long long)G * ogstride < 0x7fffffffll / 4, "fgnn_chan_matmul_bwd_dz: output exceeds 2 GiB");
+    const int M = G * ya->C;
+    hipLaunchKernelGGL(chan_matmul_bwd1_kernel<true>, dim3(M), dim3(256), 0, (hipStream_t)stream, *ya, *yb, dm, dmgstride, ldm,
+                       nvalid, N, M, dza, dzb, ogstride, ldo, s12a, s12b);
+    FGNN_LAUNCH_CHECK();
+    return 0;
+}
diff --git a/graph_neural_net_amd/csrc/mlp_bwd_pair_t16.hip b/graph_neural_net_amd/csrc/mlp_bwd_pair_t16.hip
--- a/graph_neural_net_amd/csrc/mlp_bwd_pair_t16.hip
+++ b/graph_neural_net_amd/csrc/mlp_bwd_pair_t16.hip
@@ -23,7 +23,7 @@
     static constexpr int LDS_F = MAIN_F > RED_F ? MAIN_F : RED_F;
 };
 
-template <bool SKIP, bool HAS_DX>
+template <bool SKIP, bool HAS_DX, bool DZ_IN>
 __global__ __launch_bounds__(64 * NW, 2) void mlp_bwd_pair_t16_kernel(const PairArgs P, const int tpg, const int total_tiles) {
     extern __shared__ __attribute__((aligned(16))) float smem[];
     using L = PairLayout16;
@@ -34,7 +34,7 @@
     const int P2 = A.N * A.N;
     const View va = make_view(A.a.ptr, A.a.gstride, A.a.ldp, A.G);
     const View vdy = make_view(A.dy, A.dgstride, A.ldd, A.G);
-    const View vz = make_view(A.z, A.zgstride, A.ldz, A.G);
+    const View vz = DZ_IN ? vdy : make_view(A.z, A.zgstride, A.ldz, A.G);
     const View vdx = make_view(P.m[1].dxa, P.m[1].dxa_gstride, P.m[1].dxa_ld, P.m[1].G);
 
     PH_DECL
@@ -77,11 +77,17 @@
     float4 *rec = reinterpret_cast<float4 *>(smem + L::REC_OFF) + wv * 64;
     auto fetch_records = [&](int g, int nv) {
         if (lane < 32) {
-            rec[lane] = coef_record(A, g, lane, nv);
+            if constexpr (!DZ_IN) rec[lane] = coef_record(A, g, lane, nv);
             if (normA) rec[32 + lane] = reinterpret_cast<const float4 *>(A.a.nrm)[(long long)g * A.a.C + lane];
         }
     };
-    auto read_records = [&]() { FGNN_T16_READ_RECORDS(normA) };
+    auto read_records = [&]() {
+        if constexpr (DZ_IN) {
+            FGNN_T16_READ_IN_RECORDS(normA)
+        } else {
+            FGNN_T16_READ_RECORDS(normA)
+        }
+    };
 
     float xa[8], dyr[8], zr[8], oldr[8];
 #pragma unroll
@@ -117,7 +123,7 @@
         const int p = (act ? tile - g * tpg : 0) * 32 + px;
         const bool inb0 = act && p < P2;
         load8(dyr, vdy, lane_voff(vdy, q, p, inb0), g * vdy.gs4);
-        load8(zr, vz, lane_voff(vz, q, p, inb0), g * vz.gs4);
+        if constexpr (!DZ_IN) load8(zr, vz, lane_voff(vz, q, p, inb0), g * vz.gs4);
         if (has_dx) load8(oldr, vdx, lane_voff(vdx, q, p, inb0 && rmw && role == 0), g * vdx.gs4);
     }
     if (cached_g >= 0) read_records();
@@ -187,10 +193,14 @@
             }
             PH(1)
             float dpre[8];
-            FGNN_T16_DZ(dpre)
+            if constexpr (DZ_IN) {
+                FGNN_T16_DZ_IN(dpre)
+            } else {
+                FGNN_T16_DZ(dpre)
+            }
             stage8(S2, lane_base, dpre);
             load8(dyr, vdy, lane_voff(vdy, q, np, ninb), ng * vdy.gs4);
-            load8(zr, vz, lane_voff(vz, q, np, ninb), ng * vz.gs4);
+            if constexpr (!DZ_IN) load8(zr, vz, lane_voff(vz, q, np, ninb), ng * vz.gs4);
             PH(2)
             __builtin_amdgcn_sched_barrier(0);
             FGNN_T16_HIDDEN_BWD(L::OFF_WT2, dpre, dW2, db2, S2, S1, h2)
@@ -313,16 +323,16 @@
     PH_FLUSH
 }
 
-template <bool SKIP, bool HAS_DX>
+template <bool SKIP, bool HAS_DX, bool DZ_IN>
 int launch_pair16(const fgnn_mlp_bwd_args *a1, const fgnn_mlp_bwd_args *a2, int tpg, int total, hipStream_t st) {
     constexpr int LDS = PairLayout16::LDS_F * 4;
     static_assert(LDS <= 160 * 1024, "LDS budget");
     static LdsAttrCache attr_cache;
-    (void)fgnn_raise_lds(attr_cache, (const void *)mlp_bwd_pair_t16_kernel<SKIP, HAS_DX>, LDS);
+    (void)fgnn_raise_lds(attr_cache, (const void *)mlp_bwd_pair_t16_kernel<SKIP, HAS_DX, DZ_IN>, LDS);
     PairArgs P;
     P.m[0] = *a1;
     P.m[1] = *a2;
-    hipLaunchKernelGGL((mlp_bwd_pair_t16_kernel<SKIP, HAS_DX>), dim3(a1->cu_share == 2 && !SKIP ? BWD_WG / 2 : BWD_WG), dim3(64 * NW), LDS, st, P, tpg,
+    hipLaunchKernelGGL((mlp_bwd_pair_t16_kernel<SKIP, HAS_DX, DZ_IN>), dim3(a1->cu_share == 2 && !SKIP ? BWD_WG / 2 : BWD_WG), dim3(64 * NW), LDS, st, P, tpg,
                        total);
     FGNN_LAUNCH_CHECK();
     return 0;
@@ -335,7 +345,7 @@
 #endif
 
 extern "C" int fgnn_mlp_bwd_pair_t16(const fgnn_mlp_bwd_args *a1, const fgnn_mlp_bwd_args *a2, void *stream) {
-    if (check_pair_common(a1, a2, "fgnn_mlp_bwd_pair_t16", 29, true)) return 1;
+    if (check_pair_common(a1, a2, "fgnn_mlp_bwd_pair_t16", 29, true, true)) return 1;
     FGNN_CHECK(a1->depth == 3 && a1->a.C == 32 && a1->b.C == 0 && a2->b.C == 0 && !a1->xbits && !a2->xbits,
                "fgnn_mlp_bwd_pair_t16: built for depth 3 and ONE dense input slab of 32 channels (got depth %d, %d + %d); use fgnn_mlp_bwd_pair",
                a1->depth, a1->a.C, a1->b.C);
@@ -345,6 +355,13 @@
     const int tpg = fgnn_tiles_per_graph(a1->N);
     const long long total = (long long)a1->G * tpg;
     hipStream_t st = (hipStream_t)stream;
-    if (a2->dxa) return a1->ranges ? launch_pair16<true, true>(a1, a2, tpg, (int)total, st) : launch_pair16<false, true>(a1, a2, tpg, (int)total, st);
-    return a1->ranges ? launch_pair16<true, false>(a1, a2, tpg, (int)total, st) : launch_pair16<false, false>(a1, a2, tpg, (int)total, st);
+#define FGNN_PAIR16(DZ_IN_)                                                                                                                      \
+    {                                                                                                                                            \
+        if (a2->dxa)                                                                                                                             \
+            return a1->ranges ? launch_pair16<true, true, DZ_IN_>(a1, a2, tpg, (int)total, st) : launch_pair16<false, true, DZ_IN_>(a1, a2, tpg, (int)total, st); \
+        return a1->ranges ? launch_pair16<true, false, DZ_IN_>(a1, a2, tpg, (int)total, st) : launch_pair16<false, false, DZ_IN_>(a1, a2, tpg, (int)total, st);   \
+    }
+    if (!a1->z) FGNN_PAIR16(true)
+    FGNN_PAIR16(false)
+#undef FGNN_PAIR16
 }
diff --git a/graph_neural_net_amd/engine.py b/graph_neural_net_amd/engine.py
--- a/graph_neural_net_amd/engine.py
+++ b/graph_neural_net_amd/engine.py
@@ -138,13 +138,14 @@
     PAIR_BWD = os.environ.get('FGNN_PAIR_BWD', '1') != '0'
     PACK_IN_STRUCT = os.environ.get('FGNN_PACK_IN_STRUCT', '1') != '0'
     T16 = os.environ.get('FGNN_T16', 'pair,bwd')
+    DZ_HANDOFF = os.environ.get('FGNN_DZ_HANDOFF', '1') != '0'
 
     MFMA = os.environ.get('FGNN_MFMA', 'f32')
 
     BLOCK1 = os.environ.get('FGNN_BLOCK1', 'generic')
     GN_FINALIZE = ('fgnn_gn_finalize', 'fgnn_gn_finalize2')
 
-    def __init__(self, layout, G, N, device, ragged=False, cu_share=0, mfma=None, block1=None):
+    def __init__(self, layout, G, N, device, ragged=False, cu_share=0, mfma=None, block1=None, dz_handoff=None):
         _lib.load()
         self.T16 = type(self).T16
         self.cu_share = int(cu_share)
@@ -186,6 +187,10 @@
             for j in (1, 2):
                 self._packs[('b', k, j)] = (b12, cin, 0, 1, torch.empty(fl(b12, cin, 0, layout.depth, 1), **f32))
             self._packs[('b', k, 3)] = (b3, 32, cin, 1, torch.empty(fl(b3, 32, cin, layout.depth, 1), **f32))
+        handoff = self.DZ_HANDOFF if dz_handoff is None else bool(dz_handoff)
+        self.dz_blocks = frozenset(k for k in range(1, K + 1)
+                                   if handoff and self._t16_pair(layout.c0 if k == 1 else 32)
+                                   and _lib.load().fgnn_chan_matmul_bwd_dz_supported(N))
 
     def _t16(self, what):
         return self.T16 not in ('0', '') and what in self.T16.split(',')
@@ -366,10 +371,13 @@
                   tag='mlp_bwd[cin=%d,dx=%d]' % (a.C + (b.C if b is not None else 0),
                                                 (a.C if dxa is not None else 0) + (b.C if (b is not None and dxb is not None) else 0)))
 
-    def _mlp_bwd_pair(self, params, k, sin, din, emit):
+    def _mlp_bwd_pair(self, params, k, sin, din, emit, dz_in=False):
         W = self._bwd
         a1 = self._mlp_bwd_args(params, k, 1, sin, None, W['dy1'], None, None, None, False, False, False, None)
         a2 = self._mlp_bwd_args(params, k, 2, sin, None, W['dy2'], None, din, None, True, False, emit, None)
+        if dz_in:
+            for a in (a1, a2):
+                a.z, a.zgstride, a.ldz, a.s12, a.znrm = None, 0, 0, None, None
         entry = 'fgnn_mlp_bwd_pair_x3' if self.x3 else ('fgnn_mlp_bwd_pair_t16' if self._t16_pair(sin.C) else 'fgnn_mlp_bwd_pair')
         _lib.call(entry, C.byref(a1), C.byref(a2), _lib.stream_ptr(),
                   tag='mlp_bwd_pair[cin=%d,dx=%d]' % (sin.C, sin.C if din is not None else 0))
@@ -416,12 +424,14 @@
             args.s12part = W['s12part'].data_ptr()
         return args
 
-    def backward_from_dE(self, params, grads, dE, finalize=True, dx=None):
+    def backward_from_dE(self, params, grads, dE, finalize=True, dx=None, hook=None):
         L = self.layout
         W = self._alloc_bwd()
         st = _lib.stream_ptr()
         gs = 32 * self.ldp
         K = L.num_blocks
+        if hook is None:
+            hook = lambda stage, k: None
         in_prologue = bool(_lib.load().fgnn_mlp_bwd_coef_tiles_supported(self.G, self.N)) and self.ranges is None
         dy = W['dy'][0]
         out = self._slab_z(K, 3, params)
@@ -445,17 +455,25 @@
                 dy = din
                 continue
             ya, yb = self._slab_z(k, 1, params), self._slab_z(k, 2, params)
-            _lib.call('fgnn_chan_matmul_bwd_ord', C.byref(ya), C.byref(yb), _lib.ptr(W['dmult']), gs, self.ldp,
-                      self._nv(), self.G, self.N, _lib.ptr(W['dy1']), _lib.ptr(W['dy2']), gs, self.ldp,
-                      _lib.ptr(W['s12'][(k, 1)]), _lib.ptr(W['s12'][(k, 2)]),
-                      _lib.ptr(self.mm_order) if self.mm_order is not None else None, self._fill(), st, tag='fgnn_chan_matmul_bwd')
+            dz_in = k in self.dz_blocks and dxs is None
+            if dz_in:
+                _lib.call('fgnn_chan_matmul_bwd_dz', C.byref(ya), C.byref(yb), _lib.ptr(W['dmult']), gs, self.ldp,
+                          self._nv(), self.G, self.N, _lib.ptr(W['dy1']), _lib.ptr(W['dy2']), gs, self.ldp,
+                          _lib.ptr(W['s12'][(k, 1)]), _lib.ptr(W['s12'][(k, 2)]), st, tag='fgnn_chan_matmul_bwd')
+            else:
+                _lib.call('fgnn_chan_matmul_bwd_ord', C.byref(ya), C.byref(yb), _lib.ptr(W['dmult']), gs, self.ldp,
+                          self._nv(), self.G, self.N, _lib.ptr(W['dy1']), _lib.ptr(W['dy2']), gs, self.ldp,
+                          _lib.ptr(W['s12'][(k, 1)]), _lib.ptr(W['s12'][(k, 2)]),
+                          _lib.ptr(self.mm_order) if self.mm_order is not None else None, self._fill(), st, tag='fgnn_chan_matmul_bwd')
+            hook('matmul_bwd', k)
             if first:
                 W['struct_rows'] = 0
             if self.PAIR_BWD and dxs is None and L.depth == 3 and sin.C in (2, 32):
-                self._mlp_bwd_pair(params, k, sin, din, emit=not first)
+                self._mlp_bwd_pair(params, k, sin, din, emit=not first, dz_in=dz_in)
             else:
                 self._mlp_bwd(params, k, 1, sin, None, W['dy1'], None, din, None, True, False, dx_strides=dxs)
                 self._mlp_bwd(params, k, 2, sin, None, W['dy2'], None, din, None, True, False, emit=not first, dx_strides=dxs)
+            hook('mlp2_bwd', k)
             if not first and not in_prologue:
                 _lib.call('fgnn_gn_bwd_coef_tiles', _lib.ptr(W['s12part']), _lib.ptr(self.nrm[(k - 1, 3)]), self._nv(),
                           self.G, 32, self.N, _lib.ptr(W['s12'][(k - 1, 3)]), _lib.ptr(W['coef'][2]), st)
diff --git a/include/fgnn_hip.h b/include/fgnn_hip.h
--- a/include/fgnn_hip.h
+++ b/include/fgnn_hip.h
@@ -271,6 +271,10 @@
 int fgnn_chan_matmul_bwd_ord(const fgnn_slab *ya, const fgnn_slab *yb, const float *dm, long long dmgstride, long long ldm,
                              const int *nvalid, int G, int N, float *da, float *db, long long ogstride, long long ldo,
                              float *s12a, float *s12b, const int *order, int fill , void *stream);
+int fgnn_chan_matmul_bwd_dz_supported(int N);
+int fgnn_chan_matmul_bwd_dz(const fgnn_slab *ya, const fgnn_slab *yb, const float *dm, long long dmgstride, long long ldm,
+                            const int *nvalid, int G, int N, float *dza, float *dzb, long long ogstride, long long ldo,
+                            float *s12a, float *s12b, void *stream);
 
 int fgnn_adam_step(float *params, const float *grads, float *exp_avg, float *exp_avg_sq, int n, double lr,
                    double beta1, double beta2, double eps, int step, double grad_scale, void *stream);
```

After: 42890 (median of 6 runs). About the same (+0.7%).
